# EpicDuckPotato/stereo_vo

Measured on AMD Instinct MI355X. Metric: stereo frames/sec on 1241x376 KITTI pairs, higher is better.
Workload: dtype u8/f32/f64; 1 GPU; kitti_1241x376_1500corners_5kf_window (BASELINE configs[1]); streams_per_gpu=96, max_corners=1500, window=5, pipeline_groups=3, hardware_queues=4

## Files before the change

### include/svo.h

```cpp
#ifndef SVO_H_
#define SVO_H_

#include <stddef.h>
#include <stdint.h>

#ifdef __cplusplus
extern "C" {
#endif

typedef enum svo_status {
  SVO_OK = 0,
  SVO_ERR_INVALID = -1,
  SVO_ERR_HIP = -2,
  SVO_ERR_CAPACITY = -3,
  SVO_ERR_NO_DEVICE = -4,
  SVO_ERR_NUMERIC = -5
} svo_status;

typedef struct svo_camera_info {
  double focal, cx, cy;
  double k1, k2, p1, p2;
  double baseline;
} svo_camera_info;

// ... 195 lines not shown
typedef struct svo_lm_ops {
  void* user;
  int (*linearize)(void* user, double radius, int first, double* payload1);
  int (*step)(void* user, const double* dc, const double* cand_poses7, double radius, const svo_lm_step_ctl* ctl,
              double* payload2, double* payload1_next, double* next_radius, int* next_at_candidate);
  int (*accept)(void* user);
} svo_lm_ops;
typedef struct svo_lm_stats {
  int linearize_calls;
  int step_calls;
  int speculations;
  int speculation_hits;
  int single_exchange;
  int collectives;
  int device_control;
  int fallbacks;
  double host_us;
} svo_lm_stats;

void svo_ba_default_options(svo_ba_options* o);
int svo_lm_solve(int n_poses, double* poses7, const svo_lm_ops* ops, const svo_ba_options* opt,
                 svo_ba_summary* summary, svo_lm_stats* stats);
int svo_lm_decide_step(double cost, double mcc, double radius, double decrease_factor, double cost_new,
                       double model_change_points, int* accept, double* next_radius);
int svo_ba_create(svo_ctx* ctx, svo_ba** out, int window_size, const svo_camera_info* cam,
                  const svo_ba_options* opt, int max_landmarks, int max_observations);
void svo_ba_destroy(svo_ba* ba);
int svo_ba_reset(svo_ba* ba);
int svo_ba_add_keyframe(svo_ba* ba, const double* pose7, const int64_t* tracked_ids,
                        const float* tracked_xy, int n_tracked, const float* new_xy,
                        const float* new_xyz, int n_new, int64_t* new_ids, int* n_new_out);
int svo_ba_solve(svo_ba* ba, svo_ba_summary* summary);
int svo_cholesky_solve(double* A, double* b, int n);
int svo_cholesky_solve_dev(svo_ctx* ctx, double* A, double* b, int n);
int svo_ba_get_pose(svo_ba* ba, int k, double* pose7);
int svo_ba_window_count(svo_ba* ba);
int svo_ba_get_points(svo_ba* ba, const int64_t* ids, int n, float* xyz);

int svo_ba_load_problem(svo_ba* ba, int n_poses, const double* poses7, int n_points,
                        const double* points3, int n_obs, const int32_t* obs_pose,
                        const int32_t* obs_point, const double* obs_uv);
int svo_ba_set_allreduce(svo_ba* ba, svo_allreduce_fn fn, void* user);
int svo_ba_set_comm(svo_ba* ba, void* nccl_comm);
int svo_rccl_unique_id(void* id128);
int svo_rccl_comm_create(void** nccl_comm, int n_ranks, int rank, const void* id128, int device);
int svo_rccl_comm_destroy(void* nccl_comm);
int svo_ba_set_device_lm(svo_ba* ba, int mode);
int svo_ba_set_solve_form(svo_ba* ba, int form);
int svo_ba_set_bulk_control(svo_ba* ba, int mode);
int svo_ba_last_stats(svo_ba* ba, svo_lm_stats* stats);
int svo_ba_wave_chunks_limit(void);
int svo_ba_set_wave_chunks(svo_ba* ba, int k);
int svo_ba_solve_forms(svo_ba* ba, long* counts, int n, long* gave_up);
int svo_ba_solve_problem(svo_ba* ba, svo_ba_summary* summary);
int svo_ba_solve_problems(svo_ba** bas, int n, svo_ba_summary* summaries);
int svo_ba_read_problem(svo_ba* ba, double* poses7, double* points3);

typedef struct svo_pipeline svo_pipeline;
typedef struct svo_pipeline_params {
  svo_camera_info cam;
  int width, height;
  int max_corners;
  double quality;
  float min_feature_distance;
  float parallax_thresh;
  int window_size;
  int max_features;
  int ba_max_iterations;
  double ba_max_time_s;
} svo_pipeline_params;

typedef struct svo_frame_result {
  int n_detected, n_tracked, n_inliers, n_new;
  int is_keyframe;
  float av_parallax, percent_lost;
  double pose7[7];
  int ba_iterations;
} svo_frame_result;

void svo_pipeline_default_params(svo_pipeline_params* p);
int svo_pipeline_create(svo_ctx* ctx, svo_pipeline** out, const svo_pipeline_params* p);
void svo_pipeline_destroy(svo_pipeline* p);
int svo_pipeline_reset(svo_pipeline* p);
int svo_pipeline_process_batch_dev(svo_pipeline* p, const uint8_t* left, const uint8_t* right,
                                   int batch, svo_frame_result* results);
int svo_pipeline_process_batch(svo_pipeline* p, const uint8_t* left, const uint8_t* right,
                               int batch, svo_frame_result* results);
int svo_pipeline_set_rectification(svo_pipeline* p, const svo_rectify_eye* left, const svo_rectify_eye* right);
int svo_pipeline_set_keyframe_clouds(svo_pipeline* p, const svo_cloud_params* params, int max_keyframes_per_call);
int svo_pipeline_set_keyframe_speckle_filter(svo_pipeline* p, const svo_speckle_params* params);
int svo_pipeline_set_keyframe_lr_check(svo_pipeline* p, const svo_lr_check_params* params);
int svo_pipeline_set_keyframe_sgm(svo_pipeline* p, const svo_sgm_params* params);
typedef struct svo_keyframe_cloud {
  int frame;
  int lane;
  int n_total, n_stored;
  const svo_cloud_point* dev;
} svo_keyframe_cloud;
int svo_pipeline_keyframe_clouds(svo_pipeline* p, int* n, const svo_keyframe_cloud** table);
int svo_pipeline_copy_keyframe_cloud(svo_pipeline* p, int i, svo_cloud_point* host, int capacity);
int svo_pipeline_get_tracked(svo_pipeline* p, int64_t* ids, float* xy, int capacity, int* n);

typedef struct svo_pipeline_group svo_pipeline_group;
int svo_pipeline_group_create(svo_ctx* ctx, svo_pipeline_group** out, const svo_pipeline_params* p, int n_lanes);
void svo_pipeline_group_destroy(svo_pipeline_group* g);
int svo_pipeline_group_reset(svo_pipeline_group* g);
int svo_pipeline_group_lanes(const svo_pipeline_group* g);
int svo_pipeline_group_process_batch_dev(svo_pipeline_group* g, const uint8_t* left, const uint8_t* right, size_t lane_stride,
                                         int batch, svo_frame_result* results);
int svo_pipeline_group_staging(svo_pipeline_group* g, int slot, uint8_t** left, uint8_t** right, size_t* lane_stride);
int svo_pipeline_group_upload(svo_pipeline_group* g, int slot, int batch);
int svo_pipeline_group_process_uploaded(svo_pipeline_group* g, int slot, svo_frame_result* results);
int svo_pipeline_group_process_batch(svo_pipeline_group* g, const uint8_t* left, const uint8_t* right, size_t lane_stride,
                                     int batch, svo_frame_result* results);
int svo_pipeline_group_set_rectification(svo_pipeline_group* g, int lane, const svo_rectify_eye* left, const svo_rectify_eye* right);
int svo_pipeline_group_set_keyframe_clouds(svo_pipeline_group* g, int lane, const svo_cloud_params* params, int max_keyframes_per_call);
int svo_pipeline_group_set_keyframe_speckle_filter(svo_pipeline_group* g, const svo_speckle_params* params);
int svo_pipeline_group_set_keyframe_lr_check(svo_pipeline_group* g, const svo_lr_check_params* params);
int svo_pipeline_group_set_keyframe_sgm(svo_pipeline_group* g, const svo_sgm_params* params);
int svo_pipeline_group_keyframe_clouds(svo_pipeline_group* g, int* n, const svo_keyframe_cloud** table);
int svo_pipeline_group_copy_keyframe_cloud(svo_pipeline_group* g, int i, svo_cloud_point* host, int capacity);
int svo_pipeline_group_get_tracked(svo_pipeline_group* g, int lane, int64_t* ids, float* xy, int capacity, int* n);
int svo_pipeline_group_last_stats(const svo_pipeline_group* g, long* launches6, long* lanes6);
int svo_pipeline_group_solve_work(svo_pipeline_group* g, double* out4, int reset);
int svo_pipeline_group_solve_forms(svo_pipeline_group* g, long* counts, int n, long* gave_up);

int svo_draw_track(const uint8_t* gray, int width, int height, int row_stride, const float* from_xy,
                   const float* to_xy, int n, uint8_t* rgb);
int svo_pipeline_draw_track(svo_pipeline* p, const uint8_t* keyframe_gray, int row_stride, uint8_t* rgb);

typedef struct svo_synth_params {
  uint64_t seed;
  int width, height;
  double focal, cx, cy, baseline;
  double step_z, step_x, yaw_per_frame;
  int n_billboards;
} svo_synth_params;
void svo_synth_default_params(svo_synth_params* p, int width, int height);
int svo_synth_render(const svo_synth_params* p, int frame, uint8_t* left, uint8_t* right);
int svo_synth_pose(const svo_synth_params* p, int frame, double* rt12);

int svo_image_read_gray(const char* path, uint8_t* buf, size_t capacity, int* width, int* height);
int svo_kitti_read_poses(const char* poses_file, double* rt12, int capacity_frames, int* n_frames);
int svo_ate_rmse(const double* est_xyz, const double* gt_xyz, int n, int with_scale, double* rmse);
typedef struct svo_run_stats {
  int frames, keyframes;
  double ate_rmse;
  double seconds;
} svo_run_stats;
int svo_kitti_run(svo_ctx* ctx, const svo_pipeline_params* params, const char* data_path, int sequence,
                  int max_frames, double* traj_rt12, svo_run_stats* stats);

#ifdef __cplusplus
}
#endif
#endif
```

### stereo_vo_amd/api.py

```python
import ctypes as C
import os

import numpy as np

_HERE = os.path.dirname(os.path.abspath(__file__))
_LIB = None


class SvoError(RuntimeError):
    pass


def lib_path():
    return os.path.join(_HERE, "libsvo_hip.so")


class Limits(C.Structure):
    _fields_ = [("max_width", C.c_int), ("max_height", C.c_int), ("max_batch", C.c_int),
                ("max_corners", C.c_int), ("max_candidates", C.c_int), ("max_features", C.c_int)]


class CameraInfo(C.Structure):
    _fields_ = [(n, C.c_double) for n in ("focal", "cx", "cy", "k1", "k2", "p1", "p2", "baseline")]

# ... 216 lines not shown
def lm_decide_step(cost, mcc, radius, decrease_factor, cost_new, model_change_points):
    acc, rad = C.c_int(0), C.c_double(0.0)
    lib().svo_lm_decide_step(C.c_double(cost), C.c_double(mcc), C.c_double(radius), C.c_double(decrease_factor), C.c_double(cost_new),
                             C.c_double(model_change_points), C.byref(acc), C.byref(rad))
    return bool(acc.value), rad.value


def lm_solve(poses7, linearize, step, accept, max_iterations=50, max_time_s=0.0):
    poses = np.ascontiguousarray(poses7, np.float64).copy()
    K = poses.shape[0]
    n = 6 * (K - 1)
    pay1 = n * n + 3 * n + 2

    def _lin(user, radius, first, out):
        np.ctypeslib.as_array(out, shape=(pay1,))[:] = linearize(radius, first)
        return 0

    def _step(user, dc, cand, radius, ctl, out2, out1, out_radius, out_at_cand):
        d = np.ctypeslib.as_array(dc, shape=(max(n, 1),))[:n].copy()
        c = np.ctypeslib.as_array(cand, shape=(K, 7)).copy()
        p2, p1, nr, at_cand = step(d, c, radius, ctl.contents)
        np.ctypeslib.as_array(out2, shape=(4,))[:] = p2
        if p1 is not None:
            np.ctypeslib.as_array(out1, shape=(pay1,))[:] = p1
        out_radius[0] = nr if p1 is not None else 0.0
        out_at_cand[0] = int(bool(at_cand))
        return 0

    def _acc(user):
        accept()
        return 0
    ops = LmOps(None, LM_LINEARIZE_FN(_lin), LM_STEP_FN(_step), LM_ACCEPT_FN(_acc))
    opt = ba_default_options()
    opt.max_iterations, opt.max_time_s = max_iterations, max_time_s
    s, st = BASummary(), LmStats()
    rc = lib().svo_lm_solve(K, _p(poses), C.byref(ops), C.byref(opt), C.byref(s), C.byref(st))
    if rc:
        raise SvoError(f"svo_lm_solve failed ({rc})")
    return poses, s, st


ALLREDUCE_FN = C.CFUNCTYPE(C.c_int, C.c_void_p, C.c_size_t, C.c_void_p)

SYMBOLS = [
    "svo_create", "svo_destroy", "svo_last_error", "svo_stream", "svo_sync", "svo_version", "svo_reference_constants",
    "svo_profile_select", "svo_profile_read", "svo_measure_peak",
    "svo_reproj_eval", "svo_reproj_eval_dev",
    "svo_corner_detect", "svo_corner_detect_batch_dev", "svo_corner_response",
    "svo_stereo_bm", "svo_stereo_disparity_at", "svo_stereo_disparity_at_dev",
    "svo_triangulate", "svo_lk_track", "svo_build_pyramid", "svo_track_features", "svo_dedup",
    "svo_pnp_ransac",
    "svo_ba_default_options", "svo_ba_create", "svo_ba_destroy", "svo_ba_reset", "svo_ba_add_keyframe", "svo_ba_solve",
    "svo_ba_get_pose", "svo_ba_window_count", "svo_ba_get_points", "svo_ba_load_problem",
    "svo_ba_set_allreduce", "svo_ba_set_device_lm", "svo_ba_set_bulk_control", "svo_ba_set_solve_form", "svo_ba_wave_chunks_limit", "svo_ba_set_wave_chunks", "svo_ba_solve_forms", "svo_ba_solve_problem", "svo_ba_solve_problems", "svo_ba_read_problem", "svo_ba_set_comm", "svo_ba_last_stats", "svo_lm_solve", "svo_lm_decide_step",
    "svo_rccl_unique_id", "svo_rccl_comm_create", "svo_rccl_comm_destroy",
    "svo_pipeline_default_params", "svo_pipeline_create", "svo_pipeline_destroy", "svo_pipeline_reset",
    "svo_pipeline_process_batch_dev", "svo_pipeline_process_batch", "svo_pipeline_get_tracked",
    "svo_pipeline_group_create", "svo_pipeline_group_destroy", "svo_pipeline_group_reset", "svo_pipeline_group_lanes",
    "svo_pipeline_group_process_batch_dev", "svo_pipeline_group_get_tracked", "svo_pipeline_group_last_stats",
    "svo_pipeline_group_solve_work", "svo_pipeline_group_solve_forms", "svo_pipeline_group_staging", "svo_pipeline_group_upload", "svo_pipeline_group_process_uploaded", "svo_pipeline_group_process_batch",
    "svo_synth_default_params", "svo_synth_render", "svo_synth_pose",
    "svo_image_read_gray", "svo_kitti_read_poses", "svo_ate_rmse", "svo_kitti_run", "svo_cholesky_solve", "svo_cholesky_solve_dev", "svo_draw_track", "svo_pipeline_draw_track",
    "svo_rectify_eye_from_camera_info", "svo_rectify_build_map", "svo_rectify_remap", "svo_rectify_remap_batch_dev",
    "svo_pipeline_set_rectification", "svo_pipeline_group_set_rectification",
    "svo_stereo_bm_batch_dev", "svo_cloud_default_params", "svo_disparity_cloud_batch_dev", "svo_stereo_cloud",
    "svo_pipeline_set_keyframe_clouds", "svo_pipeline_keyframe_clouds", "svo_pipeline_copy_keyframe_cloud",
    "svo_pipeline_group_set_keyframe_clouds", "svo_pipeline_group_keyframe_clouds", "svo_pipeline_group_copy_keyframe_cloud",
    "svo_speckle_workspace_bytes", "svo_disparity_speckle_filter_batch_dev", "svo_disparity_speckle_filter",
    "svo_pipeline_set_keyframe_speckle_filter", "svo_pipeline_group_set_keyframe_speckle_filter",
    "svo_stereo_bm_cost_batch_dev", "svo_disparity_lr_check_batch_dev", "svo_disparity_lr_check",
    "svo_pipeline_set_keyframe_lr_check", "svo_pipeline_group_set_keyframe_lr_check",
    "svo_sgm_default_params", "svo_sgm_workspace_bytes", "svo_stereo_sgm_batch_dev", "svo_stereo_sgm",
    "svo_pipeline_set_keyframe_sgm", "svo_pipeline_group_set_keyframe_sgm",
    "svo_voxel_map_default_params", "svo_voxel_map_bytes", "svo_voxel_map_create", "svo_voxel_map_destroy", "svo_voxel_map_clear",
    "svo_voxel_map_insert_dev", "svo_pose7_to_cam_to_world", "svo_voxel_map_insert_pose7_dev", "svo_voxel_map_stats",
    "svo_voxel_map_extract_dev", "svo_voxel_map_extract", "svo_voxel_map_download",
]


def lib():
    global _LIB
    if _LIB is None:
        p = lib_path()
        if not os.path.exists(p):
            raise SvoError(f"{p} not built — run `python -c 'import __graft_entry__ as g; g.build()'`")
        L = C.CDLL(p)
        L.svo_version.restype = C.c_char_p
        L.svo_last_error.restype = C.c_char_p
        L.svo_last_error.argtypes = [C.c_void_p]
        L.svo_stream.restype = C.c_void_p
        L.svo_stream.argtypes = [C.c_void_p]
        L.svo_destroy.argtypes = [C.c_void_p]
        L.svo_destroy.restype = None
        vp, ci, sz = C.c_void_p, C.c_int, C.c_size_t
        L.svo_cloud_default_params.argtypes = [vp, ci, ci]
        L.svo_stereo_bm_batch_dev.argtypes = [vp, vp, vp, ci, ci, ci, ci, sz, ci, ci, vp]
        L.svo_disparity_cloud_batch_dev.argtypes = [vp, vp, vp, ci, ci, ci, ci, sz, vp, vp, vp, vp, vp]
        L.svo_stereo_cloud.argtypes = [vp, vp, vp, ci, ci, ci, ci, ci, vp, vp, vp, vp, vp, vp]
        L.svo_pipeline_set_keyframe_clouds.argtypes = [vp, vp, ci]
        L.svo_pipeline_keyframe_clouds.argtypes = [vp, vp, vp]
        L.svo_pipeline_copy_keyframe_cloud.argtypes = [vp, ci, vp, ci]
        L.svo_pipeline_group_set_keyframe_clouds.argtypes = [vp, ci, vp, ci]
        L.svo_pipeline_group_keyframe_clouds.argtypes = [vp, vp, vp]
        L.svo_pipeline_group_copy_keyframe_cloud.argtypes = [vp, ci, vp, ci]
        for f in ("svo_cloud_default_params", "svo_stereo_bm_batch_dev", "svo_disparity_cloud_batch_dev", "svo_stereo_cloud",
                  "svo_pipeline_set_keyframe_clouds", "svo_pipeline_keyframe_clouds", "svo_pipeline_copy_keyframe_cloud",
                  "svo_pipeline_group_set_keyframe_clouds", "svo_pipeline_group_keyframe_clouds", "svo_pipeline_group_copy_keyframe_cloud"):
            getattr(L, f).restype = ci
        L.svo_speckle_workspace_bytes.argtypes = [ci, ci, ci]
        L.svo_speckle_workspace_bytes.restype = sz
        L.svo_disparity_speckle_filter_batch_dev.argtypes = [vp, vp, ci, ci, ci, vp, vp, sz, vp]
        L.svo_disparity_speckle_filter.argtypes = [vp, vp, ci, ci, vp, vp]
        L.svo_pipeline_set_keyframe_speckle_filter.argtypes = [vp, vp]
# ... 439 lines not shown
        ctx._chk(self.L.svo_ba_create(ctx.h, C.byref(self.h), window_size, C.byref(cam), C.byref(opt),
                                      max_landmarks, max_observations), "svo_ba_create")
        if device_lm is not None:
            ctx._chk(self.L.svo_ba_set_device_lm(self.h, 1 if device_lm else 0), "svo_ba_set_device_lm")
        if solve_form is not None:
            ctx._chk(self.L.svo_ba_set_solve_form(self.h, {"wide": 0, "compact": 1}[solve_form]), "svo_ba_set_solve_form")
        if bulk_control is not None:
            ctx._chk(self.L.svo_ba_set_bulk_control(self.h, 1 if bulk_control else 0), "svo_ba_set_bulk_control")
        self.L.svo_ba_destroy.argtypes = [C.c_void_p]
        self._cb = None

    def close(self):
        if self.h:
            self.L.svo_ba_destroy(self.h)
            self.h = C.c_void_p()

    def __del__(self):
        try:
            self.close()
        except Exception:
            pass

    def load_problem(self, poses7, points3, obs_pose, obs_point, obs_uv):
        poses7, points3, obs_uv = _f64(poses7), _f64(points3), _f64(obs_uv)
        op = np.ascontiguousarray(obs_pose, np.int32)
        oj = np.ascontiguousarray(obs_point, np.int32)
        self._shape = (poses7.shape[0], points3.shape[0])
        self.ctx._chk(self.L.svo_ba_load_problem(self.h, poses7.shape[0], _p(poses7), points3.shape[0],
                                                 _p(points3), op.shape[0], _p(op), _p(oj), _p(obs_uv)),
                      "svo_ba_load_problem")

    def set_allreduce(self, fn):
        self._cb = ALLREDUCE_FN(lambda ptr, n, user: int(fn(ptr, n) or 0)) if fn else None
        self.ctx._chk(self.L.svo_ba_set_allreduce(self.h, self._cb if self._cb else C.cast(None, ALLREDUCE_FN), None),
                      "svo_ba_set_allreduce")

    def set_comm(self, nccl_comm):
        self.ctx._chk(self.L.svo_ba_set_comm(self.h, C.c_void_p(nccl_comm) if nccl_comm else None), "svo_ba_set_comm")

    def solve_problem(self):
        s = BASummary()
        self.ctx._chk(self.L.svo_ba_solve_problem(self.h, C.byref(s)), "svo_ba_solve_problem")
        return s

    def set_wave_chunks(self, k):
        self.ctx._chk(self.L.svo_ba_set_wave_chunks(self.h, int(k)), "svo_ba_set_wave_chunks")

    def solve_forms(self):
        n = self.L.svo_ba_wave_chunks_limit() + 1
        out, gu = (C.c_long * n)(), C.c_long(0)
        self.ctx._chk(self.L.svo_ba_solve_forms(self.h, out, n, C.byref(gu)), "svo_ba_solve_forms")
        return list(out), gu.value

    @staticmethod
    def solve_problems(bas):
        n = len(bas)
        hs = (C.c_void_p * n)(*[b.h for b in bas])
        sums = (BASummary * n)()
        rc = bas[0].L.svo_ba_solve_problems(hs, n, sums)
        if rc < 0:
            bas[0].ctx._chk(rc, "svo_ba_solve_problems")
        return rc, list(sums)

    def last_stats(self):
        st = LmStats()
        self.ctx._chk(self.L.svo_ba_last_stats(self.h, C.byref(st)), "svo_ba_last_stats")
        return st

    def read_problem(self):
        K, N = self._shape
        poses = np.empty((K, 7))
        pts = np.empty((N, 3))
        self.ctx._chk(self.L.svo_ba_read_problem(self.h, _p(poses), _p(pts)), "svo_ba_read_problem")
        return poses, pts

    def add_keyframe(self, pose7, tracked_ids, tracked_xy, new_xy, new_xyz):
        pose7 = _f64(pose7)
        tid = np.ascontiguousarray(tracked_ids, np.int64)
        txy, nxy, nxyz = _f32(tracked_xy), _f32(new_xy), _f32(new_xyz)
        nn = nxy.shape[0] if nxy.ndim == 2 else 0
        ids = np.empty(max(nn, 1), np.int64)
        m = C.c_int(0)
        self.ctx._chk(self.L.svo_ba_add_keyframe(self.h, _p(pose7), _p(tid), _p(txy), tid.shape[0], _p(nxy),
                                                 _p(nxyz), nn, _p(ids), C.byref(m)), "svo_ba_add_keyframe")
        return ids[:m.value].copy()

    def solve(self):
        s = BASummary()
        self.ctx._chk(self.L.svo_ba_solve(self.h, C.byref(s)), "svo_ba_solve")
        return s

    def get_pose(self, k=-1):
        p = np.empty(7)
        self.ctx._chk(self.L.svo_ba_get_pose(self.h, k, _p(p)), "svo_ba_get_pose")
        return p

    def window_count(self):
        return self.L.svo_ba_window_count(self.h)

    def get_points(self, ids):
        ids = np.ascontiguousarray(ids, np.int64)
        out = np.empty((ids.shape[0], 3), np.float32)
        self.ctx._chk(self.L.svo_ba_get_points(self.h, _p(ids), ids.shape[0], _p(out)), "svo_ba_get_points")
        return out


# ... 168 lines not shown
        self.ctx._chk(self.L.svo_pipeline_group_process_batch_dev(self.h, C.c_void_p(left_ptr), C.c_void_p(right_ptr), C.c_size_t(lane_stride),
                                                                  batch, res), "svo_pipeline_group_process_batch_dev")
        self.last_raw = bytes(res)
        return [list(res[l * batch:(l + 1) * batch]) for l in range(self.n_lanes)]

    def staging(self, slot):
        lp, rp, stride = C.POINTER(C.c_uint8)(), C.POINTER(C.c_uint8)(), C.c_size_t(0)
        self.L.svo_pipeline_group_staging.argtypes = [C.c_void_p, C.c_int, C.c_void_p, C.c_void_p, C.c_void_p]
        self.ctx._chk(self.L.svo_pipeline_group_staging(self.h, slot, C.byref(lp), C.byref(rp), C.byref(stride)), "svo_pipeline_group_staging")
        h, w = self.prm.height, self.prm.width
        mb = stride.value // (h * w)
        shape = (self.n_lanes, mb, h, w)
        n = self.n_lanes * mb * h * w
        return (np.ctypeslib.as_array(lp, shape=(n,)).reshape(shape), np.ctypeslib.as_array(rp, shape=(n,)).reshape(shape))

    def upload(self, slot, batch):
        self.ctx._chk(self.L.svo_pipeline_group_upload(self.h, slot, batch), "svo_pipeline_group_upload")

    def process_uploaded(self, slot, batch):
        res = (FrameResult * (self.n_lanes * batch))()
        self.L.svo_pipeline_group_process_uploaded.argtypes = [C.c_void_p, C.c_int, C.c_void_p]
        self.ctx._chk(self.L.svo_pipeline_group_process_uploaded(self.h, slot, res), "svo_pipeline_group_process_uploaded")
        self.last_raw = bytes(res)
        return [list(res[l * batch:(l + 1) * batch]) for l in range(self.n_lanes)]

    def process_batch(self, left, right):
        left, right = _u8(left), _u8(right)
        batch = left.shape[1]
        res = (FrameResult * (self.n_lanes * batch))()
        self.L.svo_pipeline_group_process_batch.argtypes = [C.c_void_p, C.c_void_p, C.c_void_p, C.c_size_t, C.c_int, C.c_void_p]
        self.ctx._chk(self.L.svo_pipeline_group_process_batch(self.h, _p(left), _p(right), C.c_size_t(batch * left.shape[2] * left.shape[3]), batch, res),
                      "svo_pipeline_group_process_batch")
        self.last_raw = bytes(res)
        return [list(res[l * batch:(l + 1) * batch]) for l in range(self.n_lanes)]

    def get_tracked(self, lane, capacity=8192):
        ids = np.empty(capacity, np.int64)
        xy = np.empty((capacity, 2), np.float32)
        n = C.c_int(0)
        self.ctx._chk(self.L.svo_pipeline_group_get_tracked(self.h, lane, _p(ids), _p(xy), capacity, C.byref(n)), "svo_pipeline_group_get_tracked")
        return ids[:n.value].copy(), xy[:n.value].copy()

    def solve_work(self, reset=False):
        out = (C.c_double * 4)()
        self.ctx._chk(self.L.svo_pipeline_group_solve_work(self.h, out, int(reset)), "svo_pipeline_group_solve_work")
        return list(out)

    def solve_forms(self):
        n = self.L.svo_ba_wave_chunks_limit() + 1
        out, gu = (C.c_long * n)(), C.c_long(0)
        self.ctx._chk(self.L.svo_pipeline_group_solve_forms(self.h, out, n, C.byref(gu)), "svo_pipeline_group_solve_forms")
        return list(out), gu.value

    def last_stats(self):
        a, b = (C.c_long * 6)(), (C.c_long * 6)()
        self.ctx._chk(self.L.svo_pipeline_group_last_stats(self.h, a, b), "svo_pipeline_group_last_stats")
        return {s: (a[i], b[i]) for i, s in enumerate(self.STAGES) if s != "unused"}


class RunStats(C.Structure):
    _fields_ = [("frames", C.c_int), ("keyframes", C.c_int), ("ate_rmse", C.c_double), ("seconds", C.c_double)]


def image_read_gray(path, max_pixels=1 << 24):
    buf = np.empty(max_pixels, np.uint8)
    w, h = C.c_int(0), C.c_int(0)
    rc = lib().svo_image_read_gray(path.encode(), _p(buf), C.c_size_t(max_pixels), C.byref(w), C.byref(h))
    if rc:
        raise SvoError(f"svo_image_read_gray({path}) rc={rc}")
    return buf[:w.value * h.value].reshape(h.value, w.value).copy()


def kitti_read_poses(path, max_frames=100000):
    rt = np.empty((max_frames, 12))
    n = C.c_int(0)
    rc = lib().svo_kitti_read_poses(path.encode(), _p(rt), max_frames, C.byref(n))
    if rc:
        raise SvoError(f"svo_kitti_read_poses({path}) rc={rc}")
    return rt[:n.value].reshape(-1, 3, 4).copy()


def ate_rmse(est_xyz, gt_xyz, with_scale=False):
    est_xyz, gt_xyz = _f64(est_xyz), _f64(gt_xyz)
    out = C.c_double(0)
    rc = lib().svo_ate_rmse(_p(est_xyz), _p(gt_xyz), est_xyz.shape[0], int(with_scale), C.byref(out))
    if rc:
        raise SvoError(f"svo_ate_rmse rc={rc}")
    return out.value


def kitti_run(ctx, params, data_path, sequence, max_frames):
    traj = np.zeros((max_frames, 12))
    st = RunStats()
    ctx._chk(lib().svo_kitti_run(ctx.h, C.byref(params), data_path.encode(), sequence, max_frames, _p(traj), C.byref(st)),
             "svo_kitti_run")
    return traj[:st.frames].reshape(-1, 3, 4).copy(), st


def cholesky_solve(A, b):
    A = np.array(A, np.float64, order="C")
    b = np.array(b, np.float64)
    rc = lib().svo_cholesky_solve(_p(A), _p(b), b.shape[0])
    if rc != 0:
        raise SvoError(f"svo_cholesky_solve rc={rc}")
    return b

# ... 11 lines not shown
```

### stereo_vo_amd/csrc/ba.hip

```cpp
#include <math.h>
#include <stdlib.h>

#include <errno.h>
#include <fcntl.h>
#include <signal.h>
#include <sys/mman.h>
#include <sys/types.h>
#include <unistd.h>

#include <algorithm>
#include <atomic>
#include <mutex>
#include <sched.h>
#include <chrono>
#include <deque>
#include <memory>
#include <vector>

#include "kernels.h"
#include "group_kernels.h"
#include "lm_decide.h"
#include "lm_device.h"
#include "lm_turns.h"
#include "ref_constants.h"
// ... 1460 lines not shown
  __shared__ double sm[RED_LDS_DOUBLES];
  __shared__ double sOut[4];
  __shared__ int sFlag;
  const int tid = threadIdx.x, b = blockIdx.x;
  const int nb1 = with_pay1 ? ba_reduce_blocks(P.E, P.NG) : 0, epb = ba_reduce_epb(P.NG);
  if (b < nb1) {
    double* out = P.pay1_out;
    (void)reduce_elements<true>(P, b * epb, min(P.E, (b + 1) * epb), P.pay_tag, sm, RED_LDS_DOUBLES, &sFlag, [out](int e, double v) { pay_store(&out[e], v); });
  } else if (with_pay2) {
    (void)sum_pay2<true>(P, P.pay_parity, P.pay_tag, sm, sOut, &sFlag);
    if (tid < 4) pay_store(&P.pay2_out[tid], sOut[tid]);
    if (ctl.chain) {
      if (tid == 0) decide_device(ctl, sOut[0], sOut[1], P.ctl_dev, P.pay2_out);
    }
  }
  reduce_publish(P);
}

__device__ __forceinline__ bool wait_until(const unsigned* word, unsigned target, bool monotone) {
  long long t0 = 0;
  for (unsigned spins = 0;; ++spins) {
    const unsigned v = __hip_atomic_load(word, __ATOMIC_RELAXED, __HIP_MEMORY_SCOPE_AGENT);
    if (monotone ? (int)(v - target) >= 0 : v == target) return true;
    __builtin_amdgcn_s_sleep(2);
    if ((spins & 255u) == 255u) {
      const long long tn = (long long)wall_clock64();
      if (!t0) t0 = tn;
      else if (tn - t0 > LM_WAIT_TICKS) return false;
    }
  }
}

struct LmDevArgs {
  unsigned* cnt;
  const void* arena_src;
  void* arena_dst;
  size_t arena_bytes;
  double* points_a;
  double* points_b;
  double* export_points;
  float4* store;
  unsigned store_mask;
  double* dev_res;
  double* host_result;
  int* host_flag;
  int host_seq;
  unsigned base_arrive;
  int tab_words;
  LmDevOpt opt;
  unsigned* dbg;
  int test_giveup;
  int wave_chunks;
  int wave_contig;
};
enum { LMC_ARRIVE = 0, LMC_WORDS = 16 };
enum { LMR_ITERATIONS = 0, LMR_SUCCESSFUL, LMR_TERMINATION, LMR_INITIAL_COST, LMR_FINAL_COST, LMR_LINEARIZE_CALLS, LMR_STEP_CALLS, LMR_SEL,
       LMR_T_WAIT, LMR_T_CTL, LMR_T_BODY, LMR_T_TOTAL, LMR_SAME_SWEEP, LMR_NEXT_USED, LMR_C_ARRIVE, LMR_TP0, LMR_DOUBLES = LMR_TP0 + 14 };
enum { LMS_START = 0, LMS_FIRST, LMS_RELIN, LMS_STEP, LMS_ACCEPT_RELIN, LMS_DELIVER };
enum { LMOP_EXIT = 0, LMOP_LINEARIZE, LMOP_ITERATE, LMOP_DELIVER, LMOP_ABORT };

struct LmDevState {
  double radius, df, cost, initial_cost, mcc, spec;
  double elapsed;
  double pay2[6];
  int iterations, successful, termination, need_linearize, state, sel, chain, first, saturated;
  unsigned arrive_total;
  int lin_calls, step_calls, same_sweeps, next_used;
  int go, act, use_next, accepted, relin, bad, flag;
  unsigned long long tag;
  unsigned op_count;
  long long t0, t_wait, t_ctl, t_body, t_mark;
  long long tp[14];
};
constexpr double LM_MIN_RADIUS = 1e-32, LM_MAX_RADIUS = 1e16;

__host__ __device__ static inline size_t ba_lm_ctl_doubles(int n, int K) { return (size_t)n * n + 3 * (size_t)n + 2 + 4 * (size_t)(n > 0 ? n : 1) + (size_t)(n > 0 ? n : 1) + 14 * (size_t)K + 21 * (size_t)(K > 1 ? K - 1 : 1) + 8; }
__host__ __device__ static inline int ba_wire_elements(int K) { const int F = K - 1; return 18 * F * (F + 1) + 33 * F + 2; }
__host__ __device__ static inline size_t ba_lm_union_doubles(int n, int K) { const size_t a = (size_t)LM_CPW * (size_t)wg_lds_doubles(ba_wire_elements(K)), b = ba_lm_ctl_doubles(n, K); return a > b ? a : b; }
__host__ __device__ static inline size_t ba_lm_lds_doubles(int n, int K, int tab_words , int kw = 1) {
  return ba_lm_union_doubles(n, K) + (size_t)LM_CPW * (size_t)kw * (size_t)tab_words / 4 + 3 * (size_t)(n > 0 ? n : 1) + 14 * (size_t)K;
}

__device__ __forceinline__ void lm_place_total(int e, double v, double* cP, double* cU, int F, int n) {
  const int nU = F * (F + 1) / 2;
  if (e < 36 * nU) {
    const int d = e / 36, el = e - 36 * d;
    int ka = 0, rest = d;
    while (rest >= F - ka) { rest -= F - ka; ++ka; }
    const int kb = ka + rest;
    cP[(6 * ka + el / 6) * n + 6 * kb + el % 6] = v;
  } else if (e < 36 * nU + 33 * F) {
    const int k = (e - 36 * nU) / 33, el = (e - 36 * nU) - 33 * k;
    if (el < 6) cP[n * n + n + 6 * k + el] = v;
    else if (el < 12) cP[n * n + 6 * k + (el - 6)] = v;
    else cU[21 * k + (el - 12)] = v;
  } else {
    cP[n * n + 3 * n + (e - 36 * nU - 33 * F)] = v;
  }
}
__device__ __forceinline__ void lm_fold_u(double* cP, const double* cU, int F, int n) {
  for (int i = threadIdx.x; i < 36 * F; i += (int)blockDim.x) {
    const int k = i / 36, a = (i % 36) / 6, b = i % 6;
    const int lo = a < b ? a : b, hi = a < b ? b : a;
    const double uu = cU[21 * k + lo * 6 - lo * (lo - 1) / 2 + (hi - lo)];
    double* s = &cP[(6 * k + a) * n + 6 * k + b];
    *s = uu + *s;
    if (a == b) cP[n * n + 2 * n + 6 * k + a] = uu;
  }
  __syncthreads();
}

__device__ __forceinline__ bool lm_fetch_totals(double* cP, double* cU, const double* res, int F, int n, unsigned long long tag, double* elapsed, int n_blocks, int* s_flag) {
  const int nU = F * (F + 1) / 2, E = 36 * nU + 33 * F + 2;
  {
    const int per = (E + n_blocks - 1) / n_blocks, slices = (E + per - 1) / per;
    if (!wait_sentinels(res, per - 1, per, slices - 1, tag, s_flag)) return false;
    if (!wait_sentinels(res, E - 1, 1, 2, tag, s_flag)) return false;
  }
// ... 3 lines not shown
#pragma unroll
    for (int u = 0; u < 8; ++u) {
      const int i = base + u * (int)blockDim.x + (int)threadIdx.x;
      gi[u] = i < E + 1 ? i : -1;
    }
    double v[8];
    unsigned ok = granule_load8(res, gi, tag, v);
    long long t0 = 0;
    for (unsigned spins = 0; ok != 0xFFu; ++spins) {
      __builtin_amdgcn_s_sleep(2);
      if ((spins & 255u) == 255u) {
        const long long tn = (long long)wall_clock64();
        if (!t0) t0 = tn;
        else if (tn - t0 > LM_WAIT_TICKS) break;
      }
      int again[8];
#pragma unroll
      for (int u = 0; u < 8; ++u) again[u] = (ok >> u) & 1u ? -1 : gi[u];
      double w[8];
      const unsigned ok2 = granule_load8(res, again, tag, w);
#pragma unroll
      for (int u = 0; u < 8; ++u) if (!((ok >> u) & 1u) && ((ok2 >> u) & 1u)) { v[u] = w[u]; ok |= 1u << u; }
    }
    good = good && ok == 0xFFu;
#pragma unroll
    for (int u = 0; u < 8; ++u) {
      const int e = gi[u];
      if (e < 0) continue;
      if (e < E) lm_place_total(e, v[u], cP, cU, F, n);
      else *elapsed = v[u];
    }
  }
  __syncthreads();
  lm_fold_u(cP, cU, F, n);
  return good;
}

template <bool LOCAL, bool GROUPED = false, bool MULTI = false>
__device__ __attribute__((noinline)) int lm_controller(const BaDev& P, const LmDevArgs& a, LmDevState& cs, double* cl, double* cSc, double* sStep, double* sOut4,
                                                        const double* tot = nullptr, const double* tot2 = nullptr) {
  const int tid = threadIdx.x, nt = blockDim.x, n = P.n, K = P.K, nn = n > 0 ? n : 1;
  const int grid = LOCAL ? 1 : ba_lm_blocks(P.C, MULTI ? a.wave_chunks : 1);
  const int pay1 = n * n + 3 * n + 2;
  double* cP = cl;
  double* cDf = cP + pay1;
  double* cRhs = cDf + nn;
  double* cCol = cRhs + nn;
  double* cTerm = cCol + nn;
  double* cU = cTerm + nn + 14 * K;
  double* cDc = sStep;
  double* cCand = sStep + nn;
  double* cPose = cCand + 7 * K;
  const LmDevOpt& opt = a.opt;
  enum { ACT_NONE = 0, ACT_LOOPTOP, ACT_FINISH, ACT_ACCEPT_TAIL, ACT_SOLVE };
  int act = ACT_NONE;
  auto issue = [&](int op) {
    if (tid == 0) {
      if (op == LMOP_DELIVER) cs.arrive_total += (unsigned)grid;
      cs.tag = (1ull << 62) | ((unsigned long long)(unsigned)a.host_seq << 20) | (unsigned long long)(++cs.op_count & 0xFFFFFu);
      const long long tn = (long long)wall_clock64();
      cs.t_ctl += tn - cs.t_mark; cs.t_mark = tn;
    }
    __syncthreads();
    return op;
  };

  auto cstamp = [&](int slot) { if (a.dbg && tid == 0) { const long long tn = (long long)wall_clock64(); cs.tp[slot] += tn - cs.tp[11]; cs.tp[11] = tn; } };
  const int st = cs.state;
  __syncthreads();
  if (st == LMS_START) {
    if (tid == 0) {
      cs.go = 1;
      cs.radius = opt.initial_radius; cs.df = 2.0; cs.cost = 0.0; cs.initial_cost = 0.0; cs.mcc = 0.0; cs.elapsed = 0.0;
      cs.t0 = cs.t_mark = (long long)wall_clock64();
      cs.iterations = 0; cs.successful = 0; cs.termination = 1; cs.need_linearize = 0; cs.sel = 0; cs.chain = 0; cs.spec = 0.0; cs.saturated = 0;
      cs.arrive_total = a.base_arrive;
      cs.lin_calls = 1; cs.step_calls = 0; cs.same_sweeps = 0; cs.next_used = 0; cs.bad = 0; cs.op_count = 0; cs.tag = 0;
      cs.t_wait = cs.t_ctl = cs.t_body = 0;
      for (int i = 0; i < 14; ++i) cs.tp[i] = 0;
      cs.state = LMS_FIRST; cs.first = 1;
    }
    __syncthreads();
    {
      const ptrdiff_t shift = a.arena_src ? reinterpret_cast<const char*>(a.arena_src) - reinterpret_cast<const char*>(a.arena_dst) : 0;
      for (int i = tid; i < 7 * K; i += nt) cPose[i] = sys_load(&P.poses[i], shift);
    }
    return issue(LMOP_LINEARIZE);
  }
  if (st == LMS_DELIVER) return LMOP_EXIT;

  if (tid == 0) {
    const long long w0 = (long long)wall_clock64();
    cs.t_body += w0 - cs.t_mark;
    cs.t_mark = w0;
    cs.first = 0;
  }
  __syncthreads();
  if (a.dbg && tid == 0) cs.tp[11] = (long long)wall_clock64();

  bool fetch = true;
  if (st == LMS_STEP) {
    if (!cs.chain) {
      if constexpr (LOCAL) {
        if (tid < 4) cs.pay2[tid] = tot2[tid];
      } else {
        if (!sum_pay2<GROUPED>(P, (int)(cs.op_count & 1u), cs.tag, cP, sOut4, &cs.flag)) { if (tid == 0) cs.bad = 1; }
        if (tid < 4) cs.pay2[tid] = sOut4[tid];
      }
      __syncthreads();
    }
    for (int i = tid; i < 7 * K; i += nt) {
      const double dd = cCand[i] - cPose[i];
      cTerm[i] = dd * dd;
      cTerm[7 * K + i] = cPose[i] * cPose[i];
    }
    __syncthreads();
    if (tid == 0) {
      const double* cPay2 = cs.pay2;
      const double cost_new = cPay2[0], model_change = cs.mcc + cPay2[1];
      double step2 = cPay2[2], x2 = cPay2[3];
      for (int i = 7; i < 7 * K; ++i) { step2 += cTerm[i]; x2 += cTerm[7 * K + i]; }
      const bool have_next = cs.chain != 0 || cs.spec > 0;
      const bool next_at_cand = cs.spec > 0 ? true : cPay2[4] != 0.0;
      const double next_radius = cs.spec > 0 ? cs.spec : cPay2[5];
      int a_ = ACT_LOOPTOP, use = 0, relin = 0;
      if (!(model_change > 0)) {
        cs.radius /= cs.df; cs.df *= 2; cs.saturated = 0;
        use = have_next && next_radius > 0 && next_radius == cs.radius && !next_at_cand;
        cs.need_linearize = !use;
      } else if (sqrt(step2) <= opt.parameter_tolerance * (sqrt(x2) + opt.parameter_tolerance)) {
        cs.termination = 0; a_ = ACT_FINISH;
      } else if (fabs(cs.cost - cost_new) <= opt.function_tolerance * cs.cost) {
        cs.termination = 0; a_ = ACT_FINISH;
      } else {
        const SvoLmDecision dec = svo_lm_decide(cs.cost, cs.mcc, cs.radius, cs.df, cost_new, cPay2[1]);
        if (dec.accept) {
          cs.sel ^= 1;
          cs.cost = cost_new;
          ++cs.successful;
          cs.saturated = dec.next_radius == fmin(LM_MAX_RADIUS, cs.radius / (1.0 / 3.0));
          cs.radius = dec.next_radius;
          cs.df = 2.0;
          use = have_next && next_radius > 0 && next_radius == cs.radius && next_at_cand;
          relin = !use;
          a_ = ACT_ACCEPT_TAIL;
        } else {
          cs.radius = dec.next_radius; cs.df *= 2; cs.saturated = 0;
          use = have_next && next_radius > 0 && next_radius == cs.radius && !next_at_cand;
          cs.need_linearize = !use;
        }
      }
      cs.accepted = a_ == ACT_ACCEPT_TAIL;
      cs.next_used += use;
      cs.act = a_; cs.use_next = use; cs.relin = relin;
    }
    __syncthreads();
    if (cs.accepted) for (int i = tid; i < 7 * K; i += nt) cPose[i] = cCand[i];
    fetch = cs.chain != 0 || cs.spec > 0;
  }
  if (fetch) {
    if (tid == 0) { const long long w0 = (long long)wall_clock64(); cs.t_mark = w0; }
    if constexpr (LOCAL) {
      for (int e = tid; e < P.E; e += nt) lm_place_total(e, tot[e], cP, cU, K - 1, n);
      __syncthreads();
      lm_fold_u(cP, cU, K - 1, n);
    } else {
      if (!lm_fetch_totals(cP, cU, a.dev_res, K - 1, n, cs.tag, &cs.elapsed, grid, &cs.flag)) { if (tid == 0) cs.bad = 1; }
    }
    if (tid == 0) { const long long w1 = (long long)wall_clock64(); cs.t_wait += w1 - cs.t_mark; cs.t_mark = w1; }
  }
  __syncthreads();
  if (st == LMS_STEP) {
    act = cs.act;
    const bool relin = act == ACT_ACCEPT_TAIL && cs.relin;
    __syncthreads();
    if (relin) {
      if (tid == 0) { ++cs.lin_calls; cs.state = LMS_ACCEPT_RELIN; }
      return issue(LMOP_LINEARIZE);
    }
  } else {
    if (st == LMS_FIRST) {
      if (tid == 0) { cs.cost = cP[pay1 - 2]; cs.initial_cost = cs.cost; }
      for (int q = tid; q < n; q += nt) cSc[q] = 1.0 / (1.0 + sqrt(cP[n * n + 2 * n + q]));
      act = ACT_ACCEPT_TAIL;
    } else if (st == LMS_RELIN) {
      if (tid == 0) cs.need_linearize = 0;
      act = ACT_SOLVE;
    } else {
      act = ACT_ACCEPT_TAIL;
    }
    __syncthreads();
  }

  __syncthreads();
  cstamp(6);
  if (cs.bad) return LMOP_ABORT;
  for (;;) {
    if (act == ACT_ACCEPT_TAIL) {
      for (int q = tid; q < n; q += nt) { const double g = cP[n * n + n + q]; cTerm[q] = g * g; }
      __syncthreads();
      if (tid == 0) {
        double g2 = cP[pay1 - 1];
        for (int q = 0; q < n; ++q) g2 += cTerm[q];
        if (sqrt(g2) <= opt.gradient_tolerance) { cs.termination = 0; cs.act = ACT_FINISH; } else cs.act = ACT_LOOPTOP;
      }
      __syncthreads();
      act = cs.act;
      __syncthreads();
    }
    if (act == ACT_LOOPTOP) {
      if (tid == 0) {
        int a_ = ACT_SOLVE;
        if (cs.iterations >= opt.max_iterations) { cs.termination = 1; a_ = ACT_FINISH; }
        else if (opt.max_time_s > 0 && cs.elapsed >= opt.max_time_s) { cs.termination = 1; a_ = ACT_FINISH; }
        else if (cs.radius <= LM_MIN_RADIUS) { cs.termination = 0; a_ = ACT_FINISH; }
        else {
          ++cs.iterations;
          if (cs.need_linearize) { ++cs.lin_calls; cs.state = LMS_RELIN; a_ = ACT_NONE; }
        }
        cs.act = a_;
      }
      __syncthreads();
      act = cs.act;
      __syncthreads();
      if (act == ACT_NONE) return issue(LMOP_LINEARIZE);
    }
    if (act == ACT_FINISH) {
      if (tid == 0) cs.state = LMS_DELIVER;
      if (blockIdx.x == 0) {
        if (tid == 0) {
          double* r = a.host_result;
          pay_store(&r[LMR_ITERATIONS], (double)cs.iterations); pay_store(&r[LMR_SUCCESSFUL], (double)cs.successful);
          pay_store(&r[LMR_TERMINATION], (double)cs.termination); pay_store(&r[LMR_INITIAL_COST], cs.initial_cost);
          pay_store(&r[LMR_FINAL_COST], cs.cost); pay_store(&r[LMR_LINEARIZE_CALLS], (double)cs.lin_calls);
          pay_store(&r[LMR_STEP_CALLS], (double)cs.step_calls); pay_store(&r[LMR_SEL], (double)cs.sel);
          const long long tn = (long long)wall_clock64();
          pay_store(&r[LMR_T_WAIT], (double)cs.t_wait); pay_store(&r[LMR_T_CTL], (double)(cs.t_ctl + (tn - cs.t_mark)));
          pay_store(&r[LMR_T_BODY], (double)cs.t_body); pay_store(&r[LMR_T_TOTAL], (double)(tn - cs.t0));
          pay_store(&r[LMR_SAME_SWEEP], (double)cs.same_sweeps); pay_store(&r[LMR_NEXT_USED], (double)cs.next_used);
          pay_store(&r[LMR_C_ARRIVE], (double)(cs.arrive_total + (unsigned)grid));
          for (int i = 0; i < 14; ++i) pay_store(&r[LMR_TP0 + i], (double)cs.tp[i]);
        }
        for (int i = tid; i < 7 * K; i += nt) pay_store(&a.host_result[LMR_DOUBLES + i], cPose[i]);
      }
      return issue(LMOP_DELIVER);
    }
    const double radius = cs.radius;
    for (int q = tid; q < n; q += nt) {
      const double sq = cSc[q];
      cDf[q] = fmin(fmax(cP[n * n + 2 * n + q] * sq * sq, MIN_DIAG), MAX_DIAG) / radius;
      cRhs[q] = -(cP[n * n + q] + cP[n * n + n + q]) * sq;
    }
    __syncthreads();
    for (int r = tid >> 3; r < n; r += nt >> 3) {
      const double sr = cSc[r];
      for (int c = tid & 7; c <= r; c += 8) {
        const double v = (r / 6 > c / 6) ? cP[c * n + r] : cP[r * n + c];
        double w = v * sr * cSc[c];
        if (r == c) w += cDf[r];
        cP[r * n + c] = w;
      }
    }
    __syncthreads();
    cstamp(7);
    const bool ok = n == 0 || svo_dev_cholesky_solve(cP, cRhs, n, cCol);
    cstamp(8);
    if (ok) {
      for (int q = tid; q < n; q += nt) {
        const double rq = cRhs[q], sq = cSc[q];
        cDc[q] = rq * sq;
        cTerm[q] = 0.5 * rq * (cDf[q] * rq - cP[n * n + n + q] * sq);
      }
      __syncthreads();
      if (tid == 0) {
        double mcc = 0.0;
        for (int q = 0; q < n; ++q) mcc += cTerm[q];
        cs.mcc = mcc;
        cs.chain = 0; cs.spec = 0.0;
        if (cs.iterations < opt.max_iterations) {
          if (cs.saturated) { cs.spec = fmin(LM_MAX_RADIUS, cs.radius / (1.0 / 3.0)); ++cs.same_sweeps; }
          else cs.chain = 1;
        }
        ++cs.step_calls;
        cs.state = LMS_STEP;
      }
      if (tid < K) {
        if (tid == 0) for (int q = 0; q < 7; ++q) cCand[q] = cPose[q];
        else svo_plus_pose(&cPose[7 * tid], &cDc[6 * (tid - 1)], &cCand[7 * tid]);
      }
      __syncthreads();
      cstamp(9);
      return issue(LMOP_ITERATE);
    }
    if (tid == 0) { cs.radius /= cs.df; cs.df *= 2; cs.need_linearize = 1; }
    __syncthreads();
    act = ACT_LOOPTOP;
  }
}
// ... 188 lines not shown
  return ok;
}

#ifndef SVO_LM_WAVES_PER_EU
#define SVO_LM_WAVES_PER_EU 2
#endif
template <bool GROUPED, bool MULTI = false>
__device__ __forceinline__ void ba_lm_body(const LmLanePtrs& lanes) {
  extern __shared__ double lds[];
  __shared__ LmShared sh;
  __shared__ LmDevState cs;
  __shared__ __align__(16) unsigned char sLaneRaw[sizeof(LmLane)];
  LmLane& sLane = *reinterpret_cast<LmLane*>(sLaneRaw);
  const int tid = threadIdx.x, lane = tid & 63, wave = tid >> 6;
  {
    const unsigned* src = reinterpret_cast<const unsigned*>(lanes.p[blockIdx.y]);
    unsigned* dst = reinterpret_cast<unsigned*>(&sLane);
    for (int i = tid; i < (int)(sizeof(LmLane) / 4); i += blockDim.x) dst[i] = __hip_atomic_load(&src[i], __ATOMIC_RELAXED, __HIP_MEMORY_SCOPE_SYSTEM);
  }
  __syncthreads();
  const int kw = MULTI ? sLane.a.wave_chunks : 1;
  const int n_blocks = ba_lm_blocks(sLane.P.C, kw);
  if ((int)blockIdx.x >= n_blocks) return;
  BaDev P = sLane.P;
  const LmDevArgs& a = sLane.a;
  const int n = P.n, K = P.K, nn = n > 0 ? n : 1;
  const int union_doubles = (int)ba_lm_union_doubles(n, K);
  double* union_lds = lds;
  const WgLds L = wg_lds(lds + wave * wg_lds_doubles(P.E), P.E);
  uint16_t* tabs = reinterpret_cast<uint16_t*>(lds + union_doubles) + wave * kw * a.tab_words;
  double* cSc = lds + union_doubles + LM_CPW * kw * a.tab_words / 4;
  double* sStep = cSc + 2 * nn;
  const int my_chunk = (int)blockIdx.x * LM_CPW + wave;
  const bool my_wave_works = !MULTI && my_chunk < P.C;
  const LmTurns turns = lm_turns(P.C, kw, n_blocks, MULTI && a.wave_contig);
  if (a.test_giveup) {
    if (blockIdx.x == 0 && tid == 0) __hip_atomic_store(a.host_flag, -a.host_seq, __ATOMIC_RELAXED, __HIP_MEMORY_SCOPE_SYSTEM);
    return;
  }
  __builtin_amdgcn_s_setprio(3);
  P.step_in = nullptr;
  P.flag = nullptr;
  if (tid == 0) { cs.state = LMS_START; cs.bad = 0; cs.accepted = 0; }
  LmWave W;
  W.R = ObsRec{false, 0, 0, 0, lane, 0, D3{0, 0, 1}, 0.0, 0.0};
  W.cand = D3{0, 0, 1};
  W.c.s[0] = W.c.s[1] = W.c.s[2] = 1.0;
  const ptrdiff_t shift = a.arena_src ? reinterpret_cast<const char*>(a.arena_src) - reinterpret_cast<const char*>(a.arena_dst) : 0;
  if (my_wave_works) {
    W.R = load_obs_image(P, my_chunk, lane, a.points_a, shift);
    if (shift && W.R.active && lane == W.R.first) { a.points_a[3 * W.R.j] = W.R.p.x; a.points_a[3 * W.R.j + 1] = W.R.p.y; a.points_a[3 * W.R.j + 2] = W.R.p.z; }
    load_chunk_table(P, my_chunk, tabs, shift);
  }
  if (MULTI) {
    for (int t = 0; t < turns.count; ++t) {
      const int chunk = turns.chunk(t);
      const ObsRec R = load_obs_image(P, chunk, lane, a.points_a, shift);
      if (shift) {
        const int4 rc = R.active ? make_int4(R.k, R.j, R.first, R.len) : make_int4(-1, 0, 0, 0);
        const_cast<int4*>(P.rec)[R.o] = rc;
        double* uv = const_cast<double*>(P.obs_uv) + 2 * R.o;
        uv[0] = R.u; uv[1] = R.v;
        if (R.active && lane == R.first) { a.points_a[3 * R.j] = R.p.x; a.points_a[3 * R.j + 1] = R.p.y; a.points_a[3 * R.j + 2] = R.p.z; }
      }
      load_chunk_table(P, chunk, tabs + t * a.tab_words, shift);
    }
    stores_acknowledged();
  }
  long long t_first = 0;
  __syncthreads();
  for (;;) {
    const int st_before = cs.state;
    const int op = lm_controller<false, GROUPED, MULTI>(P, a, cs, union_lds, cSc, sStep, sh.sOut);
    if (a.dbg && tid == 0) {
      unsigned* g = a.dbg + 16 * blockIdx.x;
      g[0] = (unsigned)op; g[1] = (unsigned)cs.state; g[2] = (unsigned)cs.iterations; g[3] = (unsigned)cs.need_linearize;
      g[4] = (unsigned)cs.chain | ((unsigned)cs.bad << 8);
      g[5] = cs.arrive_total; g[6] = cs.op_count; g[7] = (unsigned)cs.lin_calls;
    }
    if (op == LMOP_ABORT || cs.bad) {
      if (tid == 0) __hip_atomic_store(a.host_flag, -a.host_seq, __ATOMIC_RELAXED, __HIP_MEMORY_SCOPE_SYSTEM);
      return;
    }
    if (op == LMOP_EXIT) break;
    if (!MULTI && st_before == LMS_STEP && cs.accepted) W.R.p = W.cand;
    if (!t_first) t_first = (long long)wall_clock64();
    const bool sel = cs.sel != 0;
    P.points = sel ? a.points_b : a.points_a;
    P.cand_points = sel ? a.points_a : a.points_b;
    P.pay_tag = cs.tag;
    P.pay_parity = (int)(cs.op_count & 1u);
    if (op == LMOP_DELIVER) {
      if (a.export_points && my_wave_works) {
        ObsRec R = W.R;
        if (R.active) R.p = D3{P.points[3 * R.j], P.points[3 * R.j + 1], P.points[3 * R.j + 2]};
        deliver_chunk_points(R, a.export_points, union_lds + wave * ((64 * REC_STRIDE) / LM_CPW), (64 * REC_STRIDE) / LM_CPW);
      }
      if (MULTI) {
        double* stage = union_lds + wave * ((64 * REC_STRIDE) / LM_CPW);
        for (int t = turns.count - 1; t >= 0; --t) {
          const ObsRec R = load_obs(P, turns.chunk(t), lane, P.points);
          if (a.export_points) deliver_chunk_points(R, a.export_points, stage, (64 * REC_STRIDE) / LM_CPW);
          if (a.store && R.active && lane == R.first) {
            const unsigned key = sys_load(&P.lm_key[R.j], shift);
            const unsigned long long lo = ((unsigned long long)__float_as_uint((float)R.p.y) << 32) | __float_as_uint((float)R.p.x);
            const unsigned long long hi = ((unsigned long long)key << 32) | __float_as_uint((float)R.p.z);
            slot_store2<true>(reinterpret_cast<double*>(a.store + (key & a.store_mask)), __longlong_as_double((long long)lo), __longlong_as_double((long long)hi));
          }
          wave_lds_fence();
        }
      }
      if (a.store && my_wave_works && W.R.active && lane == W.R.first) {
        const int j = W.R.j;
        const unsigned key = sys_load(&P.lm_key[j], shift);
        const float x = (float)P.points[3 * j], y = (float)P.points[3 * j + 1], z = (float)P.points[3 * j + 2];
        const unsigned long long lo = ((unsigned long long)__float_as_uint(y) << 32) | __float_as_uint(x), hi = ((unsigned long long)key << 32) | __float_as_uint(z);
        slot_store2<true>(reinterpret_cast<double*>(a.store + (key & a.store_mask)), __longlong_as_double((long long)lo), __longlong_as_double((long long)hi));
      }
      if (a.dbg && tid == 0) {
        unsigned* g = a.dbg + 16 * blockIdx.x;
        for (int i = 0; i < 6; ++i) g[8 + i] = (unsigned)cs.tp[i];
        g[8 + 3] = (unsigned)(cs.tp[3] + cs.tp[10]);
        g[14] = (unsigned)cs.tp[6];
      }
      stores_acknowledged();
      __syncthreads();
      if (tid == 0) {
        const unsigned old = __hip_atomic_fetch_add(a.cnt + LMC_ARRIVE, 1u, __ATOMIC_RELAXED, __HIP_MEMORY_SCOPE_AGENT);
        if (old + 1u == cs.arrive_total) __hip_atomic_store(a.host_flag, a.host_seq, __ATOMIC_RELAXED, __HIP_MEMORY_SCOPE_SYSTEM);
      }
      __syncthreads();
      continue;
    }
    long long* tp = a.dbg ? cs.tp : nullptr;
    bool good;
    if constexpr (MULTI) good = lm_iterate_multi(P, a, turns, tabs, L, union_lds, union_doubles, cs, sStep, sh, n_blocks, t_first, op == LMOP_ITERATE ? tp : nullptr, op != LMOP_ITERATE);
    else good = lm_iterate<GROUPED>(P, a, W, my_wave_works, tabs, L, union_lds, union_doubles, cs, sStep, sh, n_blocks, t_first, op == LMOP_ITERATE ? tp : nullptr, op != LMOP_ITERATE);
    if (!good) {
      if (tid == 0) __hip_atomic_store(a.host_flag, -a.host_seq, __ATOMIC_RELAXED, __HIP_MEMORY_SCOPE_SYSTEM);
      return;
    }
    __syncthreads();
  }
}
__global__ __launch_bounds__(128) __attribute__((amdgpu_waves_per_eu(SVO_LM_WAVES_PER_EU, SVO_LM_WAVES_PER_EU))) void ba_lm_kernel(LmLanePtrs lanes) { ba_lm_body<false>(lanes); }
__global__ __launch_bounds__(128) __attribute__((amdgpu_waves_per_eu(SVO_LM_WAVES_PER_EU, SVO_LM_WAVES_PER_EU))) void ba_lm_grouped_kernel(LmLanePtrs lanes) { ba_lm_body<true>(lanes); }
__global__ __launch_bounds__(128) __attribute__((amdgpu_waves_per_eu(SVO_LM_WAVES_PER_EU, SVO_LM_WAVES_PER_EU))) void ba_lm_multi_kernel(LmLanePtrs lanes) { ba_lm_body<false, true>(lanes); }

constexpr int LMC_MAX_WAVES = 6;
__host__ __device__ static inline int lmc_wave_doubles(int E) { return 64 * REC_STRIDE + ((E + 1) & ~1) + 2 + 4; }
__host__ __device__ static inline size_t ba_lmc_union_doubles(int n, int K, int NW) {
  const size_t a = (size_t)NW * (size_t)lmc_wave_doubles(ba_wire_elements(K)), b = ba_lm_ctl_doubles(n, K);
  return a > b ? a : b;
}
__host__ __device__ static inline size_t ba_lmc_lds_doubles(int n, int K, int tab_words, int NW) {
  const size_t Ep = ((size_t)ba_wire_elements(K) + 1) & ~(size_t)1, nn = n > 0 ? n : 1;
  return ba_lmc_union_doubles(n, K, NW) + (size_t)NW * (size_t)tab_words / 4 + 2 * Ep + 8 + 3 * nn + 14 * (size_t)K;
}

__device__ __forceinline__ void lmc_acc(double* tot, double* q, int idx, int c, int C, int G, double p) {
  if (G <= 1) { tot[idx] = c == 0 ? p : tot[idx] + p; return; }
  const int r = c % G;
  const double qq = r == 0 ? p : q[idx] + p;
  if (r == G - 1 || c == C - 1) tot[idx] = c < G ? qq : tot[idx] + qq;
  else q[idx] = qq;
}

struct LmcLds { double* wave_area; uint16_t* tab; double *tot, *q, *tot2, *q2; int wave_doubles; };

__device__ __forceinline__ void lmc_sweep(const BaDev& P, const LmcLds& L, const double* sStep, bool do_b, bool do_a, bool a_from_b, bool a_at_cand,
// ... 441 lines not shown
  if (threadIdx.x < 2) atomicAdd(&gDU[n + threadIdx.x], sAcc[threadIdx.x]);
}

struct svo_ba {
  svo_ctx* ctx = nullptr;
  svo_camera_info cam{};
  svo_ba_options opt{};
  int window_size = 5, max_landmarks = 0, max_obs = 0, max_poses = 0;
  svo_allreduce_fn allreduce = nullptr;
  void* allreduce_user = nullptr;
  void* comm = nullptr;
  BaDev d;
  size_t cap_points = 0, cap_obs = 0, cap_pay1 = 0;
  size_t cap_part1 = 0, cap_part2 = 0, cap_res = 0;
  double* d_res = nullptr;
  unsigned long long tag_seq = 0;
  int tab_max_words = 0;
  double flops_iter = 0, bytes_iter = 0;
  double acc_flops = 0, acc_bytes = 0, acc_solves = 0, acc_iters = 0;
  std::vector<double> h_poses;
  int n_points = 0;
  uint8_t* d_arena = nullptr;
  uint8_t* h_arena = nullptr;
  size_t arena_cap = 0;
  hipStream_t stream = nullptr;
  bool stream_owned = true;
  double* d_pay = nullptr;
  double* d_step = nullptr;
  double* d_bctl = nullptr;
  double* h_bstat = nullptr;
  int bulk_ctl = -1;
  uint8_t* h_pin = nullptr;
  size_t pin_bytes = 0;
  int* h_flag = nullptr;
  double* h_step = nullptr;
  bool res_export = false;
  bool host_points_valid = false;
  size_t arena_pts_off = 0, arena_bytes = 0;
  bool arena_dirty = false;
  double* h_out_points = nullptr;
  FusedAdmission res_admission;
  unsigned* d_lmc = nullptr;
  unsigned* d_lmdbg = nullptr;
  double* h_result = nullptr;
  int device_lm = -1;
  int lm_form = -1;
  bool lm_compact_inflight = false;
  int lm_wave_chunks = 0;
  long lm_k_solves[LM_MAX_WAVE_CHUNKS + 1] = {};
  int lm_penalty = 0;
  long wide_launches = 0;
  long fallbacks = 0;
  bool lm_inflight = false;
  hipStream_t lm_stream = nullptr;
  LmLane* h_lane = nullptr;
  unsigned lm_base = 0;
  bool lm_counters_dirty = false;
  bool lm_have_base = false;
  bool arena_partial = false;
  size_t arena_cpts_off = 0, arena_p0_off = 0, arena_p1_off = 0;
  std::chrono::steady_clock::time_point lm_t0;
  double* h_pay = nullptr;
  double *cur_points = nullptr, *cand_points = nullptr, *cur_poses = nullptr, *cand_poses = nullptr;
  bool have_scale = false;
  std::vector<double> mirror;
  struct Obs { float u, v; int64_t id; };
  struct PoseVar { double pose[7]; std::vector<Obs> obs; };
  std::deque<PoseVar> window;
  std::vector<double> feat_pos;
  bool new_frame_added = false;
  std::vector<int64_t> solve_lm_ids;
  bool upload_has_ids = false;
  float4* store = nullptr; unsigned store_mask = 0;
  float4* h_store_stage = nullptr; unsigned* h_store_slot = nullptr; size_t store_stage_cap = 0;
  std::vector<double> s_poses, s_points, s_uv, s_out_pts;
  std::vector<int32_t> s_op, s_oj;
  std::vector<int32_t> u_lm_start, u_chunks, u_cnt;
  std::vector<uint16_t> u_tab; std::vector<uint32_t> u_tab_off;
  unsigned* d_arrive = nullptr; unsigned arrive_total = 0; int seq = 0;
  bool upload_pending = false;
  bool mfma_ok = false;
  svo_lm_stats stats{};
  double lm_tp[14] = {0, 0, 0, 0, 0, 0, 0, 0, 0, 0, 0, 0, 0, 0};
  double lmc_tp[14] = {0, 0, 0, 0, 0, 0, 0, 0, 0, 0, 0, 0, 0, 0}; long lmc_n = 0, lmc_iters = 0, lm_iters_wide = 0;
  double lm_wg_min[7] = {0, 0, 0, 0, 0, 0, 0}, lm_wg_mean[7] = {0, 0, 0, 0, 0, 0, 0}, lm_wg_max[7] = {0, 0, 0, 0, 0, 0, 0};
  double lm_t_wait = 0, lm_t_ctl = 0, lm_t_body = 0, lm_t_total = 0; long lm_n = 0, lm_iters = 0, lm_same = 0, lm_used = 0, lm_steps = 0, lm_lins = 0;
  double t_lin = 0, t_step = 0, t_upload = 0, t_total = 0, t_prep = 0, t_read = 0; long n_lin = 0, n_step = 0, n_solves = 0, n_spec = 0, n_hit = 0;
};

static int ba_alloc(svo_ba* ba) {
  svo_ctx* ctx = ba->ctx;
  BaDev& d = ba->d;
  const int Kmax = ba->max_poses, nmax = 6 * (Kmax - 1);
  ba->cap_points = ba->max_landmarks; ba->cap_obs = ba->max_obs;
  ba->cap_pay1 = std::max((size_t)nmax * nmax + 3 * (size_t)nmax + 2 + 2, (size_t)(18 * (Kmax - 1) * Kmax + 33 * (Kmax - 1) + 2));
  const size_t step_doubles = (size_t)(nmax > 0 ? nmax : 1) + 7 * (size_t)Kmax;
#define A(ptr, T, cnt) SVO_HIP_CHECK(ctx, hipMalloc((void**)&(ptr), sizeof(T) * (size_t)(cnt)))
  A(d.sp, double, 3 * ba->cap_points);
  A(ba->d_pay, double, PAY2_SLOTS + ba->cap_pay1);
  A(ba->d_step, double, step_doubles);
  A(ba->d_bctl, double, BC_WORDS + (nmax > 0 ? nmax : 1));
  SVO_HIP_CHECK(ctx, hipHostMalloc((void**)&ba->h_bstat, sizeof(double) * ((size_t)BULK_RING * BS_DOUBLES + BC_WORDS), hipHostMallocCoherent));
  memset(ba->h_bstat, 0, sizeof(double) * ((size_t)BULK_RING * BS_DOUBLES + BC_WORDS));
  A(ba->d_lmc, unsigned, LMC_WORDS);
  SVO_HIP_CHECK(ctx, hipHostMalloc((void**)&ba->h_lane, sizeof(LmLane), hipHostMallocCoherent));
  if (getenv("SVO_BA_TRACE")) A(ba->d_lmdbg, unsigned, 16 * 4096);
  SVO_HIP_CHECK(ctx, hipMemset(ba->d_lmc, 0, LMC_WORDS * sizeof(unsigned)));
  A(ba->d_arrive, unsigned, 16);
  SVO_HIP_CHECK(ctx, hipMemset(ba->d_arrive, 0, 16 * sizeof(unsigned)));
#undef A
  {
    const size_t M = ba->cap_obs, Kc = (size_t)Kmax;
    const size_t pairs = M * (Kc + 1) / 2 + 64;
    const size_t slots = 2 * M + 64;
    const size_t est = 16 * 3 * ba->cap_points + (16 + 16) * slots + 2 * pairs + (slots / 64 + 2) * (2 * (Kc * Kc + 2 * Kc + 4) + 64 + 4) + 2 * 56 * Kc + 16 * 256;
    if (est < ((size_t)512 << 20)) {
      ba->arena_cap = est;
      SVO_HIP_CHECK(ctx, hipMalloc((void**)&ba->d_arena, ba->arena_cap));
      SVO_HIP_CHECK(ctx, hipHostMalloc((void**)&ba->h_arena, ba->arena_cap, hipHostMallocDefault));
    }
  }
  {
    const char* e = getenv("SVO_BA_CU_SHARE");
    const int nres = e ? atoi(e) : 0;
    if (nres > 0 && nres < 32 && ba->max_obs <= 100000) {
      uint32_t mask[8];
      for (int i = 0; i < 8; ++i) mask[i] = (1u << nres) - 1u;
      SVO_HIP_CHECK(ctx, hipExtStreamCreateWithCUMask(&ba->stream, 8, mask));
      g_ba_cu_share = nres;
    } else {
      SVO_HIP_CHECK(ctx, hipStreamCreateWithFlags(&ba->stream, hipStreamNonBlocking));
    }
  }
  {
    const size_t Fm = (size_t)Kmax - 1, Em = ((18 * Fm * (Fm + 1) + 33 * Fm + 2) + 7) & ~(size_t)7;
    if (Em * 128 * 16 <= ((size_t)64 << 20)) {
      SVO_HIP_CHECK(ctx, hipMalloc((void**)&d.part1, 16 * Em * 128));
      SVO_HIP_CHECK(ctx, hipMemsetAsync(d.part1, 0, 16 * Em * 128, ba->stream));
      ba->cap_part1 = Em * 128;
      SVO_HIP_CHECK(ctx, hipMalloc((void**)&d.part2, 16 * 2 * 4 * 128));
      SVO_HIP_CHECK(ctx, hipMemsetAsync(d.part2, 0, 16 * 2 * 4 * 128, ba->stream));
      ba->cap_part2 = 2 * 4 * 128;
      SVO_HIP_CHECK(ctx, hipMalloc((void**)&ba->d_res, 16 * (Em + 1)));
      SVO_HIP_CHECK(ctx, hipMemsetAsync(ba->d_res, 0, 16 * (Em + 1), ba->stream));
      ba->cap_res = Em + 1;
    }
    SVO_HIP_CHECK(ctx, hipDeviceSynchronize());
  }
  const size_t pin_step_doubles = step_doubles + 7 * (size_t)Kmax;
  ba->pin_bytes = 64 + 128 + sizeof(double) * (pin_step_doubles + PAY2_SLOTS + ba->cap_pay1 + 8 + 3 * ba->cap_points + LMR_DOUBLES + 7 * (size_t)Kmax + 8);
  SVO_HIP_CHECK(ctx, hipHostMalloc((void**)&ba->h_pin, ba->pin_bytes, hipHostMallocCoherent));
  memset(ba->h_pin, 0, ba->pin_bytes);
  ba->h_flag = reinterpret_cast<int*>(ba->h_pin);
  ba->h_step = reinterpret_cast<double*>(ba->h_pin + 64 + 128);
  ba->h_pay = ba->h_step + pin_step_doubles;
  ba->h_out_points = ba->h_pay + ((PAY2_SLOTS + ba->cap_pay1 + 7) & ~(size_t)7);
  ba->h_result = ba->h_out_points + ((3 * ba->cap_points + 7) & ~(size_t)7);
  d.pay2 = ba->d_pay;
  d.pay1 = ba->d_pay + PAY2_SLOTS;
  return SVO_OK;
}

extern "C" void svo_ba_default_options(svo_ba_options* o) {
  if (!o) return;
  o->max_iterations = 50;
  o->max_time_s = svo_ref::BA_MAX_SOLVER_TIME_S;
  o->function_tolerance = 1e-6;
  o->gradient_tolerance = 1e-10;
  o->parameter_tolerance = 1e-8;
  o->initial_radius = 1e4;
  o->max_features = svo_ref::MAX_FEATURES;
  o->accumulation = SVO_BA_ACC_AUTO;
}

extern "C" int svo_ba_create(svo_ctx* ctx, svo_ba** out, int window_size, const svo_camera_info* cam,
                             const svo_ba_options* opt, int max_landmarks, int max_observations) {
  if (!ctx || !out || !cam) return SVO_ERR_INVALID;
  svo_use_device(ctx);
  SVO_REQUIRE(ctx, window_size >= 1 && window_size <= 64, "ba_create: window size must be 1..64");
  SVO_REQUIRE(ctx, max_landmarks >= 1 && max_observations >= 1, "ba_create: capacities must be positive");
  svo_ba* ba = new svo_ba();
  ba->ctx = ctx;
  ba->cam = *cam;
  if (opt) ba->opt = *opt; else svo_ba_default_options(&ba->opt);
  ba->window_size = window_size;
  ba->max_poses = window_size + 1 > 2 ? window_size + 1 : 2;
  if (ba->max_poses > 64) ba->max_poses = 64;
  ba->max_landmarks = max_landmarks;
  ba->max_obs = max_observations;
  int rc = ba_alloc(ba);
  if (rc) { svo_ba_destroy(ba); return rc; }
  *out = ba;
  return SVO_OK;
}

extern "C" void svo_ba_destroy(svo_ba* ba) {
  if (!ba) return;
  BaDev& d = ba->d;
  if (getenv("SVO_TIMING") && ba->n_lin)
    fprintf(stderr, "[svo ba] %ld solves: pass A alone %.1f us x %ld, step (pass B + speculative pass A) %.1f us x %ld, speculation %ld/%ld hit, "
                    "per solve: gather %.1f us, upload %.1f us, upload + LM %.1f us, read-back %.1f us\n", ba->n_solves, 1e3 * ba->t_lin / ba->n_lin, ba->n_lin,
            ba->n_step ? 1e3 * ba->t_step / ba->n_step : 0.0, ba->n_step, ba->n_hit, ba->n_spec, 1e3 * ba->t_prep / std::max(ba->n_solves, 1l),
            1e3 * ba->t_upload / std::max(ba->n_solves, 1l), 1e3 * ba->t_total / std::max(ba->n_solves, 1l), 1e3 * ba->t_read / std::max(ba->n_solves, 1l));
  if (getenv("SVO_TIMING") && ba->lm_n)
    fprintf(stderr, "[svo ba] device-resident solves: %ld, %.1f LM iterations each; per solve (workgroup 0, us): total %.1f = waiting for the passes %.1f + step control %.1f "
                    "+ own share of the passes %.1f; steps %ld (same sweep %ld, next linearisation used %ld), stand-alone linearisations %ld\n", ba->lm_n, (double)ba->lm_iters / ba->lm_n, 1e-2 * ba->lm_t_total / ba->lm_n, 1e-2 * ba->lm_t_wait / ba->lm_n,
            1e-2 * ba->lm_t_ctl / ba->lm_n, 1e-2 * ba->lm_t_body / ba->lm_n, ba->lm_steps, ba->lm_same, ba->lm_used, ba->lm_lins);
  if (getenv("SVO_TIMING") && ba->lm_n) {
    fprintf(stderr, "[svo ba] solve forms: compact %ld, wide at k = 1..%d:", ba->lm_k_solves[0], LM_MAX_WAVE_CHUNKS);
    for (int k = 1; k <= LM_MAX_WAVE_CHUNKS; ++k) fprintf(stderr, " %ld", ba->lm_k_solves[k]);
    fprintf(stderr, "; gave up %ld\n", ba->fallbacks);
  }
  const bool wide_traced = ba->lm_iters_wide > 0 && ba->d_lmdbg != nullptr;
  const double wi = (double)std::max(ba->lm_iters_wide, 1l), ci = (double)std::max(ba->lmc_iters, 1l);
  if (getenv("SVO_TIMING") && wide_traced)
    fprintf(stderr, "[svo ba]   per LM iteration (workgroup 0, us): pass B %.2f, radius-free part of pass A %.2f, collecting payload2 + decision %.2f, rest of pass A %.2f, "
                    "own slice of level 2 %.2f (of which waiting for everybody's partials %.2f) | collecting the totals + assembly %.2f, system build %.2f, Cholesky %.2f, step tail %.2f\n", 1e-2 * ba->lm_tp[0] / wi, 1e-2 * ba->lm_tp[1] / wi,
            1e-2 * ba->lm_tp[2] / wi, 1e-2 * (ba->lm_tp[3] + ba->lm_tp[10]) / wi, 1e-2 * ba->lm_tp[4] / wi, 1e-2 * ba->lm_tp[5] / wi,
            1e-2 * ba->lm_tp[6] / wi, 1e-2 * ba->lm_tp[7] / wi, 1e-2 * ba->lm_tp[8] / wi, 1e-2 * ba->lm_tp[9] / wi);
  if (getenv("SVO_TIMING") && wide_traced)
    fprintf(stderr, "[svo ba]   rest of pass A, chained steps (workgroup 0's first wavefront, us per LM iteration): lanes' arithmetic behind the decision %.2f, Schur owners %.2f, "
                    "per-pose owners + posting the partials %.2f\n", 1e-2 * ba->lm_tp[10] / wi, 1e-2 * ba->lm_tp[12] / wi, 1e-2 * (ba->lm_tp[3] - ba->lm_tp[12]) / wi);
  if (getenv("SVO_TIMING") && wide_traced) {
    static const char* nm[7] = {"pass B", "radius-free part of pass A", "collecting payload2", "rest of pass A", "own slice of level 2", "waiting for the partials", "collecting the totals"};
    for (int sl = 0; sl < 7; ++sl)
      fprintf(stderr, "[svo ba]   over the workgroups of a solve, per LM iteration (us): %-28s min %.2f mean %.2f max %.2f\n", nm[sl], 1e-2 * ba->lm_wg_min[sl] / wi,
              1e-2 * ba->lm_wg_mean[sl] / wi, 1e-2 * ba->lm_wg_max[sl] / wi);
  }
  if (getenv("SVO_TIMING") && ba->lmc_iters && ba->d_lmdbg)
    fprintf(stderr, "[svo ba] compact solves: %ld, %.1f LM iterations each, %.1f rounds of turns per LM iteration; per LM iteration (wavefront 0, us): turns of sweeps with pass B %.2f, "
                    "turns of pass-A-only sweeps %.2f, waiting at a round's first barrier %.2f, in-order accumulation + second barrier %.2f | collecting the totals + assembly %.2f, "
                    "system build %.2f, Cholesky %.2f, step tail %.2f\n", ba->lmc_n, (double)ba->lmc_iters / std::max(ba->lmc_n, 1l), ba->lmc_tp[13] / ci, 1e-2 * ba->lmc_tp[0] / ci,
            1e-2 * ba->lmc_tp[3] / ci, 1e-2 * ba->lmc_tp[1] / ci, 1e-2 * ba->lmc_tp[2] / ci, 1e-2 * ba->lmc_tp[6] / ci, 1e-2 * ba->lmc_tp[7] / ci, 1e-2 * ba->lmc_tp[8] / ci, 1e-2 * ba->lmc_tp[9] / ci);
  if (ba->stream) (void)hipStreamSynchronize(ba->stream);
  void* ptrs[] = {ba->d_res, ba->d_lmdbg, ba->d_lmc, ba->d_arrive, ba->d_pay, ba->d_step, ba->d_bctl, d.sp, d.part1, d.part2, ba->d_arena};
  if (ba->h_bstat) (void)hipHostFree(ba->h_bstat);
  if (ba->h_arena) (void)hipHostFree(ba->h_arena);
  if (ba->h_store_stage) (void)hipHostFree(ba->h_store_stage);
  for (void* p : ptrs)
    if (p) (void)hipFree(p);
  if (ba->h_pin) (void)hipHostFree(ba->h_pin);
  if (ba->h_lane) (void)hipHostFree(ba->h_lane);
  if (ba->stream && ba->stream_owned) (void)hipStreamDestroy(ba->stream);
  delete ba;
}

extern "C" int svo_ba_set_allreduce(svo_ba* ba, svo_allreduce_fn fn, void* user) {
  if (!ba) return SVO_ERR_INVALID;
  ba->allreduce = fn;
  ba->allreduce_user = user;
  return SVO_OK;
}

extern "C" int svo_ba_set_comm(svo_ba* ba, void* nccl_comm) {
  if (!ba) return SVO_ERR_INVALID;
  ba->comm = nccl_comm;
  return SVO_OK;
}

extern "C" int svo_ba_set_device_lm(svo_ba* ba, int mode) {
  if (!ba || mode < -1 || mode > 1) return SVO_ERR_INVALID;
  ba->device_lm = mode;
  return SVO_OK;
}

int svo_ba_use_stream(svo_ba* ba, void* stream) {
  if (!ba || !stream || ba->lm_inflight) return SVO_ERR_INVALID;
  svo_use_device(ba->ctx);
  if (ba->stream) {
    (void)hipStreamSynchronize(ba->stream);
    if (ba->stream_owned) (void)hipStreamDestroy(ba->stream);
  }
  ba->stream = (hipStream_t)stream;
  ba->stream_owned = false;
  return SVO_OK;
}

void svo_ba_note_group_lanes(int delta) { g_group_lanes.fetch_add(delta, std::memory_order_relaxed); }

extern "C" int svo_ba_set_solve_form(svo_ba* ba, int form) {
  if (!ba || form < -1 || form > 1) return SVO_ERR_INVALID;
  ba->lm_form = form;
  return SVO_OK;
}

extern "C" int svo_ba_wave_chunks_limit(void) { return LM_MAX_WAVE_CHUNKS; }

extern "C" int svo_ba_set_wave_chunks(svo_ba* ba, int k) {
  if (!ba || k < 0 || k > LM_MAX_WAVE_CHUNKS) return SVO_ERR_INVALID;
  ba->lm_wave_chunks = k;
  return SVO_OK;
}

extern "C" int svo_ba_solve_forms(svo_ba* ba, long* counts, int n, long* gave_up) {
  if (!ba || !counts || n < 1) return SVO_ERR_INVALID;
  for (int i = 0; i < n; ++i) counts[i] = i <= LM_MAX_WAVE_CHUNKS ? ba->lm_k_solves[i] : 0;
  if (gave_up) *gave_up = ba->fallbacks;
  return SVO_OK;
}

extern "C" int svo_ba_set_bulk_control(svo_ba* ba, int mode) {
  if (!ba || mode < -1 || mode > 1) return SVO_ERR_INVALID;
  ba->bulk_ctl = mode;
  return SVO_OK;
}

extern "C" int svo_ba_last_stats(svo_ba* ba, svo_lm_stats* stats) {
  if (!ba || !stats) return SVO_ERR_INVALID;
  *stats = ba->stats;
  return SVO_OK;
}


static inline int ba_upper_index(int ka, int kb, int F) { return ka * F - ka * (ka - 1) / 2 + (kb - ka); }

static int ba_ensure_partials(svo_ba* ba) {
  svo_ctx* ctx = ba->ctx;
  BaDev& d = ba->d;
  auto grow = [&](double** p, size_t* cap, size_t granules) -> int {
    if (granules <= *cap) return SVO_OK;
    if (ba->upload_pending || ba->lm_inflight) SVO_HIP_CHECK(ctx, hipStreamSynchronize(ba->stream));
    if (*p) SVO_HIP_CHECK(ctx, hipFree(*p));
    *p = nullptr;
    const size_t want = granules + granules / 2 + 64;
    SVO_HIP_CHECK(ctx, hipMalloc((void**)p, 16 * want));
    SVO_HIP_CHECK(ctx, hipMemsetAsync(*p, 0, 16 * want, ba->stream));
    SVO_HIP_CHECK(ctx, hipStreamSynchronize(ba->stream));
    *cap = want;
    return SVO_OK;
  };
  int rc = grow(&d.part1, &ba->cap_part1, (size_t)d.Epad * (size_t)(d.NG > 0 ? d.NG : 1));
  if (!rc) rc = grow(&d.part2, &ba->cap_part2, 2 * 4 * (size_t)(d.NG > 0 ? d.NG : 1));
  if (!rc) rc = grow(&ba->d_res, &ba->cap_res, (size_t)d.E + 1);
  return rc;
}

static int ba_upload_checked(svo_ba* ba, int K, const double* poses7, int npts, const double* points3, int M,
                     const int32_t* op, const int32_t* oj, const double* uv) {
  svo_ctx* ctx = ba->ctx;
  SVO_REQUIRE(ctx, K >= 1 && K <= ba->max_poses, "ba: pose count outside the window capacity");
  SVO_REQUIRE(ctx, npts >= 0 && (size_t)npts <= ba->cap_points && M >= 0 && (size_t)M <= ba->cap_obs, "ba: problem exceeds capacity");
  BaDev& d = ba->d;
  if (ba->upload_pending) { SVO_HIP_CHECK(ctx, hipStreamSynchronize(ba->stream)); ba->upload_pending = false; }
  d.K = K; d.n = 6 * (K - 1); d.M = M; d.f = ba->cam.focal; d.cx = ba->cam.cx; d.cy = ba->cam.cy;
  ba->n_points = npts;
  std::vector<int32_t>&lm_start = ba->u_lm_start, &chunks = ba->u_chunks;
  lm_start.assign((size_t)npts + 1, 0);
  chunks.clear();
  for (int o = 0; o < M; ++o) {
    SVO_REQUIRE(ctx, oj[o] >= 0 && oj[o] < npts && op[o] >= 0 && op[o] < K, "ba: observation index out of range");
// ... 124 lines not shown
    ba->d_arena = nullptr; ba->h_arena = nullptr;
    ba->arena_cap = total + total / 4 + 4096;
    SVO_HIP_CHECK(ctx, hipMalloc((void**)&ba->d_arena, ba->arena_cap));
    SVO_HIP_CHECK(ctx, hipHostMalloc((void**)&ba->h_arena, ba->arena_cap, hipHostMallocDefault));
  }
  uint8_t* h = ba->h_arena;
  if (npts) { memcpy(h + o_pts, points3, sizeof(double) * 3 * (size_t)npts); memcpy(h + o_cpts, points3, sizeof(double) * 3 * (size_t)npts); }
  {
    int4* rec = reinterpret_cast<int4*>(h + o_rec);
    double* suv = reinterpret_cast<double*>(h + o_uv);
    for (int c = 0; c < d.C; ++c) {
      const int c0 = chunks[c], c1 = chunks[c + 1];
      for (int lane = 0; lane < 64; ++lane) {
        const size_t slot = (size_t)c * 64 + lane;
        const int o = c0 + lane;
        if (o < c1) {
          const int j = oj[o];
          rec[slot] = int4{op[o], j, lm_start[j] - c0, lm_start[j + 1] - lm_start[j]};
          suv[2 * slot] = uv[2 * (size_t)o]; suv[2 * slot + 1] = uv[2 * (size_t)o + 1];
        } else {
          rec[slot] = int4{-1, 0, lane, 0};
          suv[2 * slot] = 0.0; suv[2 * slot + 1] = 0.0;
        }
      }
    }
  }
  if (!tab.empty()) memcpy(h + o_tab, tab.data(), sizeof(uint16_t) * tab.size());
  if (!tab_off.empty()) memcpy(h + o_toff, tab_off.data(), sizeof(uint32_t) * tab_off.size());
  if (with_keys) { unsigned* k = reinterpret_cast<unsigned*>(h + o_key); for (int j = 0; j < npts; ++j) k[j] = (unsigned)ba->solve_lm_ids[(size_t)j]; }
  uint8_t* D = ba->d_arena;
  d.points = (double*)(D + o_pts); d.cand_points = (double*)(D + o_cpts);
  ba->cur_points = (double*)(D + o_pts); ba->cand_points = (double*)(D + o_cpts);
  ba->cur_poses = (double*)(D + o_p0); ba->cand_poses = (double*)(D + o_p1);
  d.rec = (const int4*)(D + o_rec); d.obs_uv = (const double*)(D + o_uv);
  d.tab = (const uint16_t*)(D + o_tab); d.tab_off = (const uint32_t*)(D + o_toff);
  d.tab_lds_words = (d.det && ba->tab_max_words > 0 && ba->tab_max_words <= 4096) ? ((ba->tab_max_words + 3) & ~3) : 0;
  d.lm_key = with_keys ? (const unsigned*)(D + o_key) : nullptr;
  memcpy(h + o_p0, poses7, sizeof(double) * 7 * (size_t)K);
  memcpy(h + o_p1, poses7, sizeof(double) * 7 * (size_t)K);
  ba->h_poses.assign(poses7, poses7 + 7 * (size_t)K);
  d.poses = (double*)(D + o_p0);
  d.cand_poses = (double*)(D + o_p1);
  ba->arena_bytes = (total + 15) & ~(size_t)15;
  ba->arena_dirty = true;
  ba->arena_partial = false;
  ba->arena_cpts_off = o_cpts; ba->arena_p0_off = o_p0; ba->arena_p1_off = o_p1;
  (void)has_empty_landmark; (void)st;
  if (d.det) { const int rcp = ba_ensure_partials(ba); if (rcp) return rcp; }
  return SVO_OK;
}

static int ba_upload(svo_ba* ba, int K, const double* poses7, int npts, const double* points3, int M,
                     const int32_t* op, const int32_t* oj, const double* uv) {
  const int rc = ba_upload_checked(ba, K, poses7, npts, points3, M, op, oj, uv);
  if (rc != SVO_OK) {
    ba->d.K = 0; ba->d.n = 0; ba->d.M = 0; ba->d.L = 0; ba->d.C = 0;
    ba->n_points = 0;
    ba->host_points_valid = false;
    ba->arena_dirty = false;
  }
  return rc;
}

static int ba_refresh_arena_image(svo_ba* ba) {
  svo_ctx* ctx = ba->ctx;
  const size_t npts = (size_t)ba->n_points;
  if (npts) {
    double* img = reinterpret_cast<double*>(ba->h_arena + ba->arena_pts_off);
    if (ba->host_points_valid) {
      const std::vector<int32_t>& lm = ba->u_lm_start;
      for (size_t j = 0; j < npts; ++j) {
        if (j + 1 < lm.size() && lm[j + 1] == lm[j]) continue;
        img[3 * j] = ba->h_out_points[3 * j]; img[3 * j + 1] = ba->h_out_points[3 * j + 1]; img[3 * j + 2] = ba->h_out_points[3 * j + 2];
      }
    } else {
      std::vector<double> tmp(3 * npts);
      SVO_HIP_CHECK(ctx, hipMemcpy(tmp.data(), ba->d.points, sizeof(double) * 3 * npts, hipMemcpyDeviceToHost));
      const std::vector<int32_t>& lm = ba->u_lm_start;
      for (size_t j = 0; j < npts; ++j) {
        if (j + 1 < lm.size() && lm[j + 1] == lm[j]) continue;
        img[3 * j] = tmp[3 * j]; img[3 * j + 1] = tmp[3 * j + 1]; img[3 * j + 2] = tmp[3 * j + 2];
      }
    }
    memcpy(ba->h_arena + ba->arena_cpts_off, img, sizeof(double) * 3 * npts);
  }
  memcpy(ba->h_arena + ba->arena_p0_off, ba->h_poses.data(), sizeof(double) * 7 * (size_t)ba->d.K);
  memcpy(ba->h_arena + ba->arena_p1_off, ba->h_poses.data(), sizeof(double) * 7 * (size_t)ba->d.K);
  uint8_t* D = ba->d_arena;
  ba->cur_points = (double*)(D + ba->arena_pts_off); ba->cand_points = (double*)(D + ba->arena_cpts_off);
  ba->cur_poses = (double*)(D + ba->arena_p0_off); ba->cand_poses = (double*)(D + ba->arena_p1_off);
  ba->d.points = ba->cur_points; ba->d.cand_points = ba->cand_points; ba->d.poses = ba->cur_poses; ba->d.cand_poses = ba->cand_poses;
  ba->arena_partial = false;
  ba->arena_dirty = true;
  return SVO_OK;
}

static int ba_flush_arena(svo_ba* ba) {
  if (ba->arena_partial) { const int rc = ba_refresh_arena_image(ba); if (rc) return rc; }
  if (!ba->arena_dirty) return SVO_OK;
  svo_ctx* ctx = ba->ctx;
  SVO_HIP_CHECK(ctx, hipMemcpyAsync(ba->d_arena, ba->h_arena, ba->arena_bytes, hipMemcpyHostToDevice, ba->stream));
  ba->arena_dirty = false;
  ba->upload_pending = true;
  return SVO_OK;
}

// ... 171 lines not shown
}
int ba_lm_admission_cost(int grid, size_t lds, int device, bool multi = false) {
  (void)ba_fused_budget(device);
  const int per_cu = ba_lm_per_cu(lds, multi);
  if (per_cu <= 0) return 1 << 30;
  if (per_cu >= g_fused_per_cu) return grid;
  return (grid * g_fused_per_cu + per_cu - 1) / per_cu;
}

inline FusedAdmission* ba_resident_admission(svo_ba* ba) { return &ba->res_admission; }

bool ba_device_lm_wanted() {
  static const char* e = getenv("SVO_BA_DEVICE_LM");
  if (e && *e) return atoi(e) != 0;
  return svo_throughput_mode();
}

int ba_lm_tab_words(const svo_ba* ba) { return std::max(64, (ba->tab_max_words + 63) & ~63); }
size_t ba_lm_lds_bytes(const svo_ba* ba, int kw) { return sizeof(double) * ba_lm_lds_doubles(ba->d.n, ba->d.K, ba_lm_tab_words(ba), kw); }

constexpr int LM_WAVE_CHUNKS_DEFAULT = 3;
int ba_lm_wave_chunks(const svo_ba* ba) {
  static const int env = [] {
    const char* e = getenv("SVO_BA_WAVE_CHUNKS");
    const int v = e && *e ? atoi(e) : LM_WAVE_CHUNKS_DEFAULT;
    return v < 1 ? 1 : (v > LM_MAX_WAVE_CHUNKS ? LM_MAX_WAVE_CHUNKS : v);
  }();
  if (ba->d.G > 1 || ba->d.C <= LM_CPW) return 1;
  return ba->lm_wave_chunks > 0 ? ba->lm_wave_chunks : env;
}
bool ba_lm_wave_contig() {
  static const bool contig = [] { const char* e = getenv("SVO_BA_WAVE_ORDER"); return e && e[0] == 'c'; }();
  return contig;
}

constexpr size_t LMC_LDS_BUDGET = 156 * 1024;
constexpr int LM_MAX_CHUNKS_GROUPED = 288;
constexpr int LMC_MAX_CHUNKS = 256;
int ba_lmc_tab_words(const svo_ba* ba) { return std::max(64, (ba->tab_max_words + 63) & ~63); }
int ba_lmc_waves(const svo_ba* ba) {
  static const int cap = [] { const char* e = getenv("SVO_BA_COMPACT_WAVES"); const int v = e ? atoi(e) : LMC_MAX_WAVES; return v < 1 ? 1 : (v > LMC_MAX_WAVES ? LMC_MAX_WAVES : v); }();
  const BaDev& d = ba->d;
  int nw = std::min(cap, std::max(1, d.C));
  while (nw >= 1 && sizeof(double) * ba_lmc_lds_doubles(d.n, d.K, ba_lmc_tab_words(ba), nw) > LMC_LDS_BUDGET) --nw;
  return nw;
}
bool ba_wants_compact(const svo_ba* ba) {
  if (ba->lm_penalty > 0) return true;
  if (ba->lm_form >= 0) return ba->lm_form == 1;
  static const int env = [] { const char* e = getenv("SVO_BA_FORM"); return !e || !*e ? -1 : (e[0] == 'c' ? 1 : (e[0] == 'w' ? 0 : -1)); }();
  return env == 1;
}

bool ba_device_lm_fill(svo_ba* ba, int* cost, size_t* lds_out, bool forced, bool compact = false, int* waves_out = nullptr) {
  BaDev& d = ba->d;
  if (!d.det || d.C <= 0 || !ba_zero_copy(ba) || !(forced || ba->device_lm == 1 || (ba->device_lm < 0 && ba_device_lm_wanted())) || !ba->h_lane) return false;
  size_t lds = 0;
  int nw = 0, kw = 1;
  if (compact) {
    if (d.C > LMC_MAX_CHUNKS || ba->tab_max_words > 4096) return false;
    nw = ba_lmc_waves(ba);
    if (nw < 1) return false;
    lds = sizeof(double) * ba_lmc_lds_doubles(d.n, d.K, ba_lmc_tab_words(ba), nw);
  } else {
  if (d.C > LM_MAX_CHUNKS_GROUPED || d.CPW != 1 || ba->tab_max_words > TAB_LDS_WORDS) return false;
  if (d.G > 1 && ba->device_lm != 1) return false;
  kw = ba_lm_wave_chunks(ba);
  lds = ba_lm_lds_bytes(ba, kw);
  if (lds > 120 * 1024) return false;
  }
  d.points = ba->cur_points; d.cand_points = ba->cand_points; d.poses = ba->cur_poses; d.cand_poses = ba->cand_poses;
  d.flag = nullptr;
  if (ba->arena_partial && ba_refresh_arena_image(ba)) return false;
  LmLane& L = *ba->h_lane;
  L.P = d;
  LmDevArgs& a = L.a;
  a.cnt = ba->d_lmc;
  a.arena_src = ba->arena_dirty ? ba->h_arena : nullptr;
  a.arena_dst = ba->d_arena; a.arena_bytes = ba->arena_bytes;
  a.points_a = ba->cur_points; a.points_b = ba->cand_points;
  a.export_points = ba->n_points ? ba->h_out_points : nullptr;
  a.store = d.lm_key ? ba->store : nullptr; a.store_mask = ba->store_mask;
  a.dev_res = ba->d_res;
  a.host_result = ba->h_result;
  a.host_flag = ba->h_flag; a.host_seq = ba->seq + 1;
  const bool fresh = ba->lm_counters_dirty || !ba->lm_have_base;
  a.base_arrive = fresh ? 0 : ba->lm_base;
  a.tab_words = compact ? ba_lmc_tab_words(ba) : ba_lm_tab_words(ba);
  a.wave_chunks = kw;
  a.wave_contig = ba_lm_wave_contig() ? 1 : 0;
  a.opt.max_iterations = ba->opt.max_iterations;
  a.opt.function_tolerance = ba->opt.function_tolerance; a.opt.gradient_tolerance = ba->opt.gradient_tolerance;
  a.opt.parameter_tolerance = ba->opt.parameter_tolerance; a.opt.initial_radius = ba->opt.initial_radius;
  a.opt.max_time_s = ba->opt.max_time_s;
  a.dbg = d.C <= 8192 ? ba->d_lmdbg : nullptr;
  {
    static const int every = [] { const char* e = getenv("SVO_BA_TEST_GIVEUP"); return e && *e ? atoi(e) : 0; }();
    a.test_giveup = (!compact && every > 0 && (++ba->wide_launches % every) == 0) ? 1 : 0;
  }
  *cost = compact ? 0 : ba_lm_admission_cost(ba_lm_blocks(d.C, kw), lds, ba->ctx->device, kw > 1);
  *lds_out = lds;
  if (waves_out) *waves_out = nw;
  return true;
}

int ba_device_lm_launch(svo_ba** bas, int n, hipStream_t st, bool forced, unsigned long long* launched_mask) {
  if (launched_mask) *launched_mask = 0;
  static const bool overflow = [] { const char* e = getenv("SVO_BA_OVERFLOW"); return e && *e && atoi(e) != 0; }();
  (void)g_group_lanes;
  bool to_compact[SVO_MAX_LANES] = {};
  int launched_total = 0;
  for (int i = 0; i < n && i < SVO_MAX_LANES; ++i) bas[i]->lm_inflight = false;
  for (int form = 0; form < 3; ++form) {
  const void* kernel = form == 0 ? (const void*)ba_lm_kernel : (form == 1 ? (const void*)ba_lm_grouped_kernel : (const void*)ba_lm_multi_kernel);
  LmLanePtrs ptrs;
  int launched = 0, max_c = 0;
  size_t max_lds = 0;
  svo_ba* took[SVO_MAX_LANES];
  int tidx[SVO_MAX_LANES];
  for (int i = 0; i < n && i < SVO_MAX_LANES; ++i) {
    svo_ba* ba = bas[i];
    int cost = 0;
    size_t lds = 0;
    if ((ba->d.G > 1 ? 1 : (ba_lm_wave_chunks(ba) > 1 ? 2 : 0)) != form) continue;
    if (ba_wants_compact(ba)) { to_compact[i] = true; continue; }
    if (!ba_device_lm_fill(ba, &cost, &lds, forced)) continue;
    if (lds > 32 * 1024 && hipFuncSetAttribute(kernel, hipFuncAttributeMaxDynamicSharedMemorySize, 120 * 1024) != hipSuccess) continue;
    bool admitted = ba_resident_admission(ba)->admit(cost, ba->ctx->device);
    if (!admitted && form == 2 && ba->lm_wave_chunks <= 0) {
      const int k0 = ba->h_lane->a.wave_chunks, dev = ba->ctx->device;
      const int per_cu0 = ba_lm_per_cu(lds, true);
      int blocks = ba_lm_blocks(ba->d.C, k0);
      for (int k = k0 + 1; k <= LM_MAX_WAVE_CHUNKS && !admitted; ++k) {
        if (ba_lm_blocks(ba->d.C, k) == blocks) continue;
        blocks = ba_lm_blocks(ba->d.C, k);
        const size_t lds_k = ba_lm_lds_bytes(ba, k);
        if (lds_k > 120 * 1024 || per_cu0 <= 0 || ba_lm_per_cu(lds_k, true) < per_cu0) break;
        if (lds_k > 32 * 1024 && hipFuncSetAttribute(kernel, hipFuncAttributeMaxDynamicSharedMemorySize, 120 * 1024) != hipSuccess) break;
        const int cost_k = ba_lm_admission_cost(blocks, lds_k, dev, true);
        admitted = ba_resident_admission(ba)->admit(cost_k, dev);
        if (admitted) { ba->h_lane->a.wave_chunks = k; lds = lds_k; }
      }
    }
    if (!admitted) { to_compact[i] = overflow; continue; }
    if (ba->lm_counters_dirty || !ba->lm_have_base) {
      if (hipMemsetAsync(ba->d_lmc, 0, LMC_WORDS * sizeof(unsigned), st) != hipSuccess) { ba_resident_admission(ba)->release(); continue; }
    }
    ba->lm_counters_dirty = false;
    ptrs.p[launched] = ba->h_lane;
    took[launched] = ba;
    tidx[launched] = i;
    max_c = std::max(max_c, ba_lm_blocks(ba->d.C, ba->h_lane->a.wave_chunks));
    max_lds = std::max(max_lds, lds);
    ++launched;
  }
  if (launched) {
    const auto t0 = now();
    {
      SvoProfScope prof(took[0]->ctx, SVO_PROF_BA_STEP, st);
      if (form == 1) hipLaunchKernelGGL(ba_lm_grouped_kernel, dim3(max_c, launched), dim3(128), max_lds, st, ptrs);
      else if (form == 2) hipLaunchKernelGGL(ba_lm_multi_kernel, dim3(max_c, launched), dim3(128), max_lds, st, ptrs);
      else hipLaunchKernelGGL(ba_lm_kernel, dim3(max_c, launched), dim3(128), max_lds, st, ptrs);
    }
    if (hipGetLastError() != hipSuccess) {
      for (int i = 0; i < launched; ++i) ba_resident_admission(took[i])->release();
      launched = 0;
    }
    for (int i = 0; i < launched; ++i) {
      svo_ba* ba = took[i];
      ++ba->seq;
      ba->lm_t0 = t0;
      if (ba->arena_dirty) ba->arena_partial = true;
      ba->arena_dirty = false;
      ba->lm_inflight = true; ba->lm_compact_inflight = false;
      ++ba->lm_k_solves[std::min(std::max(ba->h_lane->a.wave_chunks, 1), LM_MAX_WAVE_CHUNKS)];
      ba->lm_stream = st;
      ba->res_export = ba->h_lane->a.export_points != nullptr;
      if (launched_mask) *launched_mask |= 1ull << tidx[i];
    }
  }
  launched_total += launched;
  }
  const int launched = launched_total;
  int n_compact = 0;
  {
    LmLanePtrs cptrs;
    svo_ba* ctook[SVO_MAX_LANES];
    int cidx[SVO_MAX_LANES];
    int nw = LMC_MAX_WAVES;
    for (int i = 0; i < n && i < SVO_MAX_LANES; ++i) {
      svo_ba* ba = bas[i];
      if (!to_compact[i]) continue;
      int cost = 0, waves = 0;
      size_t lds = 0;
      if (!ba_device_lm_fill(ba, &cost, &lds, forced, true, &waves)) continue;
      cptrs.p[n_compact] = ba->h_lane; ctook[n_compact] = ba; cidx[n_compact] = i;
      nw = std::min(nw, waves);
      ++n_compact;
    }
    if (n_compact) {
      size_t clds = 0;
      for (int k = 0; k < n_compact; ++k)
        clds = std::max(clds, sizeof(double) * ba_lmc_lds_doubles(ctook[k]->d.n, ctook[k]->d.K, ctook[k]->h_lane->a.tab_words, nw));
      static bool attr_set = false;
      if (!attr_set) attr_set = hipFuncSetAttribute((const void*)ba_lm_compact_kernel, hipFuncAttributeMaxDynamicSharedMemorySize, (int)LMC_LDS_BUDGET) == hipSuccess;
      const auto t0 = now();
      bool ok = attr_set;
      if (ok) {
        SvoProfScope prof(ctook[0]->ctx, SVO_PROF_BA_STEP, st);
        hipLaunchKernelGGL(ba_lm_compact_kernel, dim3(1, n_compact), dim3(64 * nw), clds, st, cptrs);
        ok = hipGetLastError() == hipSuccess;
      }
      if (!ok) n_compact = 0;
      for (int k = 0; k < n_compact; ++k) {
        svo_ba* ba = ctook[k];
        ++ba->seq;
        ba->lm_t0 = t0;
        if (ba->arena_dirty) ba->arena_partial = true;
        ba->arena_dirty = false;
        ba->lm_inflight = true; ba->lm_compact_inflight = true;
      ++ba->lm_k_solves[0];
        ba->lm_stream = st;
        ba->res_export = ba->h_lane->a.export_points != nullptr;
        if (launched_mask) *launched_mask |= 1ull << cidx[k];
      }
    }
  }
  return launched + n_compact;
}

int ba_device_lm_end(svo_ba* ba, svo_ba_summary* sum) {
  if (!ba->lm_inflight) return SVO_ERR_INVALID;
  svo_ctx* ctx = ba->ctx;
  BaDev& d = ba->d;
  ba->lm_inflight = false;
  const bool was_compact = ba->lm_compact_inflight;
  ba->lm_compact_inflight = false;
  const int rc = ba_wait_flag(ba, ba->seq);
  ba_resident_admission(ba)->release();
  if (rc) {
    (void)hipStreamSynchronize(ba->lm_stream);
    if (getenv("SVO_BA_TRACE")) {
      unsigned c[LMC_WORDS] = {0};
      (void)hipMemcpy(c, ba->d_lmc, sizeof(c), hipMemcpyDeviceToHost);
      fprintf(stderr, "[svo ba] device solve gave up: chunks %d K %d delivered %u\n", d.C, d.K, c[LMC_ARRIVE]);
      if (ba->d_lmdbg && d.C <= 4096) {
        std::vector<unsigned> g(16 * (size_t)d.C);
        (void)hipMemcpy(g.data(), ba->d_lmdbg, sizeof(unsigned) * g.size(), hipMemcpyDeviceToHost);
        for (int b = 0; b < ba_lm_blocks(d.C, ba->h_lane->a.wave_chunks); ++b) {
          const unsigned* q = &g[16 * (size_t)b];
          if (b == 0 || memcmp(q, &g[0], 20) != 0)
            fprintf(stderr, "[svo ba]   workgroup %d: op %u state %u iterations %u need_linearize %u chain/bad %x arrive_total %u commands %u lin_calls %u\n", b, q[0], q[1],
                    q[2], q[3], q[4], q[5], q[6], q[7]);
        }
      }
    }
    if (!was_compact) ba->lm_counters_dirty = true;
    ba->host_points_valid = false;
    return rc;
  }
  const double* r = ba->h_result;
  if (!was_compact) { ba->lm_base = (unsigned)r[LMR_C_ARRIVE]; ba->lm_have_base = true; }
  memcpy(ba->h_poses.data(), r + LMR_DOUBLES, sizeof(double) * 7 * (size_t)d.K);
  if (r[LMR_SEL] != 0.0) { std::swap(ba->cur_points, ba->cand_points); std::swap(ba->cur_poses, ba->cand_poses); }
  ba->host_points_valid = ba->res_export;
  memset(&ba->stats, 0, sizeof(ba->stats));
  ba->stats.linearize_calls = (int)r[LMR_LINEARIZE_CALLS];
  ba->stats.step_calls = (int)r[LMR_STEP_CALLS];
  ba->stats.speculations = ba->stats.step_calls;
  ba->stats.speculation_hits = (int)r[LMR_NEXT_USED];
  ba->stats.single_exchange = (int)r[LMR_SAME_SWEEP];
  ba->lm_same += (long)r[LMR_SAME_SWEEP]; ba->lm_used += (long)r[LMR_NEXT_USED]; ba->lm_steps += (long)r[LMR_STEP_CALLS]; ba->lm_lins += (long)r[LMR_LINEARIZE_CALLS];
  if (was_compact) {
    for (int i = 0; i < 14; ++i) ba->lmc_tp[i] += r[LMR_TP0 + i];
    ba->lmc_n++; ba->lmc_iters += (long)r[LMR_ITERATIONS];
  } else {
    for (int i = 0; i < 14; ++i) ba->lm_tp[i] += r[LMR_TP0 + i];
    ba->lm_iters_wide += (long)r[LMR_ITERATIONS];
  }
  if (ba->d_lmdbg && getenv("SVO_TIMING")) {
    const int kw = ba->h_lane->a.wave_chunks, nb = ba_lm_blocks(d.C, kw);
    std::vector<unsigned> g(16 * (size_t)nb);
    if (hipMemcpy(g.data(), ba->d_lmdbg, sizeof(unsigned) * g.size(), hipMemcpyDeviceToHost) == hipSuccess) {
      for (int sl = 0; sl < 7; ++sl) {
        double mn = 1e300, mx = 0, sum = 0;
        for (int b = 0; b < nb; ++b) { const double v = g[16 * (size_t)b + 8 + sl]; mn = std::min(mn, v); mx = std::max(mx, v); sum += v; }
        ba->lm_wg_min[sl] += mn; ba->lm_wg_max[sl] += mx; ba->lm_wg_mean[sl] += sum / nb;
      }
      static int traced = 0;
      if (getenv("SVO_BA_TRACE_WG") && traced < 2 && r[LMR_ITERATIONS] >= 4) {
        ++traced;
        const int nU = (d.K - 1) * d.K / 2, F = d.K - 1;
        for (int b = 0; b < nb; ++b) {
          const int c = b * LM_CPW * (ba->h_lane->a.wave_contig ? kw : 1);
          const uint16_t* w = ba->u_tab.data() + ba->u_tab_off[(size_t)c];
          int ne = 0, longest = 0, plong = 0;
          for (int q = 0; q < nU; ++q) { const int len = w[q + 1] - w[q]; ne += len > 0; longest = std::max(longest, len); }
          for (int k = 0; k < F; ++k) plong = std::max(plong, (int)w[nU + 1 + k + 1] - (int)w[nU + 1 + k]);
          fprintf(stderr, "[svo ba wg] %2d: rest of pass A %.2f us/iteration, pass B %.2f | chunk %d: %d entries in %d blocks (longest list %d), longest pose list %d\n", b,
                  1e-2 * g[16 * (size_t)b + 8 + 3] / r[LMR_ITERATIONS], 1e-2 * g[16 * (size_t)b + 8 + 0] / r[LMR_ITERATIONS], c, (int)w[nU], ne, longest, plong);
        }
      }
    }
  }
  ba->lm_t_wait += r[LMR_T_WAIT]; ba->lm_t_ctl += r[LMR_T_CTL]; ba->lm_t_body += r[LMR_T_BODY]; ba->lm_t_total += r[LMR_T_TOTAL]; ba->lm_n++; ba->lm_iters += (long)r[LMR_ITERATIONS];
  if (sum) {
    sum->iterations = (int)r[LMR_ITERATIONS]; sum->successful_steps = (int)r[LMR_SUCCESSFUL]; sum->termination = (int)r[LMR_TERMINATION];
    sum->initial_cost = r[LMR_INITIAL_COST]; sum->final_cost = r[LMR_FINAL_COST];
    sum->solve_ms = ms_between(ba->lm_t0, now());
  }
  if (g_ba_cu_share != 32 && ba->lm_stream == ba->stream) SVO_HIP_CHECK(ctx, hipStreamSynchronize(ba->stream));
  d.points = ba->cur_points; d.cand_points = ba->cand_points; d.poses = ba->cur_poses; d.cand_poses = ba->cand_poses;
  return SVO_OK;
}

// ... 259 lines not shown
      hipLaunchKernelGGL(ba_backsub_kernel, dim3(grid), dim3(256), 0, st, d, 0.0, bs);
    }
    rc = allreduce(0, PAY2_SLOTS);
    if (!rc) rc = ba_launch_bulk_linearize(ba, 0.0, 0, nullptr, bs);
    if (!rc) rc = allreduce(PAY2_SLOTS, wire);
    if (rc) return rc;
    control(s);
    SVO_HIP_CHECK(ctx, hipGetLastError());
    ++enqueued;
    host_ms += ms_between(h0, now());
  }
  rc = wait_record(enqueued - 1);
  if (rc) return rc;
  (void)last_seen;
  const double* r = record(enqueued - 1);
  if (r[1] == 0.0) { ctx->err = "ba: the device-side step control did not terminate within its slot bound"; return SVO_ERR_NUMERIC; }
  SVO_HIP_CHECK(ctx, hipStreamSynchronize(st));
  memcpy(ba->h_poses.data(), r + BS_HEAD, sizeof(double) * 7 * (size_t)K);
  if (((int)r[7] & 1) != 0) { std::swap(ba->cur_points, ba->cand_points); std::swap(ba->cur_poses, ba->cand_poses); }
  ba->stats.linearize_calls = (int)r[8];
  ba->stats.step_calls = (int)r[9];
  ba->stats.speculations = (int)r[9];
  ba->stats.speculation_hits = (int)r[10];
  ba->stats.single_exchange = 0;
  ba->stats.collectives = collectives;
  ba->stats.device_control = 1;
  ba->stats.host_us = 1e3 * host_ms;
  if (getenv("SVO_TIMING") && tk_n)
    fprintf(stderr, "[svo ba] device-side step control, %d slots, thread 0 per slot (us since kernel entry): payloads loaded %.1f, step consumed %.1f, system built %.1f, "
                    "factored + solved %.1f, status written %.1f; inside the solve: panels %.1f, trailing updates + barriers %.1f, back substitution %.1f\n", tk_n, 1e-2 * tk_sum[0] / tk_n, 1e-2 * tk_sum[1] / tk_n, 1e-2 * tk_sum[2] / tk_n, 1e-2 * tk_sum[3] / tk_n, 1e-2 * tk_sum[4] / tk_n,
            1e-2 * tk_sum[5] / tk_n, 1e-2 * tk_sum[6] / tk_n, 1e-2 * tk_sum[7] / tk_n);
  if (sum) {
    sum->iterations = (int)r[2]; sum->successful_steps = (int)r[3]; sum->termination = (int)r[4];
    sum->initial_cost = r[5]; sum->final_cost = r[6];
    sum->solve_ms = ms_between(t_begin, now());
  }
  d.flag = nullptr;
  d.points = ba->cur_points; d.cand_points = ba->cand_points; d.poses = ba->cur_poses; d.cand_poses = ba->cand_poses;
  (void)nn;
  return SVO_OK;
}

static void ba_after_giveup(svo_ba* ba) {
  uint8_t* D = ba->d_arena;
  ba->cur_points = (double*)(D + ba->arena_pts_off); ba->cand_points = (double*)(D + ba->arena_cpts_off);
  ba->cur_poses = (double*)(D + ba->arena_p0_off); ba->cand_poses = (double*)(D + ba->arena_p1_off);
  ba->d.points = ba->cur_points; ba->d.cand_points = ba->cand_points; ba->d.poses = ba->cur_poses; ba->d.cand_poses = ba->cand_poses;
  ba->arena_partial = false;
  ba->arena_dirty = true;
  ba->host_points_valid = false;
  ba->upload_pending = false;
  ba->lm_penalty = 64;
  ++ba->fallbacks;
}

static int ba_lm(svo_ba* ba, svo_ba_summary* sum) {
  svo_ctx* ctx = ba->ctx;
  BaDev& d = ba->d;
  svo_lm_ops ops;
  ops.user = ba;
  ops.linearize = op_linearize;
  ops.step = op_step;
  ops.accept = op_accept;
  memset(&ba->stats, 0, sizeof(ba->stats));
  int fell_back = 0;
  if (ba_device_lm_launch(&ba, 1, ba->stream, false, nullptr) == 1) {
    const int rcd = ba_device_lm_end(ba, sum);
    d.flag = nullptr;
    if (rcd == SVO_OK) { if (ba->lm_penalty > 0) --ba->lm_penalty; return rcd; }
    ba_after_giveup(ba);
    fell_back = 1;
    if (ba_device_lm_launch(&ba, 1, ba->stream, true, nullptr) == 1) {
      const int rc2 = ba_device_lm_end(ba, sum);
      d.flag = nullptr;
      if (rc2 == SVO_OK) { ba->stats.fallbacks = 1; ctx->err.clear(); return rc2; }
      ba_after_giveup(ba);
    }
  }
  if (ba_bulk_control_wanted(ba)) return ba_lm_bulk_device(ba, sum);
  {
    const int rcf = ba_flush_arena(ba);
    if (rcf) return rcf;
  }
  ba->host_points_valid = false;
  const int rc = svo_lm_solve(d.K, ba->h_poses.data(), &ops, &ba->opt, sum, &ba->stats);
  ba->n_spec += ba->stats.speculations; ba->n_hit += ba->stats.speculation_hits;
  if (!ba->host_points_valid) SVO_HIP_CHECK(ctx, hipStreamSynchronize(ba->stream));
  d.flag = nullptr;
  d.points = ba->cur_points; d.cand_points = ba->cand_points; d.poses = ba->cur_poses; d.cand_poses = ba->cand_poses;
  if (fell_back && rc == SVO_OK) { ba->stats.fallbacks = 1; ctx->err.clear(); }
  return rc;
}

extern "C" int svo_ba_load_problem(svo_ba* ba, int n_poses, const double* poses7, int n_points, const double* points3,
                                   int n_obs, const int32_t* obs_pose, const int32_t* obs_point, const double* obs_uv) {
  if (!ba) return SVO_ERR_INVALID;
  svo_use_device(ba->ctx);
  SVO_REQUIRE(ba->ctx, poses7 && (n_points == 0 || points3) && (n_obs == 0 || (obs_pose && obs_point && obs_uv)),
              "ba_load_problem: null buffer");
  return ba_upload(ba, n_poses, poses7, n_points, points3, n_obs, obs_pose, obs_point, obs_uv);
}

extern "C" int svo_ba_solve_problem(svo_ba* ba, svo_ba_summary* summary) {
  if (!ba) return SVO_ERR_INVALID;
  svo_use_device(ba->ctx);
  SVO_REQUIRE(ba->ctx, ba->d.K >= 1, "ba_solve_problem: no problem loaded");
  const int rc = ba_lm(ba, summary);
  if (!rc) ba->upload_pending = false;
  return rc;
}

extern "C" int svo_ba_solve_problems(svo_ba** bas, int n, svo_ba_summary* summaries) {
  if (!bas || n < 1 || n > SVO_MAX_LANES) return SVO_ERR_INVALID;
  for (int i = 0; i < n; ++i) if (!bas[i] || bas[i]->d.K < 1) return SVO_ERR_INVALID;
  svo_use_device(bas[0]->ctx);
  for (int i = 0; i < n; ++i) {
    memset(&bas[i]->stats, 0, sizeof(bas[i]->stats));
    if (summaries) memset(&summaries[i], 0, sizeof(summaries[i]));
    if (bas[i]->stream != bas[0]->stream) SVO_HIP_CHECK(bas[i]->ctx, hipStreamSynchronize(bas[i]->stream));
  }
  unsigned long long mask = 0;
  const int launched = ba_device_lm_launch(bas, n, bas[0]->stream, true, &mask);
  int first_error = 0;
  for (int i = 0; i < n; ++i) {
    svo_ba* ba = bas[i];
    svo_ba_summary* sum = summaries ? &summaries[i] : nullptr;
    int rc;
    if ((mask >> i) & 1ull) {
      rc = ba_device_lm_end(ba, sum); ba->d.flag = nullptr;
      if (rc == SVO_OK) { if (ba->lm_penalty > 0) --ba->lm_penalty; }
      else {
        ba_after_giveup(ba);
        rc = ba_lm(ba, sum);
        if (rc == SVO_OK) { ba->stats.fallbacks = 1; ba->ctx->err.clear(); }
      }
    } else rc = ba_lm(ba, sum);
    if (!rc) ba->upload_pending = false;
    else if (!first_error) first_error = rc;
  }
  return first_error ? first_error : launched;
}

extern "C" int svo_ba_read_problem(svo_ba* ba, double* poses7, double* points3) {
  if (!ba) return SVO_ERR_INVALID;
  svo_ctx* ctx = ba->ctx;
  if (poses7) memcpy(poses7, ba->h_poses.data(), sizeof(double) * 7 * (size_t)ba->d.K);
  if (points3 && ba->n_points && ba->host_points_valid) {
    memcpy(points3, ba->h_out_points, sizeof(double) * 3 * (size_t)ba->n_points);
    const double* in = reinterpret_cast<const double*>(ba->h_arena + ba->arena_pts_off);
    const std::vector<int32_t>& lm = ba->u_lm_start;
    for (int j = 0; j < ba->n_points && (size_t)j + 1 < lm.size(); ++j)
      if (lm[j + 1] == lm[j]) { points3[3 * j] = in[3 * j]; points3[3 * j + 1] = in[3 * j + 1]; points3[3 * j + 2] = in[3 * j + 2]; }
  } else if (points3 && ba->n_points && ba->arena_dirty) {
    memcpy(points3, ba->h_arena + ba->arena_pts_off, sizeof(double) * 3 * (size_t)ba->n_points);
  } else if (points3 && ba->n_points) {
    const size_t bytes = sizeof(double) * 3 * (size_t)ba->n_points;
    void* stage = bytes <= ba->arena_cap ? (void*)ba->h_arena : (void*)points3;
    SVO_HIP_CHECK(ctx, hipMemcpyAsync(stage, ba->d.points, bytes, hipMemcpyDeviceToHost, ba->stream));
    SVO_HIP_CHECK(ctx, hipStreamSynchronize(ba->stream));
    ba->upload_pending = false;
    if (stage != (void*)points3) memcpy(points3, stage, bytes);
  }
  return SVO_OK;
}

extern "C" int svo_ba_add_keyframe(svo_ba* ba, const double* pose7, const int64_t* tracked_ids, const float* tracked_xy,
                                   int n_tracked, const float* new_xy, const float* new_xyz, int n_new, int64_t* new_ids,
                                   int* n_new_out) {
  if (!ba) return SVO_ERR_INVALID;
  svo_ctx* ctx = ba->ctx;
  SVO_REQUIRE(ctx, pose7 && n_tracked >= 0 && n_new >= 0 && n_new_out, "ba_add_keyframe: bad arguments");
  SVO_REQUIRE(ctx, (n_tracked == 0 || (tracked_ids && tracked_xy)) && (n_new == 0 || (new_xy && new_xyz && new_ids)),
              "ba_add_keyframe: null buffer");
  svo_ba::PoseVar pv;
  memcpy(pv.pose, pose7, sizeof(pv.pose));
  const int64_t nfeat = (int64_t)(ba->feat_pos.size() / 3);
  for (int i = 0; i < n_tracked; ++i) {
    SVO_REQUIRE(ctx, tracked_ids[i] >= 0 && tracked_ids[i] < nfeat, "ba_add_keyframe: unknown feature id");
    pv.obs.push_back({tracked_xy[2 * i], tracked_xy[2 * i + 1], tracked_ids[i]});
  }
  const int maxf = ba->opt.max_features;
  const int max_new = n_tracked > maxf ? 0 : maxf - n_tracked;
  const int keep = n_new > max_new ? max_new : n_new;
// ... 96 lines not shown
    for (size_t i = 1; i < o.size() && ascending; ++i) ascending = o[i - 1].id <= o[i].id;
  }
  auto emit = [&](int k, const svo_ba::Obs& o) {
    if (lm_ids.empty() || lm_ids.back() != o.id) {
      lm_ids.push_back(o.id);
      for (int a = 0; a < 3; ++a) points.push_back(ba->feat_pos[3 * o.id + a]);
    }
    op.push_back(k); oj.push_back((int32_t)lm_ids.size() - 1);
    uv.push_back(o.u); uv.push_back(o.v);
  };
  if (ascending && K <= 64) {
    const svo_ba::Obs* cur[64];
    const svo_ba::Obs* end[64];
    for (int k = 0; k < K; ++k) { const auto& o = ba->window[k].obs; cur[k] = o.data(); end[k] = o.data() + o.size(); }
    for (size_t done = 0; done < total; ++done) {
      int best = -1;
      int64_t best_id = 0;
      for (int k = 0; k < K; ++k)
        if (cur[k] != end[k] && (best < 0 || cur[k]->id < best_id)) { best = k; best_id = cur[k]->id; }
      emit(best, *cur[best]++);
    }
  } else {
    struct Flat { int k; const svo_ba::Obs* o; };
    std::vector<Flat> flat;
    flat.reserve(total);
    for (int k = 0; k < K; ++k)
      for (const auto& o : ba->window[k].obs) flat.push_back({k, &o});
    std::stable_sort(flat.begin(), flat.end(), [](const Flat& a, const Flat& b) { return a.o->id < b.o->id; });
    for (const Flat& f : flat) emit(f.k, *f.o);
  }
  const auto tu0 = std::chrono::steady_clock::now();
  ba->t_prep += std::chrono::duration<double, std::milli>(tu0 - tp0).count();
  ba->upload_has_ids = true;
  int rc = ba_upload(ba, K, poses.data(), (int)lm_ids.size(), points.data(), (int)op.size(), op.data(), oj.data(), uv.data());
  ba->upload_has_ids = false;
  if (rc) return rc;
  ba->t_upload += std::chrono::duration<double, std::milli>(std::chrono::steady_clock::now() - tu0).count();
  return SVO_OK;
}

int svo_ba_solve_launch(svo_ba** bas, int n, void* stream, unsigned long long* launched_mask) {
  if (launched_mask) *launched_mask = 0;
  if (!bas || n < 1) return 0;
  svo_use_device(bas[0]->ctx);
  return ba_device_lm_launch(bas, n, stream ? (hipStream_t)stream : bas[0]->stream, true, launched_mask);
}

int svo_ba_solve_poll(svo_ba* ba) {
  if (!ba || !ba->lm_inflight) return 1;
  const int v = __atomic_load_n(ba->h_flag, __ATOMIC_ACQUIRE);
  return (v == ba->seq || (v == -ba->seq && ba->seq != 0)) ? 1 : 0;
}

int svo_ba_solve_holds_budget(svo_ba* ba) { return ba && ba->lm_inflight && !ba->lm_compact_inflight ? 1 : 0; }

int svo_ba_solve_finish(svo_ba* ba, svo_ba_summary* summary) {
  if (!ba) return SVO_ERR_INVALID;
  svo_use_device(ba->ctx);
  if (summary) memset(summary, 0, sizeof(*summary));
  const auto tu0 = std::chrono::steady_clock::now();
  const int K = ba->d.K;
  std::vector<double>& poses = ba->s_poses; std::vector<double>& points = ba->s_points;
  std::vector<int64_t>& lm_ids = ba->solve_lm_ids;
  int rc;
  const bool on_device = ba->lm_inflight;
  bool on_device_ok = on_device;
  if (ba->lm_inflight) {
    rc = ba_device_lm_end(ba, summary); ba->d.flag = nullptr;
    if (rc == SVO_OK) { if (ba->lm_penalty > 0) --ba->lm_penalty; }
    else {
      ba_after_giveup(ba);
      rc = ba_lm(ba, summary);
      if (rc == SVO_OK) { ba->stats.fallbacks = 1; ba->ctx->err.clear(); }
      on_device_ok = false;
    }
  } else rc = ba_lm(ba, summary);
  if (!rc) ba->upload_pending = false;
  ba->t_total += std::chrono::duration<double, std::milli>(std::chrono::steady_clock::now() - tu0).count();
  ba->n_solves++;
  if (rc) return rc;
  if (summary && on_device) {
    const double its = summary->iterations + 1;
    ba->acc_flops += its * ba->flops_iter; ba->acc_bytes += its * ba->bytes_iter; ba->acc_solves += 1; ba->acc_iters += summary->iterations;
  }
  const auto tr0 = std::chrono::steady_clock::now();
  std::vector<double>& out_pts = ba->s_out_pts;
  out_pts.resize(points.size());
  rc = svo_ba_read_problem(ba, poses.data(), out_pts.data());
  if (rc) return rc;
  for (int k = 0; k < K; ++k) memcpy(ba->window[k].pose, &poses[7 * k], 7 * sizeof(double));
  for (size_t l = 0; l < lm_ids.size(); ++l)
    for (int a = 0; a < 3; ++a) ba->feat_pos[3 * lm_ids[l] + a] = out_pts[3 * l + a];
  ba->new_frame_added = false;
  if (ba->store && !on_device_ok && !lm_ids.empty()) {
    rc = ba_store_scatter(ba, lm_ids, out_pts);
    if (rc) return rc;
  }
  ba->t_read += std::chrono::duration<double, std::milli>(std::chrono::steady_clock::now() - tr0).count();
  return SVO_OK;
}

void svo_ba_work(svo_ba* ba, double* out4, int reset) {
  out4[0] = ba->acc_flops; out4[1] = ba->acc_bytes; out4[2] = ba->acc_solves; out4[3] = ba->acc_iters;
  if (reset) ba->acc_flops = ba->acc_bytes = ba->acc_solves = ba->acc_iters = 0;
}

extern "C" int svo_ba_solve(svo_ba* ba, svo_ba_summary* summary) {
  if (!ba) return SVO_ERR_INVALID;
  if (summary) memset(summary, 0, sizeof(*summary));
  const int rc = svo_ba_solve_prepare(ba);
  if (rc == 1) return SVO_OK;
  if (rc) return rc;
  return svo_ba_solve_finish(ba, summary);
}
```

### stereo_vo_amd/csrc/group_kernels.h

```cpp
#ifndef SVO_GROUP_KERNELS_H_
#define SVO_GROUP_KERNELS_H_
#include "kernels.h"

#include "chain_math.h"
#include "xcd_map.h"

struct SvoLkLane {
  const uint8_t* pyr_prev; const uint8_t* pyr_next;
  const uint8_t* l0_prev; const uint8_t* l0_next;
  const float* xy; const float* init_xy; const long long* ids;
  int n;
  float* fwd; uint8_t* keep; float* parallax;
  float* kept_xy; float* init_dst; long long* ids_dst;
  float* host_xy; long long* host_ids; int* host_n; float* host_av;
  unsigned* arrive; unsigned arrive_target;
  int* word; int seq;
};
struct SvoLkLanes { int w, h; SvoXcdMap map; SvoLkLane lane[SVO_MAX_LANES]; };
int svo_kg_track(svo_ctx* ctx, hipStream_t st, const SvoLkLanes& lanes, int n_lanes, int grid_x);

struct SvoPnpLane {
  const long long* ids; const float4* store; unsigned store_mask;
  const float* xy; int n; double f, cx, cy; double q0[4], t0[3]; double thr2, confidence; int iterations;
  int launched;
  double* hyp_pose; int* hyp_count; unsigned long long* hyp_mask; int mask_words;
  double* out_pose; int* inliers; int* n_inliers; float* inlier_xy;
  double* host_pose; int* host_inliers; int* host_nin; int* host_best; int* host_bad;
  unsigned* arrive; unsigned arrive_target;
  int* word; int seq;
  SvoChainRec* chain; float prev_rvec[3], prev_tvec[3]; float cam_f, cam_cx, cam_cy, cam_b;
};
struct SvoPnpLanes { SvoPnpLane lane[SVO_MAX_LANES]; };
int svo_kg_pnp(svo_ctx* ctx, hipStream_t st, const SvoPnpLanes& lanes, int n_lanes);
int svo_kg_pnp_workgroups(int launched);
int svo_kg_pnp_first(int iterations);
int svo_pnp_update_num_iters(double p, double ep, int model_points, int max_iters);
int svo_pnp_model_points();

struct SvoStereoTriLane {
  const uint8_t* left; const uint8_t* right; const float* xy; const int* n_dev; int n_max; float* disp; SvoMat4 M;
  const float* trk; int n_trk; float min_d;
  float* kept_xy; float* xyz; int* n_kept; SvoPublish pub;
  const SvoChainRec* chain;
};
struct SvoStereoTriLanes { int w, h, stride, ndisp, block; SvoXcdMap map; SvoStereoTriLane lane[SVO_MAX_LANES]; };
int svo_kg_stereo_triangulate(svo_ctx* ctx, hipStream_t st, const SvoStereoTriLanes& lanes, int n_lanes, int grid_x);

int svo_ba_solve_prepare(svo_ba* ba);
int svo_ba_solve_launch(svo_ba** bas, int n, void* stream, unsigned long long* launched_mask);
int svo_ba_solve_poll(svo_ba* ba);
int svo_ba_solve_holds_budget(svo_ba* ba);
int svo_ba_solve_finish(svo_ba* ba, svo_ba_summary* summary);
void svo_ba_work(svo_ba* ba, double* out4, int reset);
void svo_ba_note_group_lanes(int delta);
int svo_ba_use_stream(svo_ba* ba, void* stream);
int svo_ba_attach_store(svo_ba* ba, float4* store, unsigned mask);

#endif
```

### stereo_vo_amd/host/group.cpp

```cpp
#include <math.h>
#include <stdio.h>
#include <stdlib.h>
#include <string.h>

#include <sched.h>

#include <algorithm>
#include <atomic>
#include <chrono>
#include <condition_variable>
#include <deque>
#include <mutex>
#include <thread>
#include <vector>

#include "chain_math.h"
#include "det_trig.h"
#include "group_kernels.h"
#include "group_lines.h"
#include "ref_constants.h"
#include "svo.h"

namespace {

enum LaneState { L_IDLE = 0, L_TRACK_WAIT, L_NEED_SOLVE, L_PNP_WAIT, L_TRI_WAIT, L_DONE };
enum BaState { BA_NONE = 0, BA_ASSEMBLING, BA_READY, BA_INFLIGHT, BA_HOST_SOLVING, BA_HOST_DONE };
enum Word { W_TRACK = 0, W_PNP, W_TRI, W_COUNT };
enum Counter { C_LK = 0, C_PNP, C_TRI, C_COUNT };
enum Stat { ST_TRACK = 0, ST_PNP, ST_HOST_US, ST_TRI, ST_SOLVE, ST_FRONT_END, ST_COUNT };

struct Lane {
  int lk_line = 0, chain_line = 0;
  float* d_xy[2] = {nullptr, nullptr}; float* d_init[2] = {nullptr, nullptr}; long long* d_ids[2] = {nullptr, nullptr};
  float* d_fwd = nullptr; float* d_par = nullptr; uint8_t* d_keep = nullptr;
  float* h_xy[2] = {nullptr, nullptr}; long long* h_ids[2] = {nullptr, nullptr};
  float* h_kf_xy = nullptr; long long* h_kf_ids = nullptr;
  int* h_n = nullptr; float* h_av = nullptr;
  int cur = 0, n = 0, n_initial = 0;
  bool from_host = false;
  const uint8_t* last_pyr = nullptr;
  const uint8_t* last_l0 = nullptr;
  uint8_t* d_own_pyr = nullptr;
  float4* d_store = nullptr; unsigned store_mask = 0;
  double* d_hyp_pose = nullptr; int* d_hyp_count = nullptr; unsigned long long* d_hyp_mask = nullptr;
  double* d_out = nullptr; int* d_nin = nullptr; int* d_inl = nullptr; float* d_trk_xy = nullptr;
  bool pnp_all = false;
  int* h_best = nullptr; int* h_bad = nullptr; double* h_out = nullptr; int* h_nin = nullptr; int* h_inl = nullptr;
  float* d_disp = nullptr;
  int* h_tri_cnt = nullptr; float* h_tri_xy = nullptr; float* h_tri_xyz = nullptr;
  int* words = nullptr;
  int seq[W_COUNT] = {};
  unsigned* d_arrive = nullptr;
  unsigned arrive_total[C_COUNT] = {0, 0, 0};
  svo_ba* ba = nullptr;
  std::atomic<int> ba_state{BA_NONE};
  svo_ba_summary ba_summary{};
  int ba_rc = 0;
  int ba_launch = 0, ba_line = 0;
  unsigned long long ba_ready_seq = 0;
  bool has_keyframe = false;
  double solved_pose[7] = {1, 0, 0, 0, 0, 0, 0};
  int last_iterations = 0;
  float rvec[3] = {0, 0, 0}, tvec[3] = {0, 0, 0};
  int state = L_IDLE;
  bool queued = false;
  int frame = 0;
  int pending_from = -1;
  bool first_keyframe = false;
  SvoChainRec* d_chain = nullptr;
  double t_q = 0.0;
  bool fused = false;
  int m_tracked = 0, num_inliers = 0, best = -1;
  float rmat[9], quat[4];
  std::vector<long long> kf_tracked_ids; std::vector<float> kf_tracked_xy;
  std::vector<long long> ids64; std::vector<int64_t> new_ids;
};

struct Pool {
  std::vector<std::thread> th;
  std::mutex mu;
  std::condition_variable cv;
  std::deque<std::pair<Lane*, int>> jobs;
  bool quit = false;
  int device = 0;
  void start(int n, int dev) {
    device = dev;
    for (int i = 0; i < n; ++i) th.emplace_back([this] { run(); });
  }
  void post(Lane* l, int what) {
    { std::lock_guard<std::mutex> g(mu); jobs.emplace_back(l, what); }
    cv.notify_one();
  }
  void run() {
    (void)hipSetDevice(device);
    for (;;) {
      std::pair<Lane*, int> j;
      {
        std::unique_lock<std::mutex> lk(mu);
        cv.wait(lk, [this] { return quit || !jobs.empty(); });
        if (quit && jobs.empty()) return;
        j = jobs.front(); jobs.pop_front();
      }
      Lane* l = j.first;
      if (j.second == 0) {
        l->ba_rc = svo_ba_solve_prepare(l->ba);
        l->ba_state.store(BA_READY, std::memory_order_release);
      } else {
        l->ba_rc = svo_ba_solve_finish(l->ba, &l->ba_summary);
        l->ba_state.store(BA_HOST_DONE, std::memory_order_release);
      }
    }
  }
// ... 34 lines not shown
  uint8_t* h_stage[2][2] = {{nullptr, nullptr}, {nullptr, nullptr}};
  uint8_t* d_stage[2][2] = {{nullptr, nullptr}, {nullptr, nullptr}};
  hipStream_t st_copy = nullptr;
  hipEvent_t ev_up[2] = {nullptr, nullptr};
  int up_batch[2] = {0, 0};
  std::vector<SvoRectModel*> rect_models;
  SvoRectModel* lane_rect[SVO_MAX_LANES] = {};
  uint8_t* d_rect[2] = {nullptr, nullptr};
  SvoKfClouds* kfc = nullptr;
  bool lane_cloud[SVO_MAX_LANES] = {};
};

namespace {

int fail(svo_pipeline_group* g, const char* what, hipError_t e) {
  g->ctx->err = std::string("pipeline group: ") + what + ": " + hipGetErrorString(e);
  return SVO_ERR_HIP;
}

template <typename T>
int dev_alloc(svo_pipeline_group* g, T** p, size_t count) {
  const hipError_t e = hipMalloc((void**)p, sizeof(T) * (count ? count : 1));
  if (e != hipSuccess) return fail(g, "hipMalloc", e);
  g->dev_allocs.push_back(*p);
  return SVO_OK;
}

int word_ready(const Lane* l, int w) { return __atomic_load_n(&l->words[16 * w], __ATOMIC_ACQUIRE) == l->seq[w]; }

SvoPublish make_pub(Lane* l, int w, int counter, int nblocks) {
  SvoPublish p;
  p.word = &l->words[16 * w];
  p.seq = ++l->seq[w];
  if (counter >= 0) {
    l->arrive_total[counter] += (unsigned)nblocks;
    p.arrive = l->d_arrive + 16 * counter;
    p.target = l->arrive_total[counter];
  }
  return p;
}

void fill_pending(Lane* l, svo_frame_result* res, int upto) {
  if (l->pending_from < 0) return;
  for (int j = l->pending_from; j < upto; ++j) {
    memcpy(res[j].pose7, l->solved_pose, sizeof(res[j].pose7));
    if (j == l->pending_from && res[j].is_keyframe) res[j].ba_iterations = l->last_iterations;
  }
  l->pending_from = -1;
}

int finish_solve(svo_pipeline_group* g, Lane* l) {
  const int st = l->ba_state.load(std::memory_order_acquire);
  l->ba_ready_seq = 0;
  if (st == BA_NONE) return SVO_OK;
  int rc = SVO_OK;
  const auto tf0 = std::chrono::steady_clock::now();
  if (st == BA_INFLIGHT) rc = svo_ba_solve_finish(l->ba, &l->ba_summary);
  else rc = l->ba_rc;
  if (g->timing) g->t_finish += std::chrono::duration<double, std::nano>(std::chrono::steady_clock::now() - tf0).count();
  l->ba_state.store(BA_NONE, std::memory_order_release);
  if (rc) return rc;
  l->last_iterations = l->ba_summary.iterations;
  double p[7];
  if ((rc = svo_ba_get_pose(l->ba, -1, p))) return rc;
  for (int i = 0; i < 7; ++i) l->solved_pose[i] = (double)(float)p[i];
  (void)g;
  return SVO_OK;
}

void quiesce_after_error(svo_pipeline_group* g) {
  for (int i = 0; i < svo_pipeline_group::MAX_LINES; ++i) {
    if (g->st_lk[i]) (void)hipStreamSynchronize(g->st_lk[i]);
    if (g->st_chain[i]) (void)hipStreamSynchronize(g->st_chain[i]);
    if (g->st_ba[i]) (void)hipStreamSynchronize(g->st_ba[i]);
  }
  for (Lane* l : g->lanes) {
    (void)hipMemset(l->d_arrive, 0, sizeof(unsigned) * 16 * C_COUNT);
    for (int c = 0; c < C_COUNT; ++c) l->arrive_total[c] = 0;
    for (int w = 0; w < W_COUNT; ++w) { l->seq[w] = 0; l->words[16 * w] = 0; }
    if (l->h_bad) *l->h_bad = 0;
    l->fused = false; l->pnp_all = false;
    l->queued = false;
  }
  (void)hipDeviceSynchronize();
}

}

extern "C" void svo_pipeline_group_destroy(svo_pipeline_group* g) {
  if (!g) return;
  (void)hipSetDevice(g->ctx->device);
  g->pool.stop();
  for (Lane* l : g->lanes) {
    if (l->ba_state.load() == BA_INFLIGHT) { svo_ba_summary s; (void)svo_ba_solve_finish(l->ba, &s); }
  }
  if (g->timing && g->n_kf)
    fprintf(stderr, "[svo group] %d lanes, %ld keyframes; group thread per keyframe (us): get_world_points %.1f, add_keyframe %.1f, join + write-back of the solve %.1f\n",
            g->n_lanes, g->n_kf, 1e-3 * g->t_get_points / g->n_kf, 1e-3 * g->t_add_keyframe / g->n_kf, 1e-3 * g->t_finish / g->n_kf);
  (void)hipStreamSynchronize(g->ctx->stream);
  for (Lane* l : g->lanes) { if (l->ba) { svo_ba_destroy(l->ba); l->ba = nullptr; } }
  if (g->counted_lanes) svo_ba_note_group_lanes(-g->counted_lanes);
  for (int i = 0; i < svo_pipeline_group::MAX_LINES; ++i) {
    if (g->st_lk[i] && g->st_lk[i] != g->ctx->stream) { (void)hipStreamSynchronize(g->st_lk[i]); (void)hipStreamDestroy(g->st_lk[i]); }
    if (g->st_chain[i]) { (void)hipStreamSynchronize(g->st_chain[i]); (void)hipStreamDestroy(g->st_chain[i]); }
    if (g->st_ba[i]) { (void)hipStreamSynchronize(g->st_ba[i]); (void)hipStreamDestroy(g->st_ba[i]); }
  }
// ... 91 lines not shown
    }
    if (!rc) rc = dev_alloc(g, &l->d_fwd, 2 * mf);
    if (!rc) rc = dev_alloc(g, &l->d_par, mf);
    if (!rc) rc = dev_alloc(g, &l->d_keep, mf);
    {
      size_t cap = 1, keyframes = 256;
      if (const char* e = getenv("SVO_GROUP_STORE_KEYFRAMES")) keyframes = (size_t)std::max(1, atoi(e));
      while (cap < keyframes * mf) cap <<= 1;
      l->store_mask = (unsigned)(cap - 1);
      if (!rc) rc = dev_alloc(g, &l->d_store, cap);
      if (!rc) chk(hipMemset(l->d_store, 0xFF, sizeof(float4) * cap), "hipMemset");
    }
    if (!rc) rc = dev_alloc(g, &l->d_hyp_pose, 7 * (size_t)g->pnp_iterations);
    if (!rc) rc = dev_alloc(g, &l->d_hyp_count, (size_t)g->pnp_iterations);
    if (!rc) rc = dev_alloc(g, &l->d_hyp_mask, (size_t)g->pnp_iterations * words);
    if (!rc) rc = dev_alloc(g, &l->d_out, 8);
    if (!rc) rc = dev_alloc(g, &l->d_nin, 16);
    if (!rc) rc = dev_alloc(g, &l->d_inl, mf);
    if (!rc) rc = dev_alloc(g, &l->d_trk_xy, 2 * mf);
    if (!rc) rc = dev_alloc(g, &l->d_chain, 1);
    if (!rc) rc = dev_alloc(g, &l->d_disp, mc);
    if (!rc) rc = dev_alloc(g, &l->d_own_pyr, g->pyr_stride);
    if (!rc) rc = dev_alloc(g, &l->d_arrive, 16 * C_COUNT);
    if (!rc) chk(hipMemset(l->d_arrive, 0, sizeof(unsigned) * 16 * C_COUNT), "hipMemset");
    if (rc) break;
    const size_t f2 = sizeof(float) * 2 * mf, i8 = sizeof(long long) * mf;
    size_t off = 0;
    auto take = [&](size_t bytes) { const size_t o = off; off = (off + bytes + 127) & ~(size_t)127; return o; };
    const size_t o_xy0 = take(f2), o_xy1 = take(f2), o_id0 = take(i8), o_id1 = take(i8), o_kxy = take(f2), o_kid = take(i8), o_n = take(64),
                 o_cnt = take(64), o_out = take(64), o_nin = take(64),
                 o_inl = take(sizeof(int) * mf), o_tc = take(64), o_txy = take(sizeof(float) * 2 * mc), o_txyz = take(sizeof(float) * 3 * mc),
                 o_words = take(64 * W_COUNT);
    void* hp = nullptr;
    chk(hipHostMalloc(&hp, off, hipHostMallocDefault), "hipHostMalloc");
    if (rc) break;
    g->pin_allocs.push_back(hp);
    memset(hp, 0, off);
    char* h = (char*)hp;
    l->h_xy[0] = (float*)(h + o_xy0); l->h_xy[1] = (float*)(h + o_xy1); l->h_ids[0] = (long long*)(h + o_id0); l->h_ids[1] = (long long*)(h + o_id1);
    l->h_kf_xy = (float*)(h + o_kxy); l->h_kf_ids = (long long*)(h + o_kid);
    l->h_n = (int*)(h + o_n); l->h_av = (float*)(h + o_n + 16);
    l->h_best = (int*)(h + o_cnt); l->h_bad = (int*)(h + o_cnt) + 1; l->h_out = (double*)(h + o_out); l->h_nin = (int*)(h + o_nin);
    l->h_inl = (int*)(h + o_inl); l->h_tri_cnt = (int*)(h + o_tc); l->h_tri_xy = (float*)(h + o_txy); l->h_tri_xyz = (float*)(h + o_txyz);
    l->words = (int*)(h + o_words);
    svo_ba_options opt;
    svo_ba_default_options(&opt);
    opt.max_features = p->max_features;
    opt.max_iterations = p->ba_max_iterations;
    opt.max_time_s = p->ba_max_time_s;
    const int max_obs = (p->window_size + 1) * p->max_features + 64;
    rc = svo_ba_create(ctx, &l->ba, p->window_size, &p->cam, &opt, max_obs, max_obs);
    if (!rc) rc = svo_ba_attach_store(l->ba, l->d_store, l->store_mask);
    if (!rc) rc = svo_ba_use_stream(l->ba, g->st_ba[li % g->n_ba]);
  }
  if (rc) { svo_pipeline_group_destroy(g); return rc; }
  {
    const char* e = getenv("SVO_GROUP_WORKERS");
    int nw = e ? atoi(e) : (n_lanes < 8 ? n_lanes : 8);
    if (nw < 1) nw = 1;
    if (nw > 8) nw = 8;
    g->pool.start(nw, ctx->device);
  }
  (void)hipDeviceSynchronize();
  g->counted_lanes = n_lanes;
  svo_ba_note_group_lanes(n_lanes);
  *out = g;
  return SVO_OK;
}

extern "C" int svo_pipeline_group_reset(svo_pipeline_group* g) {
  if (!g) return SVO_ERR_INVALID;
  (void)hipSetDevice(g->ctx->device);
  int rc_join = SVO_OK;
  for (Lane* l : g->lanes) {
    const int rcf = finish_solve(g, l);
    if (rcf && !rc_join) rc_join = rcf;
    svo_ba_reset(l->ba);
    l->has_keyframe = false; l->n = l->n_initial = 0; l->from_host = false; l->last_pyr = nullptr; l->last_l0 = nullptr; l->cur = 0;
    l->rvec[0] = l->rvec[1] = l->rvec[2] = l->tvec[0] = l->tvec[1] = l->tvec[2] = 0.f;
    l->state = L_IDLE; l->queued = false; l->pending_from = -1; l->last_iterations = 0;
    const double id7[7] = {1, 0, 0, 0, 0, 0, 0};
    memcpy(l->solved_pose, id7, sizeof(id7));
    if (l->h_bad) *l->h_bad = 0;
    l->fused = false; l->pnp_all = false;
    if (l->d_store && hipMemsetAsync(l->d_store, 0xFF, sizeof(float4) * ((size_t)l->store_mask + 1), g->ctx->stream) != hipSuccess && !rc_join) rc_join = SVO_ERR_HIP;
  }
  if (hipStreamSynchronize(g->ctx->stream) != hipSuccess && !rc_join) rc_join = SVO_ERR_HIP;
  if (rc_join) { quiesce_after_error(g); return rc_join; }
  return SVO_OK;
}

extern "C" int svo_pipeline_group_lanes(const svo_pipeline_group* g) { return g ? g->n_lanes : 0; }

extern "C" int svo_pipeline_group_get_tracked(svo_pipeline_group* g, int lane, int64_t* ids, float* xy, int capacity, int* n) {
  if (!g || !n || lane < 0 || lane >= g->n_lanes) return SVO_ERR_INVALID;
  const Lane* l = g->lanes[lane];
  *n = l->n;
  const float* sx = l->from_host ? l->h_kf_xy : l->h_xy[l->cur];
  const long long* si = l->from_host ? l->h_kf_ids : l->h_ids[l->cur];
  for (int i = 0; i < l->n && i < capacity; ++i) {
    if (ids) ids[i] = (int64_t)si[i];
    if (xy) { xy[2 * i] = sx[2 * i]; xy[2 * i + 1] = sx[2 * i + 1]; }
  }
  return SVO_OK;
}

extern "C" int svo_pipeline_group_solve_work(svo_pipeline_group* g, double* out4, int reset) {
  if (!g || !out4) return SVO_ERR_INVALID;
  out4[0] = out4[1] = out4[2] = out4[3] = 0.0;
  for (Lane* l : g->lanes) {
    double w[4];
    svo_ba_work(l->ba, w, reset);
    for (int i = 0; i < 4; ++i) out4[i] += w[i];
  }
  return SVO_OK;
}

extern "C" int svo_pipeline_group_solve_forms(svo_pipeline_group* g, long* counts, int n, long* gave_up) {
  if (!g || !counts || n < 1) return SVO_ERR_INVALID;
  std::vector<long> c((size_t)n);
  for (int i = 0; i < n; ++i) counts[i] = 0;
  if (gave_up) *gave_up = 0;
  for (Lane* l : g->lanes) {
    long gu = 0;
    const int rc = svo_ba_solve_forms(l->ba, c.data(), n, &gu);
    if (rc) return rc;
    for (int i = 0; i < n; ++i) counts[i] += c[(size_t)i];
    if (gave_up) *gave_up += gu;
  }
  return SVO_OK;
}

extern "C" int svo_pipeline_group_last_stats(const svo_pipeline_group* g, long* launches6, long* lanes6) {
  if (!g || !launches6 || !lanes6) return SVO_ERR_INVALID;
  static_assert(ST_COUNT == 6, "svo_pipeline_group_last_stats returns six slots");
  for (int i = 0; i < ST_COUNT; ++i) { launches6[i] = g->launches[i]; lanes6[i] = g->lanes_carried[i]; }
  return SVO_OK;
}

namespace {
bool trace_enabled() { static const bool on = getenv("SVO_GROUP_TRACE") != nullptr; return on; }
bool chain_fused_enabled() { static const bool on = [] { const char* e = getenv("SVO_GROUP_CHAIN_FUSED"); return !(e && *e && atoi(e) == 0); }(); return on; }
bool host_solves_only() { static const bool on = [] { const char* e = getenv("SVO_GROUP_HOST_SOLVES"); return e && *e && atoi(e) != 0; }(); return on; }

struct Batch {
  using Clock = std::chrono::steady_clock;
  struct Ev { double us; int lane; const char* what; int arg; };
  static constexpr int MAX_LINES = svo_pipeline_group::MAX_LINES;

  svo_pipeline_group* const g;
  svo_ctx* const ctx;
  const uint8_t* const* const lbase;
  const uint8_t* const* const rbase;
  const int batch;
  svo_frame_result* const results;
// ... 371 lines not shown
    x.xy = DET(li, i); x.n_dev = nullptr;
    x.trk = nullptr; x.n_trk = 0; x.min_d = 0.f;
    x.chain = nullptr;
    if (l->fused) {
      x.chain = l->d_chain; x.trk = l->d_trk_xy; x.min_d = g->prm.min_feature_distance;
    } else if (!l->first_keyframe) {
      x.trk = l->d_trk_xy; x.n_trk = l->num_inliers; x.min_d = g->prm.min_feature_distance;
      if (x.n_trk <= 0) x.trk = nullptr;
    }
    x.left = IMG(lbase, li, i); x.right = IMG(rbase, li, i);
    x.n_max = n_det; x.disp = l->d_disp;
    const float I9[9] = {1, 0, 0, 0, 1, 0, 0, 0, 1}, zero3[3] = {0, 0, 0};
    const bool posed = !l->fused && !l->first_keyframe;
    svo_chain_matrix_from_R(posed ? l->rmat : I9, posed ? l->tvec : zero3, g->K[0], g->K[2], g->K[5], (float)g->prm.cam.baseline, x.M.m);
    x.kept_xy = l->h_tri_xy; x.xyz = l->h_tri_xyz; x.n_kept = l->h_tri_cnt;
    x.pub = make_pub(l, W_TRI, C_TRI, workgroups);
    l->state = L_TRI_WAIT;
    l->queued = false;
  }

  void launch_tri(int line, const std::vector<int>& t_now) {
    SvoStereoTriLanes t;
    t.w = W; t.h = H; t.stride = W; t.ndisp = svo_ref::STEREO_NUM_DISPARITIES; t.block = svo_ref::STEREO_BLOCK_SIZE;
    int kt = 0, gxt = 1;
    t.map.per_chunk = 0; t.map.total = 0; t.map.chunks = 0;
    int counts[SVO_MAX_LANES], j = 0;
    for (int li : t_now) {
      const int n_det = hc[li * batch + g->lanes[li]->frame];
      gxt = std::max(gxt, n_det);
      counts[j++] = n_det;
    }
    if (g->xcd_map_tri) svo_xcd_map_fill(t.map, counts, j, g->xcd_chunks);
    for (int li : t_now) {
      Lane* l = g->lanes[li];
      fill_tri_lane(l, li, t.lane[kt++], t.map.per_chunk > 0 ? std::max(1, hc[li * batch + l->frame]) : gxt);
    }
    if ((error = svo_kg_stereo_triangulate(ctx, g->st_chain[line], t, kt, gxt))) return;
    for (int li : t_now) EV(li, "tri_launch", kt);
    count(ST_TRI, kt);
  }

  void launch_chains() {
    for (int line = 0; line < g->n_chain && !error; ++line) {
      if (chain_busy[line]) continue;
      const std::vector<int> h_now = ripe(q_pnp, line, g->n_chain, L_TRACK_WAIT) ? svo_line_take(q_pnp, line, g->n_chain) : std::vector<int>();
      std::vector<int> t_now = svo_line_take(q_tri, line, g->n_chain);
      for (int li : h_now) g->lanes[li]->chain_line = line;
      for (int li : t_now) g->lanes[li]->chain_line = line;
      if (!h_now.empty()) launch_pnp(line, h_now, t_now);
      if (!error && !t_now.empty()) launch_tri(line, t_now);
    }
  }

  static bool solve_came_back(Lane* l) {
    const int bs = l->ba_state.load(std::memory_order_acquire);
    return (bs == BA_INFLIGHT && svo_ba_solve_poll(l->ba)) || bs == BA_HOST_DONE;
  }
  bool any_solve_in_flight(bool holding_budget) const {
    bool any = false;
    for (const Lane* l : g->lanes)
      any |= l->ba_state.load(std::memory_order_acquire) == BA_INFLIGHT && (!holding_budget || svo_ba_solve_holds_budget(l->ba));
    return any;
  }

  void join_finished_solves() {
    for (int li = 0; li < S && !error; ++li) {
      Lane* l = g->lanes[li];
      if (l->state == L_NEED_SOLVE || !solve_came_back(l)) continue;
      EV(li, "solve_joined", l->frame);
      error = finish_solve(g, l);
      progressed = true;
    }
  }

  void solves_departed(const int* lanes, int n, unsigned long long taken, int line, int carried, const char* what) {
    ++g->ba_launch_id;
    if (carried > 0) count(ST_SOLVE, carried);
    for (int k = 0; k < n; ++k) {
      if (!((taken >> k) & 1ull)) continue;
      Lane* l = g->lanes[lanes[k]];
      EV(lanes[k], what, carried);
      l->ba_launch = g->ba_launch_id; l->ba_line = line; l->ba_ready_seq = 0;
      l->ba_state.store(BA_INFLIGHT, std::memory_order_release);
    }
  }
  static int first_not_taken(const int* lanes, int n, unsigned long long taken) {
    for (int k = 0; k < n; ++k) if (!((taken >> k) & 1ull)) return lanes[k];
    return -1;
  }

  void collect_ready_solves() {
    q_ba.clear();
    for (int li = 0; li < S; ++li) {
      Lane* l = g->lanes[li];
      if (l->ba_state.load(std::memory_order_acquire) != BA_READY) continue;
      q_ba.push_back(li);
      if (!l->ba_ready_seq) l->ba_ready_seq = ++g->ba_ready_counter;
    }
    std::sort(q_ba.begin(), q_ba.end(), [&](int a, int b) {
      const Lane* la = g->lanes[a]; const Lane* lb = g->lanes[b];
      return svo_solve_before(la->state == L_NEED_SOLVE, la->ba_ready_seq, lb->state == L_NEED_SOLVE, lb->ba_ready_seq);
    });
    for (int i = 0; i < MAX_LINES; ++i) ba_line_busy[i] = false;
    for (const Lane* l : g->lanes)
      if (l->ba_state.load(std::memory_order_acquire) == BA_INFLIGHT && !svo_ba_solve_poll(l->ba)) ba_line_busy[l->ba_line] = true;
  }
  int free_solve_line(int from, int to) const {
    for (int i = from; i < to; ++i) if (!ba_line_busy[i]) return i;
    return -1;
  }

  int launch_refused_compact(const int* cand, svo_ba* const* bas, int n, unsigned long long mask, int not_taken) {
    const int cline = free_solve_line(g->n_ba, g->n_ba + g->n_cmp);
    if (cline < 0) return not_taken;
    svo_ba* cb[SVO_MAX_LANES];
    int cl[SVO_MAX_LANES], nc = 0;
    for (int k = 0; k < n; ++k) if (!((mask >> k) & 1ull)) { cb[nc] = bas[k]; cl[nc++] = cand[k]; (void)svo_ba_set_solve_form(bas[k], 1); }
    unsigned long long cmask = 0;
    const int went = svo_ba_solve_launch(cb, nc, g->st_ba[cline], &cmask);
    for (int k = 0; k < nc; ++k) (void)svo_ba_set_solve_form(cb[k], -1);
    if (went <= 0) return not_taken;
    solves_departed(cl, nc, cmask, cline, went, "ba_launch_compact");
    return first_not_taken(cl, nc, cmask);
  }

  void launch_solves() {
    collect_ready_solves();
    const int free_line = free_solve_line(0, g->n_ba);
    if (q_ba.empty() || free_line < 0) return;
    svo_ba* bas[SVO_MAX_LANES];
    int cand[SVO_MAX_LANES], n = 0;
    for (int li : q_ba) {
      Lane* l = g->lanes[li];
      if (l->ba_rc == 1) { l->ba_ready_seq = 0; l->ba_state.store(BA_NONE, std::memory_order_release); continue; }
      if (l->ba_rc) { error = l->ba_rc; return; }
      bas[n] = l->ba;
      cand[n++] = li;
    }
    if (!n) return;
    unsigned long long mask = 0;
    const bool host_solves = host_solves_only();
    const int launched = host_solves ? 0 : svo_ba_solve_launch(bas, n, g->st_ba[free_line], &mask);
    solves_departed(cand, n, mask, free_line, launched, "ba_launch");
    int not_taken = first_not_taken(cand, n, mask);
    if (not_taken < 0) return;
    if (g->n_cmp > 0 && !host_solves && !any_solve_in_flight(true)) not_taken = launch_refused_compact(cand, bas, n, mask, not_taken);
    if (not_taken < 0 || any_solve_in_flight(false)) return;
    Lane* l = g->lanes[not_taken];
    l->ba_ready_seq = 0;
    l->ba_state.store(BA_HOST_SOLVING, std::memory_order_release);
    g->pool.post(l, 1);
    progressed = true;
  }

  bool idle_or_report() {
    if (progressed) {
      idle_spins = 0;
      last_progress = Clock::now();
      busy_us += std::chrono::duration<double, std::micro>(last_progress - t_pass).count();
      return true;
    }
    __builtin_ia32_pause();
    if (++idle_spins > 2000u && (idle_spins & 255u) == 0) sched_yield();
    if ((idle_spins & 0xFFFFu) != 0) return true;
    if (std::chrono::duration<double>(Clock::now() - last_progress).count() <= 5.0) return true;
    std::string msg = "pipeline group: no progress for 5 s; lanes (state/frame/solve):";
    for (const Lane* l : g->lanes) {
      char b[64];
      snprintf(b, sizeof(b), " %d/%d/%d%s", l->state, l->frame, l->ba_state.load(), l->queued ? "q" : "");
      msg += b;
    }
    ctx->err = msg;
// ... 331 lines not shown
```

### stereo_vo_amd/host/group_lines.h

```cpp
#ifndef SVO_GROUP_LINES_H_
#define SVO_GROUP_LINES_H_
#include <vector>

inline bool svo_line_carries(int lane, int line, int n_lines) { return lane % n_lines == line; }

inline std::vector<int> svo_line_take(std::vector<int>& q, int line, int n_lines) {
  std::vector<int> mine;
  for (size_t k = 0; k < q.size();) {
    if (svo_line_carries(q[k], line, n_lines)) { mine.push_back(q[k]); q.erase(q.begin() + (long)k); } else ++k;
  }
  return mine;
}

template <typename QueuedSince, typename Near>
inline bool svo_line_ripe(const std::vector<int>& q, int n_lanes, int line, int n_lines, double now_us, double gather_us,
                          QueuedSince queued_since, Near near) {
  if (gather_us <= 0.0) return true;
  int mine = 0;
  bool waited = false;
  for (int li : q) if (svo_line_carries(li, line, n_lines)) { ++mine; waited = waited || now_us - queued_since(li) >= gather_us; }
  if (!mine || waited) return true;
  for (int li = 0; li < n_lanes; ++li) if (svo_line_carries(li, line, n_lines) && near(li)) return false;
  return true;
}

inline bool svo_solve_before(bool a_waits, unsigned long long a_ready_seq, bool b_waits, unsigned long long b_ready_seq) {
  if (a_waits != b_waits) return a_waits;
  return a_ready_seq < b_ready_seq;
}
#endif
```

Baseline: 13420 frames/s.

## Let device LM solves yield after N iterations and resume on freed lines

Adds cooperative yielding to the persistent device Levenberg-Marquardt bundle-adjustment kernel. After a configurable number of iterations (default 8) the solver saves its scalars, scaling and poses to a device record, reports a 'continues' termination, and later resumes from that record. The host scheduler puts yielded solves back in the ready queue, ranked ahead of fresh ones, so a long solve no longer holds a solve line while other lanes wait. In exchange it pays extra launches, state save and restore, and a relinearization on each resume, and adds complexity to the solve state machine.

```diff
diff --git a/include/svo.h b/include/svo.h
--- a/include/svo.h
+++ b/include/svo.h
@@ -271,6 +271,7 @@
 int svo_ba_wave_chunks_limit(void);
 int svo_ba_set_wave_chunks(svo_ba* ba, int k);
 int svo_ba_solve_forms(svo_ba* ba, long* counts, int n, long* gave_up);
+int svo_ba_set_yield_iterations(svo_ba* ba, int n);
 int svo_ba_solve_problem(svo_ba* ba, svo_ba_summary* summary);
 int svo_ba_solve_problems(svo_ba** bas, int n, svo_ba_summary* summaries);
 int svo_ba_read_problem(svo_ba* ba, double* poses7, double* points3);
@@ -343,6 +344,7 @@
 int svo_pipeline_group_last_stats(const svo_pipeline_group* g, long* launches6, long* lanes6);
 int svo_pipeline_group_solve_work(svo_pipeline_group* g, double* out4, int reset);
 int svo_pipeline_group_solve_forms(svo_pipeline_group* g, long* counts, int n, long* gave_up);
+int svo_pipeline_group_set_solve_yield(svo_pipeline_group* g, int n);
 
 int svo_draw_track(const uint8_t* gray, int width, int height, int row_stride, const float* from_xy,
                    const float* to_xy, int n, uint8_t* rgb);
diff --git a/stereo_vo_amd/api.py b/stereo_vo_amd/api.py
--- a/stereo_vo_amd/api.py
+++ b/stereo_vo_amd/api.py
@@ -292,13 +292,13 @@
     "svo_pnp_ransac",
     "svo_ba_default_options", "svo_ba_create", "svo_ba_destroy", "svo_ba_reset", "svo_ba_add_keyframe", "svo_ba_solve",
     "svo_ba_get_pose", "svo_ba_window_count", "svo_ba_get_points", "svo_ba_load_problem",
-    "svo_ba_set_allreduce", "svo_ba_set_device_lm", "svo_ba_set_bulk_control", "svo_ba_set_solve_form", "svo_ba_wave_chunks_limit", "svo_ba_set_wave_chunks", "svo_ba_solve_forms", "svo_ba_solve_problem", "svo_ba_solve_problems", "svo_ba_read_problem", "svo_ba_set_comm", "svo_ba_last_stats", "svo_lm_solve", "svo_lm_decide_step",
+    "svo_ba_set_allreduce", "svo_ba_set_device_lm", "svo_ba_set_bulk_control", "svo_ba_set_solve_form", "svo_ba_wave_chunks_limit", "svo_ba_set_wave_chunks", "svo_ba_set_yield_iterations", "svo_ba_solve_forms", "svo_ba_solve_problem", "svo_ba_solve_problems", "svo_ba_read_problem", "svo_ba_set_comm", "svo_ba_last_stats", "svo_lm_solve", "svo_lm_decide_step",
     "svo_rccl_unique_id", "svo_rccl_comm_create", "svo_rccl_comm_destroy",
     "svo_pipeline_default_params", "svo_pipeline_create", "svo_pipeline_destroy", "svo_pipeline_reset",
     "svo_pipeline_process_batch_dev", "svo_pipeline_process_batch", "svo_pipeline_get_tracked",
     "svo_pipeline_group_create", "svo_pipeline_group_destroy", "svo_pipeline_group_reset", "svo_pipeline_group_lanes",
     "svo_pipeline_group_process_batch_dev", "svo_pipeline_group_get_tracked", "svo_pipeline_group_last_stats",
-    "svo_pipeline_group_solve_work", "svo_pipeline_group_solve_forms", "svo_pipeline_group_staging", "svo_pipeline_group_upload", "svo_pipeline_group_process_uploaded", "svo_pipeline_group_process_batch",
+    "svo_pipeline_group_solve_work", "svo_pipeline_group_solve_forms", "svo_pipeline_group_set_solve_yield", "svo_pipeline_group_staging", "svo_pipeline_group_upload", "svo_pipeline_group_process_uploaded", "svo_pipeline_group_process_batch",
     "svo_synth_default_params", "svo_synth_render", "svo_synth_pose",
     "svo_image_read_gray", "svo_kitti_read_poses", "svo_ate_rmse", "svo_kitti_run", "svo_cholesky_solve", "svo_cholesky_solve_dev", "svo_draw_track", "svo_pipeline_draw_track",
     "svo_rectify_eye_from_camera_info", "svo_rectify_build_map", "svo_rectify_remap", "svo_rectify_remap_batch_dev",
@@ -844,6 +844,15 @@
         self.ctx._chk(self.L.svo_ba_solve_forms(self.h, out, n, C.byref(gu)), "svo_ba_solve_forms")
         return list(out), gu.value
 
+    def set_yield_iterations(self, n):
+        self.ctx._chk(self.L.svo_ba_set_yield_iterations(self.h, int(n)), "svo_ba_set_yield_iterations")
+
+    def solve_resumes(self):
+        n = self.L.svo_ba_wave_chunks_limit() + 2
+        out = (C.c_long * n)()
+        self.ctx._chk(self.L.svo_ba_solve_forms(self.h, out, n, None), "svo_ba_solve_forms")
+        return out[n - 1]
+
     @staticmethod
     def solve_problems(bas):
         n = len(bas)
@@ -1118,6 +1127,15 @@
         self.ctx._chk(self.L.svo_pipeline_group_solve_forms(self.h, out, n, C.byref(gu)), "svo_pipeline_group_solve_forms")
         return list(out), gu.value
 
+    def set_solve_yield(self, n):
+        self.ctx._chk(self.L.svo_pipeline_group_set_solve_yield(self.h, int(n)), "svo_pipeline_group_set_solve_yield")
+
+    def solve_resumes(self):
+        n = self.L.svo_ba_wave_chunks_limit() + 2
+        out = (C.c_long * n)()
+        self.ctx._chk(self.L.svo_pipeline_group_solve_forms(self.h, out, n, None), "svo_pipeline_group_solve_forms")
+        return out[n - 1]
+
     def last_stats(self):
         a, b = (C.c_long * 6)(), (C.c_long * 6)()
         self.ctx._chk(self.L.svo_pipeline_group_last_stats(self.h, a, b), "svo_pipeline_group_last_stats")
diff --git a/stereo_vo_amd/csrc/ba.hip b/stereo_vo_amd/csrc/ba.hip
--- a/stereo_vo_amd/csrc/ba.hip
+++ b/stereo_vo_amd/csrc/ba.hip
@@ -1536,18 +1536,26 @@
   int test_giveup;
   int wave_chunks;
   int wave_contig;
+  int yield_after;
+  int resume;
+  double* yield_rec;
 };
+enum { YR_RADIUS = 0, YR_DF, YR_COST, YR_INITIAL_COST, YR_MCC, YR_ITERATIONS, YR_SUCCESSFUL, YR_SEL, YR_SATURATED, YR_NEED_LINEARIZE, YR_OP_COUNT,
+       YR_LIN_CALLS, YR_STEP_CALLS, YR_SAME_SWEEPS, YR_NEXT_USED, YR_SCALARS = 16 };
+constexpr double LM_TERMINATION_CONTINUES = 2.0;
+__host__ __device__ static inline unsigned long long lm_yield_tag(int host_seq) { return (1ull << 61) | (unsigned long long)(unsigned)host_seq; }
 enum { LMC_ARRIVE = 0, LMC_WORDS = 16 };
 enum { LMR_ITERATIONS = 0, LMR_SUCCESSFUL, LMR_TERMINATION, LMR_INITIAL_COST, LMR_FINAL_COST, LMR_LINEARIZE_CALLS, LMR_STEP_CALLS, LMR_SEL,
        LMR_T_WAIT, LMR_T_CTL, LMR_T_BODY, LMR_T_TOTAL, LMR_SAME_SWEEP, LMR_NEXT_USED, LMR_C_ARRIVE, LMR_TP0, LMR_DOUBLES = LMR_TP0 + 14 };
-enum { LMS_START = 0, LMS_FIRST, LMS_RELIN, LMS_STEP, LMS_ACCEPT_RELIN, LMS_DELIVER };
-enum { LMOP_EXIT = 0, LMOP_LINEARIZE, LMOP_ITERATE, LMOP_DELIVER, LMOP_ABORT };
+enum { LMS_START = 0, LMS_FIRST, LMS_RELIN, LMS_STEP, LMS_ACCEPT_RELIN, LMS_DELIVER, LMS_RESUME };
+enum { LMOP_EXIT = 0, LMOP_LINEARIZE, LMOP_ITERATE, LMOP_DELIVER, LMOP_ABORT, LMOP_YIELD };
 
 struct LmDevState {
   double radius, df, cost, initial_cost, mcc, spec;
   double elapsed;
   double pay2[6];
   int iterations, successful, termination, need_linearize, state, sel, chain, first, saturated;
+  int iter_base;
   unsigned arrive_total;
   int lin_calls, step_calls, same_sweeps, next_used;
   int go, act, use_next, accepted, relin, bad, flag;
@@ -1657,11 +1665,11 @@
   double* cCand = sStep + nn;
   double* cPose = cCand + 7 * K;
   const LmDevOpt& opt = a.opt;
-  enum { ACT_NONE = 0, ACT_LOOPTOP, ACT_FINISH, ACT_ACCEPT_TAIL, ACT_SOLVE };
+  enum { ACT_NONE = 0, ACT_LOOPTOP, ACT_FINISH, ACT_ACCEPT_TAIL, ACT_SOLVE, ACT_YIELD };
   int act = ACT_NONE;
   auto issue = [&](int op) {
     if (tid == 0) {
-      if (op == LMOP_DELIVER) cs.arrive_total += (unsigned)grid;
+      if (op == LMOP_DELIVER || op == LMOP_YIELD) cs.arrive_total += (unsigned)grid;
       cs.tag = (1ull << 62) | ((unsigned long long)(unsigned)a.host_seq << 20) | (unsigned long long)(++cs.op_count & 0xFFFFFu);
       const long long tn = (long long)wall_clock64();
       cs.t_ctl += tn - cs.t_mark; cs.t_mark = tn;
@@ -1683,9 +1691,33 @@
       cs.lin_calls = 1; cs.step_calls = 0; cs.same_sweeps = 0; cs.next_used = 0; cs.bad = 0; cs.op_count = 0; cs.tag = 0;
       cs.t_wait = cs.t_ctl = cs.t_body = 0;
       for (int i = 0; i < 14; ++i) cs.tp[i] = 0;
-      cs.state = LMS_FIRST; cs.first = 1;
+      cs.state = LMS_FIRST; cs.first = 1; cs.iter_base = 0;
     }
     __syncthreads();
+    if constexpr (MULTI) {
+      if (a.resume) {
+        const unsigned long long rt = lm_yield_tag(a.resume);
+        double* sc = cTerm;
+        for (int i = tid; i < YR_SCALARS + n + 7 * K; i += nt) {
+          double v = 0.0;
+          if (!granule_wait(a.yield_rec, i, rt, v)) cs.bad = 1;
+          if (i < YR_SCALARS) sc[i] = v; else if (i < YR_SCALARS + n) cSc[i - YR_SCALARS] = v; else cPose[i - YR_SCALARS - n] = v;
+        }
+        __syncthreads();
+        if (cs.bad) return LMOP_ABORT;
+        if (tid == 0) {
+          cs.radius = sc[YR_RADIUS]; cs.df = sc[YR_DF]; cs.cost = sc[YR_COST]; cs.initial_cost = sc[YR_INITIAL_COST]; cs.mcc = sc[YR_MCC];
+          cs.iterations = (int)sc[YR_ITERATIONS]; cs.successful = (int)sc[YR_SUCCESSFUL]; cs.sel = (int)sc[YR_SEL]; cs.saturated = (int)sc[YR_SATURATED];
+          cs.op_count = (unsigned)sc[YR_OP_COUNT];
+          cs.lin_calls = (int)sc[YR_LIN_CALLS] + (sc[YR_NEED_LINEARIZE] != 0.0 ? 1 : 0);
+          cs.step_calls = (int)sc[YR_STEP_CALLS]; cs.same_sweeps = (int)sc[YR_SAME_SWEEPS]; cs.next_used = (int)sc[YR_NEXT_USED];
+          cs.iter_base = cs.iterations;
+          cs.state = LMS_RESUME; cs.first = 0;
+        }
+        __syncthreads();
+        return issue(LMOP_LINEARIZE);
+      }
+    }
     {
       const ptrdiff_t shift = a.arena_src ? reinterpret_cast<const char*>(a.arena_src) - reinterpret_cast<const char*>(a.arena_dst) : 0;
       for (int i = tid; i < 7 * K; i += nt) cPose[i] = sys_load(&P.poses[i], shift);
@@ -1791,6 +1823,8 @@
     } else if (st == LMS_RELIN) {
       if (tid == 0) cs.need_linearize = 0;
       act = ACT_SOLVE;
+    } else if (MULTI && st == LMS_RESUME) {
+      act = ACT_LOOPTOP;
     } else {
       act = ACT_ACCEPT_TAIL;
     }
@@ -1819,6 +1853,7 @@
         if (cs.iterations >= opt.max_iterations) { cs.termination = 1; a_ = ACT_FINISH; }
         else if (opt.max_time_s > 0 && cs.elapsed >= opt.max_time_s) { cs.termination = 1; a_ = ACT_FINISH; }
         else if (cs.radius <= LM_MIN_RADIUS) { cs.termination = 0; a_ = ACT_FINISH; }
+        else if (MULTI && a.yield_after > 0 && !(opt.max_time_s > 0) && cs.iterations - cs.iter_base >= a.yield_after) a_ = ACT_YIELD;
         else {
           ++cs.iterations;
           if (cs.need_linearize) { ++cs.lin_calls; cs.state = LMS_RELIN; a_ = ACT_NONE; }
@@ -1830,13 +1865,29 @@
       __syncthreads();
       if (act == ACT_NONE) return issue(LMOP_LINEARIZE);
     }
-    if (act == ACT_FINISH) {
+    if (act == ACT_FINISH || (MULTI && act == ACT_YIELD)) {
+      const bool yield = MULTI && act == ACT_YIELD;
       if (tid == 0) cs.state = LMS_DELIVER;
       if (blockIdx.x == 0) {
+        if constexpr (MULTI) {
+          if (yield) {
+            const unsigned long long rt = lm_yield_tag(a.host_seq);
+            double* yr = a.yield_rec;
+            if (tid == 0) {
+              const double sc[YR_SCALARS] = {cs.radius, cs.df, cs.cost, cs.initial_cost, cs.mcc, (double)cs.iterations, (double)cs.successful, (double)cs.sel,
+                                             (double)cs.saturated, (double)cs.need_linearize, (double)cs.op_count, (double)cs.lin_calls, (double)cs.step_calls,
+                                             (double)cs.same_sweeps, (double)cs.next_used, 0.0};
+#pragma unroll
+              for (int i = 0; i < YR_SCALARS; ++i) granule_store(&yr[2 * i], sc[i], rt);
+            }
+            for (int i = tid; i < n; i += nt) granule_store(&yr[2 * (YR_SCALARS + i)], cSc[i], rt);
+            for (int i = tid; i < 7 * K; i += nt) granule_store(&yr[2 * (YR_SCALARS + n + i)], cPose[i], rt);
+          }
+        }
         if (tid == 0) {
           double* r = a.host_result;
           pay_store(&r[LMR_ITERATIONS], (double)cs.iterations); pay_store(&r[LMR_SUCCESSFUL], (double)cs.successful);
-          pay_store(&r[LMR_TERMINATION], (double)cs.termination); pay_store(&r[LMR_INITIAL_COST], cs.initial_cost);
+          pay_store(&r[LMR_TERMINATION], yield ? LM_TERMINATION_CONTINUES : (double)cs.termination); pay_store(&r[LMR_INITIAL_COST], cs.initial_cost);
           pay_store(&r[LMR_FINAL_COST], cs.cost); pay_store(&r[LMR_LINEARIZE_CALLS], (double)cs.lin_calls);
           pay_store(&r[LMR_STEP_CALLS], (double)cs.step_calls); pay_store(&r[LMR_SEL], (double)cs.sel);
           const long long tn = (long long)wall_clock64();
@@ -1848,7 +1899,7 @@
         }
         for (int i = tid; i < 7 * K; i += nt) pay_store(&a.host_result[LMR_DOUBLES + i], cPose[i]);
       }
-      return issue(LMOP_DELIVER);
+      return issue(yield ? LMOP_YIELD : LMOP_DELIVER);
     }
     const double radius = cs.radius;
     for (int q = tid; q < n; q += nt) {
@@ -2143,7 +2194,10 @@
     if (shift && W.R.active && lane == W.R.first) { a.points_a[3 * W.R.j] = W.R.p.x; a.points_a[3 * W.R.j + 1] = W.R.p.y; a.points_a[3 * W.R.j + 2] = W.R.p.z; }
     load_chunk_table(P, my_chunk, tabs, shift);
   }
-  if (MULTI) {
+  if (MULTI && a.resume) {
+    for (int t = 0; t < turns.count; ++t) load_chunk_table(P, turns.chunk(t), tabs + t * a.tab_words, shift);
+    __builtin_amdgcn_fence(__ATOMIC_ACQUIRE, "agent");
+  } else if (MULTI) {
     for (int t = 0; t < turns.count; ++t) {
       const int chunk = turns.chunk(t);
       const ObsRec R = load_obs_image(P, chunk, lane, a.points_a, shift);
@@ -2181,7 +2235,12 @@
     P.cand_points = sel ? a.points_a : a.points_b;
     P.pay_tag = cs.tag;
     P.pay_parity = (int)(cs.op_count & 1u);
-    if (op == LMOP_DELIVER) {
+    const bool yielding = MULTI && op == LMOP_YIELD;
+    if (yielding) {
+      __builtin_amdgcn_fence(__ATOMIC_RELEASE, "agent");
+    }
+    if (op == LMOP_DELIVER || yielding) {
+      if (!yielding) {
       if (a.export_points && my_wave_works) {
         ObsRec R = W.R;
         if (R.active) R.p = D3{P.points[3 * R.j], P.points[3 * R.j + 1], P.points[3 * R.j + 2]};
@@ -2207,6 +2266,7 @@
         const float x = (float)P.points[3 * j], y = (float)P.points[3 * j + 1], z = (float)P.points[3 * j + 2];
         const unsigned long long lo = ((unsigned long long)__float_as_uint(y) << 32) | __float_as_uint(x), hi = ((unsigned long long)key << 32) | __float_as_uint(z);
         slot_store2<true>(reinterpret_cast<double*>(a.store + (key & a.store_mask)), __longlong_as_double((long long)lo), __longlong_as_double((long long)hi));
+      }
       }
       if (a.dbg && tid == 0) {
         unsigned* g = a.dbg + 16 * blockIdx.x;
@@ -2754,6 +2814,13 @@
   long wide_launches = 0;
   long fallbacks = 0;
   bool lm_inflight = false;
+  double* d_yield = nullptr;
+  int yield_iters = -1;
+  bool lm_yielded = false;
+  int lm_yield_seq = 0;
+  const void* lm_yield_src = nullptr;
+  int lm_resumes_now = 0;
+  long lm_resumes = 0;
   hipStream_t lm_stream = nullptr;
   LmLane* h_lane = nullptr;
   unsigned lm_base = 0;
@@ -2805,6 +2872,8 @@
   SVO_HIP_CHECK(ctx, hipHostMalloc((void**)&ba->h_bstat, sizeof(double) * ((size_t)BULK_RING * BS_DOUBLES + BC_WORDS), hipHostMallocCoherent));
   memset(ba->h_bstat, 0, sizeof(double) * ((size_t)BULK_RING * BS_DOUBLES + BC_WORDS));
   A(ba->d_lmc, unsigned, LMC_WORDS);
+  A(ba->d_yield, double, 2 * (YR_SCALARS + (nmax > 0 ? nmax : 1) + 7 * Kmax));
+  SVO_HIP_CHECK(ctx, hipMemset(ba->d_yield, 0, sizeof(double) * 2 * (YR_SCALARS + (nmax > 0 ? nmax : 1) + 7 * Kmax)));
   SVO_HIP_CHECK(ctx, hipHostMalloc((void**)&ba->h_lane, sizeof(LmLane), hipHostMallocCoherent));
   if (getenv("SVO_BA_TRACE")) A(ba->d_lmdbg, unsigned, 16 * 4096);
   SVO_HIP_CHECK(ctx, hipMemset(ba->d_lmc, 0, LMC_WORDS * sizeof(unsigned)));
@@ -2911,7 +2980,7 @@
   if (getenv("SVO_TIMING") && ba->lm_n) {
     fprintf(stderr, "[svo ba] solve forms: compact %ld, wide at k = 1..%d:", ba->lm_k_solves[0], LM_MAX_WAVE_CHUNKS);
     for (int k = 1; k <= LM_MAX_WAVE_CHUNKS; ++k) fprintf(stderr, " %ld", ba->lm_k_solves[k]);
-    fprintf(stderr, "; gave up %ld\n", ba->fallbacks);
+    fprintf(stderr, "; gave up %ld; continuation launches of solves that stepped aside %ld (%.2f per solve)\n", ba->fallbacks, ba->lm_resumes, (double)ba->lm_resumes / ba->lm_n);
   }
   const bool wide_traced = ba->lm_iters_wide > 0 && ba->d_lmdbg != nullptr;
   const double wi = (double)std::max(ba->lm_iters_wide, 1l), ci = (double)std::max(ba->lmc_iters, 1l);
@@ -2935,7 +3004,7 @@
                     "system build %.2f, Cholesky %.2f, step tail %.2f\n", ba->lmc_n, (double)ba->lmc_iters / std::max(ba->lmc_n, 1l), ba->lmc_tp[13] / ci, 1e-2 * ba->lmc_tp[0] / ci,
             1e-2 * ba->lmc_tp[3] / ci, 1e-2 * ba->lmc_tp[1] / ci, 1e-2 * ba->lmc_tp[2] / ci, 1e-2 * ba->lmc_tp[6] / ci, 1e-2 * ba->lmc_tp[7] / ci, 1e-2 * ba->lmc_tp[8] / ci, 1e-2 * ba->lmc_tp[9] / ci);
   if (ba->stream) (void)hipStreamSynchronize(ba->stream);
-  void* ptrs[] = {ba->d_res, ba->d_lmdbg, ba->d_lmc, ba->d_arrive, ba->d_pay, ba->d_step, ba->d_bctl, d.sp, d.part1, d.part2, ba->d_arena};
+  void* ptrs[] = {ba->d_res, ba->d_lmdbg, ba->d_lmc, ba->d_yield, ba->d_arrive, ba->d_pay, ba->d_step, ba->d_bctl, d.sp, d.part1, d.part2, ba->d_arena};
   if (ba->h_bstat) (void)hipHostFree(ba->h_bstat);
   if (ba->h_arena) (void)hipHostFree(ba->h_arena);
   if (ba->h_store_stage) (void)hipHostFree(ba->h_store_stage);
@@ -2996,8 +3065,14 @@
 
 extern "C" int svo_ba_solve_forms(svo_ba* ba, long* counts, int n, long* gave_up) {
   if (!ba || !counts || n < 1) return SVO_ERR_INVALID;
-  for (int i = 0; i < n; ++i) counts[i] = i <= LM_MAX_WAVE_CHUNKS ? ba->lm_k_solves[i] : 0;
+  for (int i = 0; i < n; ++i) counts[i] = i <= LM_MAX_WAVE_CHUNKS ? ba->lm_k_solves[i] : (i == LM_MAX_WAVE_CHUNKS + 1 ? ba->lm_resumes : 0);
   if (gave_up) *gave_up = ba->fallbacks;
+  return SVO_OK;
+}
+
+extern "C" int svo_ba_set_yield_iterations(svo_ba* ba, int n) {
+  if (!ba || n < -1 || ba->lm_inflight || ba->lm_yielded) return SVO_ERR_INVALID;
+  ba->yield_iters = n;
   return SVO_OK;
 }
 
@@ -3228,6 +3303,7 @@
 
 static int ba_upload(svo_ba* ba, int K, const double* poses7, int npts, const double* points3, int M,
                      const int32_t* op, const int32_t* oj, const double* uv) {
+  ba->lm_yielded = false; ba->lm_resumes_now = 0;
   const int rc = ba_upload_checked(ba, K, poses7, npts, points3, M, op, oj, uv);
   if (rc != SVO_OK) {
     ba->d.K = 0; ba->d.n = 0; ba->d.M = 0; ba->d.L = 0; ba->d.C = 0;
@@ -3505,6 +3581,11 @@
   return env == 1;
 }
 
+int ba_lm_yield_iters(const svo_ba* ba) {
+  static const int env = [] { const char* e = getenv("SVO_BA_YIELD_ITERS"); const int v = e && *e ? atoi(e) : 0; return v < 0 ? 0 : v; }();
+  return ba->yield_iters >= 0 ? ba->yield_iters : env;
+}
+
 bool ba_device_lm_fill(svo_ba* ba, int* cost, size_t* lds_out, bool forced, bool compact = false, int* waves_out = nullptr) {
   BaDev& d = ba->d;
   if (!d.det || d.C <= 0 || !ba_zero_copy(ba) || !(forced || ba->device_lm == 1 || (ba->device_lm < 0 && ba_device_lm_wanted())) || !ba->h_lane) return false;
@@ -3524,12 +3605,13 @@
   }
   d.points = ba->cur_points; d.cand_points = ba->cand_points; d.poses = ba->cur_poses; d.cand_poses = ba->cand_poses;
   d.flag = nullptr;
-  if (ba->arena_partial && ba_refresh_arena_image(ba)) return false;
+  const bool resume = ba->lm_yielded && !compact;
+  if (!resume && ba->arena_partial && ba_refresh_arena_image(ba)) return false;
   LmLane& L = *ba->h_lane;
   L.P = d;
   LmDevArgs& a = L.a;
   a.cnt = ba->d_lmc;
-  a.arena_src = ba->arena_dirty ? ba->h_arena : nullptr;
+  a.arena_src = resume ? ba->lm_yield_src : (ba->arena_dirty ? ba->h_arena : nullptr);
   a.arena_dst = ba->d_arena; a.arena_bytes = ba->arena_bytes;
   a.points_a = ba->cur_points; a.points_b = ba->cand_points;
   a.export_points = ba->n_points ? ba->h_out_points : nullptr;
@@ -3542,6 +3624,9 @@
   a.tab_words = compact ? ba_lmc_tab_words(ba) : ba_lm_tab_words(ba);
   a.wave_chunks = kw;
   a.wave_contig = ba_lm_wave_contig() ? 1 : 0;
+  a.yield_after = kw > 1 ? ba_lm_yield_iters(ba) : 0;
+  a.resume = resume ? ba->lm_yield_seq : 0;
+  a.yield_rec = ba->d_yield;
   a.opt.max_iterations = ba->opt.max_iterations;
   a.opt.function_tolerance = ba->opt.function_tolerance; a.opt.gradient_tolerance = ba->opt.gradient_tolerance;
   a.opt.parameter_tolerance = ba->opt.parameter_tolerance; a.opt.initial_radius = ba->opt.initial_radius;
@@ -3576,7 +3661,7 @@
     int cost = 0;
     size_t lds = 0;
     if ((ba->d.G > 1 ? 1 : (ba_lm_wave_chunks(ba) > 1 ? 2 : 0)) != form) continue;
-    if (ba_wants_compact(ba)) { to_compact[i] = true; continue; }
+    if (ba_wants_compact(ba) && !ba->lm_yielded) { to_compact[i] = true; continue; }
     if (!ba_device_lm_fill(ba, &cost, &lds, forced)) continue;
     if (lds > 32 * 1024 && hipFuncSetAttribute(kernel, hipFuncAttributeMaxDynamicSharedMemorySize, 120 * 1024) != hipSuccess) continue;
     bool admitted = ba_resident_admission(ba)->admit(cost, ba->ctx->device);
@@ -3595,7 +3680,7 @@
         if (admitted) { ba->h_lane->a.wave_chunks = k; lds = lds_k; }
       }
     }
-    if (!admitted) { to_compact[i] = overflow; continue; }
+    if (!admitted) { to_compact[i] = overflow && !ba->lm_yielded; continue; }
     if (ba->lm_counters_dirty || !ba->lm_have_base) {
       if (hipMemsetAsync(ba->d_lmc, 0, LMC_WORDS * sizeof(unsigned), st) != hipSuccess) { ba_resident_admission(ba)->release(); continue; }
     }
@@ -3626,7 +3711,8 @@
       if (ba->arena_dirty) ba->arena_partial = true;
       ba->arena_dirty = false;
       ba->lm_inflight = true; ba->lm_compact_inflight = false;
-      ++ba->lm_k_solves[std::min(std::max(ba->h_lane->a.wave_chunks, 1), LM_MAX_WAVE_CHUNKS)];
+      if (ba->lm_yielded) ++ba->lm_resumes_now;
+      else { ++ba->lm_k_solves[std::min(std::max(ba->h_lane->a.wave_chunks, 1), LM_MAX_WAVE_CHUNKS)]; ba->lm_yield_src = ba->h_lane->a.arena_src; }
       ba->lm_stream = st;
       ba->res_export = ba->h_lane->a.export_points != nullptr;
       if (launched_mask) *launched_mask |= 1ull << tidx[i];
@@ -3682,6 +3768,7 @@
   return launched + n_compact;
 }
 
+constexpr int SVO_BA_CONTINUES = 1, SVO_BA_REFUSED = 2;
 int ba_device_lm_end(svo_ba* ba, svo_ba_summary* sum) {
   if (!ba->lm_inflight) return SVO_ERR_INVALID;
   svo_ctx* ctx = ba->ctx;
@@ -3714,6 +3801,13 @@
   }
   const double* r = ba->h_result;
   if (!was_compact) { ba->lm_base = (unsigned)r[LMR_C_ARRIVE]; ba->lm_have_base = true; }
+  if (!was_compact && r[LMR_TERMINATION] == LM_TERMINATION_CONTINUES) {
+    for (int i = 0; i < 14; ++i) ba->lm_tp[i] += r[LMR_TP0 + i];
+    ba->lm_t_wait += r[LMR_T_WAIT]; ba->lm_t_ctl += r[LMR_T_CTL]; ba->lm_t_body += r[LMR_T_BODY]; ba->lm_t_total += r[LMR_T_TOTAL];
+    ba->lm_yielded = true; ba->lm_yield_seq = ba->seq;
+    return SVO_BA_CONTINUES;
+  }
+  ba->lm_resumes += ba->lm_resumes_now; ba->lm_resumes_now = 0; ba->lm_yielded = false;
   memcpy(ba->h_poses.data(), r + LMR_DOUBLES, sizeof(double) * 7 * (size_t)d.K);
   if (r[LMR_SEL] != 0.0) { std::swap(ba->cur_points, ba->cand_points); std::swap(ba->cur_poses, ba->cand_poses); }
   ba->host_points_valid = ba->res_export;
@@ -4079,6 +4173,22 @@
   ba->upload_pending = false;
   ba->lm_penalty = 64;
   ++ba->fallbacks;
+  ba->lm_yielded = false; ba->lm_resumes_now = 0;
+}
+
+static void ba_drop_yield(svo_ba* ba) {
+  if (!ba->lm_yielded) return;
+  const int penalty = ba->lm_penalty; const long fallbacks = ba->fallbacks;
+  ba_after_giveup(ba);
+  ba->lm_penalty = penalty; ba->fallbacks = fallbacks;
+}
+
+static int ba_device_lm_join(svo_ba* ba, svo_ba_summary* sum) {
+  for (;;) {
+    const int rc = ba_device_lm_end(ba, sum);
+    if (rc != SVO_BA_CONTINUES) return rc;
+    if (ba_device_lm_launch(&ba, 1, ba->lm_stream, true, nullptr) != 1) { ba_drop_yield(ba); return SVO_BA_REFUSED; }
+  }
 }
 
 static int ba_lm(svo_ba* ba, svo_ba_summary* sum) {
@@ -4091,19 +4201,22 @@
   ops.accept = op_accept;
   memset(&ba->stats, 0, sizeof(ba->stats));
   int fell_back = 0;
-  if (ba_device_lm_launch(&ba, 1, ba->stream, false, nullptr) == 1) {
-    const int rcd = ba_device_lm_end(ba, sum);
+  if (ba_device_lm_launch(&ba, 1, ba->lm_yielded ? ba->lm_stream : ba->stream, ba->lm_yielded, nullptr) == 1) {
+    const int rcd = ba_device_lm_join(ba, sum);
     d.flag = nullptr;
     if (rcd == SVO_OK) { if (ba->lm_penalty > 0) --ba->lm_penalty; return rcd; }
+    if (rcd != SVO_BA_REFUSED) {
     ba_after_giveup(ba);
     fell_back = 1;
-    if (ba_device_lm_launch(&ba, 1, ba->stream, true, nullptr) == 1) {
+    }
+    if (rcd != SVO_BA_REFUSED && ba_device_lm_launch(&ba, 1, ba->stream, true, nullptr) == 1) {
       const int rc2 = ba_device_lm_end(ba, sum);
       d.flag = nullptr;
       if (rc2 == SVO_OK) { ba->stats.fallbacks = 1; ctx->err.clear(); return rc2; }
       ba_after_giveup(ba);
     }
   }
+  ba_drop_yield(ba);
   if (ba_bulk_control_wanted(ba)) return ba_lm_bulk_device(ba, sum);
   {
     const int rcf = ba_flush_arena(ba);
@@ -4154,8 +4267,9 @@
     svo_ba_summary* sum = summaries ? &summaries[i] : nullptr;
     int rc;
     if ((mask >> i) & 1ull) {
-      rc = ba_device_lm_end(ba, sum); ba->d.flag = nullptr;
+      rc = ba_device_lm_join(ba, sum); ba->d.flag = nullptr;
       if (rc == SVO_OK) { if (ba->lm_penalty > 0) --ba->lm_penalty; }
+      else if (rc == SVO_BA_REFUSED) rc = ba_lm(ba, sum);
       else {
         ba_after_giveup(ba);
         rc = ba_lm(ba, sum);
@@ -4358,6 +4472,15 @@
   return (v == ba->seq || (v == -ba->seq && ba->seq != 0)) ? 1 : 0;
 }
 
+int svo_ba_solve_continues(svo_ba* ba) {
+  if (!ba || !ba->lm_inflight || ba->lm_compact_inflight) return 0;
+  if (__atomic_load_n(ba->h_flag, __ATOMIC_ACQUIRE) != ba->seq) return 0;
+  if (ba->h_result[LMR_TERMINATION] != LM_TERMINATION_CONTINUES) return 0;
+  svo_use_device(ba->ctx);
+  return ba_device_lm_end(ba, nullptr) == SVO_BA_CONTINUES ? 1 : 0;
+}
+int svo_ba_solve_yielded(svo_ba* ba) { return ba && ba->lm_yielded ? 1 : 0; }
+
 int svo_ba_solve_holds_budget(svo_ba* ba) { return ba && ba->lm_inflight && !ba->lm_compact_inflight ? 1 : 0; }
 
 int svo_ba_solve_finish(svo_ba* ba, svo_ba_summary* summary) {
@@ -4372,8 +4495,9 @@
   const bool on_device = ba->lm_inflight;
   bool on_device_ok = on_device;
   if (ba->lm_inflight) {
-    rc = ba_device_lm_end(ba, summary); ba->d.flag = nullptr;
+    rc = ba_device_lm_join(ba, summary); ba->d.flag = nullptr;
     if (rc == SVO_OK) { if (ba->lm_penalty > 0) --ba->lm_penalty; }
+    else if (rc == SVO_BA_REFUSED) { rc = ba_lm(ba, summary); on_device_ok = false; }
     else {
       ba_after_giveup(ba);
       rc = ba_lm(ba, summary);
diff --git a/stereo_vo_amd/csrc/group_kernels.h b/stereo_vo_amd/csrc/group_kernels.h
--- a/stereo_vo_amd/csrc/group_kernels.h
+++ b/stereo_vo_amd/csrc/group_kernels.h
@@ -49,6 +49,8 @@
 int svo_ba_solve_prepare(svo_ba* ba);
 int svo_ba_solve_launch(svo_ba** bas, int n, void* stream, unsigned long long* launched_mask);
 int svo_ba_solve_poll(svo_ba* ba);
+int svo_ba_solve_continues(svo_ba* ba);
+int svo_ba_solve_yielded(svo_ba* ba);
 int svo_ba_solve_holds_budget(svo_ba* ba);
 int svo_ba_solve_finish(svo_ba* ba, svo_ba_summary* summary);
 void svo_ba_work(svo_ba* ba, double* out4, int reset);
diff --git a/stereo_vo_amd/host/group.cpp b/stereo_vo_amd/host/group.cpp
--- a/stereo_vo_amd/host/group.cpp
+++ b/stereo_vo_amd/host/group.cpp
@@ -22,6 +22,12 @@
 #include "svo.h"
 
 namespace {
+
+constexpr int GROUP_SOLVE_YIELD_DEFAULT = 8;
+int group_solve_yield_default() {
+  const char* e = getenv("SVO_BA_YIELD_ITERS");
+  return e && *e ? std::max(0, atoi(e)) : GROUP_SOLVE_YIELD_DEFAULT;
+}
 
 enum LaneState { L_IDLE = 0, L_TRACK_WAIT, L_NEED_SOLVE, L_PNP_WAIT, L_TRI_WAIT, L_DONE };
 enum BaState { BA_NONE = 0, BA_ASSEMBLING, BA_READY, BA_INFLIGHT, BA_HOST_SOLVING, BA_HOST_DONE };
@@ -58,6 +64,7 @@
   int ba_rc = 0;
   int ba_launch = 0, ba_line = 0;
   unsigned long long ba_ready_seq = 0;
+  bool ba_yielded = false;
   bool has_keyframe = false;
   double solved_pose[7] = {1, 0, 0, 0, 0, 0, 0};
   int last_iterations = 0;
@@ -198,6 +205,7 @@
 int finish_solve(svo_pipeline_group* g, Lane* l) {
   const int st = l->ba_state.load(std::memory_order_acquire);
   l->ba_ready_seq = 0;
+  l->ba_yielded = false;
   if (st == BA_NONE) return SVO_OK;
   int rc = SVO_OK;
   const auto tf0 = std::chrono::steady_clock::now();
@@ -395,6 +403,7 @@
     rc = svo_ba_create(ctx, &l->ba, p->window_size, &p->cam, &opt, max_obs, max_obs);
     if (!rc) rc = svo_ba_attach_store(l->ba, l->d_store, l->store_mask);
     if (!rc) rc = svo_ba_use_stream(l->ba, g->st_ba[li % g->n_ba]);
+    if (!rc) rc = svo_ba_set_yield_iterations(l->ba, group_solve_yield_default());
   }
   if (rc) { svo_pipeline_group_destroy(g); return rc; }
   {
@@ -444,6 +453,15 @@
   for (int i = 0; i < l->n && i < capacity; ++i) {
     if (ids) ids[i] = (int64_t)si[i];
     if (xy) { xy[2 * i] = sx[2 * i]; xy[2 * i + 1] = sx[2 * i + 1]; }
+  }
+  return SVO_OK;
+}
+
+extern "C" int svo_pipeline_group_set_solve_yield(svo_pipeline_group* g, int n) {
+  if (!g || n < 0) return SVO_ERR_INVALID;
+  for (Lane* l : g->lanes) {
+    const int rc = svo_ba_set_yield_iterations(l->ba, n);
+    if (rc) return rc;
   }
   return SVO_OK;
 }
@@ -921,8 +939,14 @@
     }
   }
 
-  static bool solve_came_back(Lane* l) {
+  bool solve_came_back(Lane* l) {
     const int bs = l->ba_state.load(std::memory_order_acquire);
+    if (bs == BA_INFLIGHT && svo_ba_solve_poll(l->ba) && svo_ba_solve_continues(l->ba)) {
+      l->ba_yielded = true;
+      l->ba_state.store(BA_READY, std::memory_order_release);
+      progressed = true;
+      return false;
+    }
     return (bs == BA_INFLIGHT && svo_ba_solve_poll(l->ba)) || bs == BA_HOST_DONE;
   }
   bool any_solve_in_flight(bool holding_budget) const {
@@ -944,12 +968,15 @@
 
   void solves_departed(const int* lanes, int n, unsigned long long taken, int line, int carried, const char* what) {
     ++g->ba_launch_id;
-    if (carried > 0) count(ST_SOLVE, carried);
+    int fresh = 0;
+    for (int k = 0; k < n; ++k) fresh += ((taken >> k) & 1ull) && !g->lanes[lanes[k]]->ba_yielded;
+    if (fresh > 0) count(ST_SOLVE, fresh);
+    else if (carried > 0) progressed = true;
     for (int k = 0; k < n; ++k) {
       if (!((taken >> k) & 1ull)) continue;
       Lane* l = g->lanes[lanes[k]];
       EV(lanes[k], what, carried);
-      l->ba_launch = g->ba_launch_id; l->ba_line = line; l->ba_ready_seq = 0;
+      l->ba_launch = g->ba_launch_id; l->ba_line = line;
       l->ba_state.store(BA_INFLIGHT, std::memory_order_release);
     }
   }
@@ -968,7 +995,7 @@
     }
     std::sort(q_ba.begin(), q_ba.end(), [&](int a, int b) {
       const Lane* la = g->lanes[a]; const Lane* lb = g->lanes[b];
-      return svo_solve_before(la->state == L_NEED_SOLVE, la->ba_ready_seq, lb->state == L_NEED_SOLVE, lb->ba_ready_seq);
+      return svo_solve_before(la->state == L_NEED_SOLVE, la->ba_yielded, la->ba_ready_seq, lb->state == L_NEED_SOLVE, lb->ba_yielded, lb->ba_ready_seq);
     });
     for (int i = 0; i < MAX_LINES; ++i) ba_line_busy[i] = false;
     for (const Lane* l : g->lanes)
@@ -984,9 +1011,9 @@
     if (cline < 0) return not_taken;
     svo_ba* cb[SVO_MAX_LANES];
     int cl[SVO_MAX_LANES], nc = 0;
-    for (int k = 0; k < n; ++k) if (!((mask >> k) & 1ull)) { cb[nc] = bas[k]; cl[nc++] = cand[k]; (void)svo_ba_set_solve_form(bas[k], 1); }
+    for (int k = 0; k < n; ++k) if (!((mask >> k) & 1ull) && !g->lanes[cand[k]]->ba_yielded) { cb[nc] = bas[k]; cl[nc++] = cand[k]; (void)svo_ba_set_solve_form(bas[k], 1); }
     unsigned long long cmask = 0;
-    const int went = svo_ba_solve_launch(cb, nc, g->st_ba[cline], &cmask);
+    const int went = nc ? svo_ba_solve_launch(cb, nc, g->st_ba[cline], &cmask) : 0;
     for (int k = 0; k < nc; ++k) (void)svo_ba_set_solve_form(cb[k], -1);
     if (went <= 0) return not_taken;
     solves_departed(cl, nc, cmask, cline, went, "ba_launch_compact");
diff --git a/stereo_vo_amd/host/group_lines.h b/stereo_vo_amd/host/group_lines.h
--- a/stereo_vo_amd/host/group_lines.h
+++ b/stereo_vo_amd/host/group_lines.h
@@ -28,4 +28,9 @@
   if (a_waits != b_waits) return a_waits;
   return a_ready_seq < b_ready_seq;
 }
+inline bool svo_solve_before(bool a_waits, bool a_yielded, unsigned long long a_ready_seq, bool b_waits, bool b_yielded, unsigned long long b_ready_seq) {
+  if (a_waits != b_waits) return a_waits;
+  if (a_yielded != b_yielded) return a_yielded;
+  return a_ready_seq < b_ready_seq;
+}
 #endif
```

New measurement: 15330 frames/s, median of 6. 1.14x the previous value.
